# adelacvg/NS2VC

Measured on AMD Instinct MI355X. Metric: denoiser-steps/sec (10s@24kHz Vocos latent, bs32), higher is better.
Workload: dtype fp16; 1 GPU; 10 s utterance (T=938 Vocos frames), batch 32/GPU, prompt Lp=469, 20-step unipc order 2, hipGraph-captured loop, fp16 MFMA operands; timed job = set_condition + 20 steps; global_batch=32, frames=938, prompt_frames=469, solver=unipc, parallelism=dp1

## Files before the change

ns2vc_amd/csrc/attn.hip:

```cpp
#include "common.h"
#include "mma.h"
#include <cstdlib>

namespace ns2vc {

template <typename T> struct AMma;
template <> struct AMma<float> {
  static constexpr int SZ = 4;
  __device__ static __forceinline__ void mma(f32x16_t& acc, const u32x4_t& a, const u32x4_t& b) {
    acc = __builtin_amdgcn_mfma_f32_32x32x2f32(__uint_as_float(a.x), __uint_as_float(b.x), acc, 0, 0, 0);
    acc = __builtin_amdgcn_mfma_f32_32x32x2f32(__uint_as_float(a.y), __uint_as_float(b.y), acc, 0, 0, 0);
    acc = __builtin_amdgcn_mfma_f32_32x32x2f32(__uint_as_float(a.z), __uint_as_float(b.z), acc, 0, 0, 0);
    acc = __builtin_amdgcn_mfma_f32_32x32x2f32(__uint_as_float(a.w), __uint_as_float(b.w), acc, 0, 0, 0);
  }
  __device__ static __forceinline__ f32x16_t mma0(const u32x4_t& a, const u32x4_t& b) {
    f32x16_t acc = __builtin_amdgcn_mfma_f32_32x32x2f32(__uint_as_float(a.x), __uint_as_float(b.x), f32x16_t{0.f, 0.f, 0.f, 0.f, 0.f, 0.f, 0.f, 0.f, 0.f, 0.f, 0.f, 0.f, 0.f, 0.f, 0.f, 0.f}, 0, 0, 0);
    acc = __builtin_amdgcn_mfma_f32_32x32x2f32(__uint_as_float(a.y), __uint_as_float(b.y), acc, 0, 0, 0);
    acc = __builtin_amdgcn_mfma_f32_32x32x2f32(__uint_as_float(a.z), __uint_as_float(b.z), acc, 0, 0, 0);
    acc = __builtin_amdgcn_mfma_f32_32x32x2f32(__uint_as_float(a.w), __uint_as_float(b.w), acc, 0, 0, 0);
    return acc;
  }
  __device__ static __forceinline__ int vpos(int key) { return key; }
};
template <typename TM> struct AMma16 {
// ... 34 lines not shown
  return fmaxf(__uint_as_float(r[0]), __uint_as_float(r[1]));
}
__device__ __forceinline__ float half_sum(float v) {
  const auto r = __builtin_amdgcn_permlane32_swap(__float_as_uint(v), __float_as_uint(v), false, false);
  return __uint_as_float(r[0]) + __uint_as_float(r[1]);
}

template <typename TM> __device__ __forceinline__ float round_op(float x);
template <> __device__ __forceinline__ float round_op<float>(float x) { return x; }
template <> __device__ __forceinline__ float round_op<bf16_t>(float x) { return __uint_as_float(pack_bf16x2(0.f, x) & 0xffff0000u); }
template <> __device__ __forceinline__ float round_op<f16_t>(float x) { return f16_lo(pack_f16x2(x, 0.f)); }
template <typename TM> __device__ __forceinline__ u32x4_t aux_chunk(float e0, float e1);
template <> __device__ __forceinline__ u32x4_t aux_chunk<float>(float e0, float e1) { return u32x4_t{__float_as_uint(e0), __float_as_uint(e1), 0u, 0u}; }
template <> __device__ __forceinline__ u32x4_t aux_chunk<bf16_t>(float e0, float e1) { return u32x4_t{pack_bf16x2(e0, e1), 0u, 0u, 0u}; }
template <> __device__ __forceinline__ u32x4_t aux_chunk<f16_t>(float e0, float e1) { return u32x4_t{pack_f16x2(e0, e1), 0u, 0u, 0u}; }
template <typename TM> __device__ __forceinline__ TM op_from_float(float x);
template <> __device__ __forceinline__ float op_from_float<float>(float x) { return x; }
template <> __device__ __forceinline__ bf16_t op_from_float<bf16_t>(float x) { bf16_t r; r.v = (uint16_t)pack_bf16x2(x, 0.f); return r; }
template <> __device__ __forceinline__ f16_t op_from_float<f16_t>(float x) { f16_t r; r.v = (uint16_t)pack_f16x2(x, 0.f); return r; }

__device__ __forceinline__ uint32_t pack_fp8x4(float a, float b, float c, float d) {
  int v = __builtin_amdgcn_cvt_pk_fp8_f32(a, b, 0, false);
  v = __builtin_amdgcn_cvt_pk_fp8_f32(c, d, v, true);
  return (uint32_t)v;
}
typedef int i32x8_t __attribute__((ext_vector_type(8)));
#ifndef NS2VC_ATTN_OPT
#define NS2VC_ATTN_OPT 1
#endif
template <bool B> struct OptTag { static constexpr bool value = B; };
__device__ int g_attn_exact_only = 0;
__device__ __forceinline__ int vpos8(int key) { return ((key & 4) << 3) | ((key & 32) >> 1) | ((key & 24) >> 1) | (key & 3); }
template <typename TM, int HD, int KEYS, bool P8, bool MASKED = false>
__global__ __launch_bounds__(256) void attn_kernel(const AttnArgs a) {
  op_mode_init<TM>();
  static_assert(!P8 || (sizeof(TM) == 2 && KEYS == 64), "the fp8 PV path: 16-bit operand types, one 64-key tile per f8f6f4 MFMA");
  constexpr int NSUB = KEYS / 32;
  constexpr int SZ = AMma<TM>::SZ;
  constexpr int EPC = 16 / SZ;
  constexpr int NS = HD * SZ / 32;
  constexpr int KROWB = HD * SZ + 48;
  constexpr int VSZ = P8 ? 1 : SZ;
  constexpr int VROWB = KEYS * VSZ + 16;
  constexpr int HDX = (HD + 1 + 31) / 32 * 32;
  constexpr int DT = HDX / 32;
  constexpr int NSL = SZ;
  constexpr int KBYTES = KEYS * KROWB, VBYTES = HDX * VROWB;
  constexpr int STAGE = KBYTES + VBYTES;
  constexpr int PPR = HD * SZ / 16;
  constexpr int NPIECE = KEYS * PPR;
  constexpr int UPT = (NPIECE + 255) / 256;
  constexpr float THRESH = P8 ? 8.0f : 12.0f;
  extern __shared__ __attribute__((aligned(16))) char smem[];

  const int tid = threadIdx.x, lane = tid & 63, wave = tid >> 6;
  const int l31 = lane & 31, hi = lane >> 5;
  const int nqb = (a.Lq + 127) >> 7;
  int b, h, qb;
  {
    const int nwg = gridDim.x, bid = blockIdx.x;
    const int qn = nwg >> 3, rn = nwg & 7, xcd = bid & 7, idx = bid >> 3;
    const int swz = (xcd < rn ? xcd * (qn + 1) : rn * (qn + 1) + (xcd - rn) * qn) + idx;
    b = swz / (a.H * nqb);
    const int rem = swz - b * (a.H * nqb);
    h = rem / nqb;
    qb = rem - h * nqb;
  }
  const int q = qb * 128 + wave * 32 + l31;
  int Lqb = a.Lq, Lkb = a.Lk;
  if constexpr (MASKED) {
    if (a.q_lens) Lqb = min(max(a.q_lens[b], 0), a.Lq);
    if (a.k_lens) Lkb = min(max(a.k_lens[b], 1), a.Lk);
    if (qb * 128 >= Lqb) {
      if (q < a.Lq) {
        char* zp = reinterpret_cast<char*>(a.out) + ((size_t)(b * a.Lq + q) * a.ldo + h * HD) * SZ;
#pragma unroll
        for (int pc = hi; pc < PPR; pc += 2) *reinterpret_cast<u32x4_t*>(zp + pc * 16) = u32x4_t{0, 0, 0, 0};
      }
      return;
    }
  }
  const float LOG2E = 1.4426950408889634f;
  const float sc2 = a.scale * LOG2E;

  for (int i = tid * 16; i < 2 * STAGE; i += 256 * 16) *reinterpret_cast<u32x4_t*>(smem + i) = u32x4_t{0, 0, 0, 0};
  __syncthreads();
  for (int i = tid; i < 2 * KEYS; i += 256) {
    const int st = i / KEYS, key = i - st * KEYS;
    *reinterpret_cast<TM*>(smem + st * STAGE + key * KROWB + HD * SZ) = op_from_float<TM>(1.0f);
    if constexpr (P8) *reinterpret_cast<uint8_t*>(smem + st * STAGE + KBYTES + HD * VROWB + key) = (uint8_t)0x38;
    else *reinterpret_cast<TM*>(smem + st * STAGE + KBYTES + HD * VROWB + key * SZ) = op_from_float<TM>(1.0f);
  }

// ... 232 lines not shown
          const uint32_t b0 = Op16<TM>::pack(o[d][8 * gp + 4] * inv, o[d][8 * gp + 5] * inv), b1 = Op16<TM>::pack(o[d][8 * gp + 6] * inv, o[d][8 * gp + 7] * inv);
          const auto x0 = __builtin_amdgcn_permlane32_swap(a0, b0, false, false);
          const auto x1 = __builtin_amdgcn_permlane32_swap(a1, b1, false, false);
#if defined(NS2VC_ATTN_ABLATE_STORE)
          asm volatile("" :: "v"(x0[0]), "v"(x1[0]), "v"(x0[1]), "v"(x1[1]));
#else
          if (q < a.Lq) *reinterpret_cast<u32x4_t*>(op + d * 32 + 8 * (2 * gp + hi)) = padded ? u32x4_t{0, 0, 0, 0} : u32x4_t{x0[0], x1[0], x0[1], x1[1]};
#endif
        }
      }
  } else if (q < a.Lq) {
#pragma unroll
    for (int d = 0; d < DT; ++d)
#pragma unroll
      for (int gq = 0; gq < 4; ++gq) {
        const int d0 = d * 32 + 8 * gq + 4 * hi;
        if (d0 < HD) store_op4<TM>(op + d0, padded ? 0.f : o[d][4 * gq] * inv, padded ? 0.f : o[d][4 * gq + 1] * inv, padded ? 0.f : o[d][4 * gq + 2] * inv,
                                   padded ? 0.f : o[d][4 * gq + 3] * inv);
      }
  }
}

template <typename TM, int HD, int KEYS> static constexpr size_t attn_lds() {
  constexpr int SZ = AMma<TM>::SZ;
  constexpr int HDX = (HD + 1 + 31) / 32 * 32;
  return 2 * (size_t)(KEYS * (HD * SZ + 48) + HDX * (KEYS * SZ + 16));
}

template <typename TM, int HD> static constexpr bool attn_has128() { return sizeof(TM) == 2 && HD <= 32; }
static int g_force_keys = 0;
void set_forced_attn_keys(int keys) { g_force_keys = keys; }
void set_attn_optimistic(int on) { const int v = on ? 0 : 1; (void)hipMemcpyToSymbol(HIP_SYMBOL(g_attn_exact_only), &v, sizeof(v)); }

template <typename TM, int HD, int KEYS> static hipError_t launch_hdk(const AttnArgs& a, hipStream_t s) {
  dim3 grid(((a.Lq + 127) / 128) * a.H * a.B);
  const size_t lds = attn_lds<TM, HD, KEYS>();
  if (a.q_lens || a.k_lens) hipLaunchKernelGGL((attn_kernel<TM, HD, KEYS, false, true>), grid, dim3(256), lds, s, a);
  else hipLaunchKernelGGL((attn_kernel<TM, HD, KEYS, false>), grid, dim3(256), lds, s, a);
  return hipGetLastError();
}
template <typename TM, int HD> static hipError_t launch_hd(const AttnArgs& a, hipStream_t s) {
  if (a.pv_fp8 && (a.q_lens || a.k_lens)) return hipErrorInvalidValue;
  if constexpr (sizeof(TM) == 2) {
    if (a.pv_fp8) {
      dim3 grid(((a.Lq + 127) / 128) * a.H * a.B);
      const size_t lds = attn_lds<TM, HD, 64>();
      hipLaunchKernelGGL((attn_kernel<TM, HD, 64, true>), grid, dim3(256), lds, s, a);
      return hipGetLastError();
    }
  } else if (a.pv_fp8) return hipErrorInvalidValue;
  if constexpr (attn_has128<TM, HD>()) {
    if (g_force_keys == 128) return launch_hdk<TM, HD, 128>(a, s);
  }
  return launch_hdk<TM, HD, 64>(a, s);
}

template <typename TM> static hipError_t launch_tm(const AttnArgs& a, int hd, hipStream_t s) {
  switch (hd) {
    case 16: return launch_hd<TM, 16>(a, s);
    case 32: return launch_hd<TM, 32>(a, s);
    case 48: return launch_hd<TM, 48>(a, s);
    case 64: return launch_hd<TM, 64>(a, s);
    default: return hipErrorInvalidValue;
  }
}

template <typename TM, int HD> static hipError_t set_attr() {
  hipError_t e = hipFuncSetAttribute(reinterpret_cast<const void*>(attn_kernel<TM, HD, 64, false>), hipFuncAttributeMaxDynamicSharedMemorySize,
                                     (int)attn_lds<TM, HD, 64>());
  if (e == hipSuccess)
    e = hipFuncSetAttribute(reinterpret_cast<const void*>(attn_kernel<TM, HD, 64, false, true>), hipFuncAttributeMaxDynamicSharedMemorySize,
                            (int)attn_lds<TM, HD, 64>());
  if constexpr (attn_has128<TM, HD>()) {
    if (e == hipSuccess)
      e = hipFuncSetAttribute(reinterpret_cast<const void*>(attn_kernel<TM, HD, 128, false>), hipFuncAttributeMaxDynamicSharedMemorySize,
                              (int)attn_lds<TM, HD, 128>());
    if (e == hipSuccess)
      e = hipFuncSetAttribute(reinterpret_cast<const void*>(attn_kernel<TM, HD, 128, false, true>), hipFuncAttributeMaxDynamicSharedMemorySize,
                              (int)attn_lds<TM, HD, 128>());
  }
  if constexpr (sizeof(TM) == 2) {
    if (e == hipSuccess)
      e = hipFuncSetAttribute(reinterpret_cast<const void*>(attn_kernel<TM, HD, 64, true>), hipFuncAttributeMaxDynamicSharedMemorySize,
                              (int)attn_lds<TM, HD, 64>());
  }
  return e;
}
template <typename TM> static hipError_t set_attr_tm() {
  hipError_t e;
  if ((e = set_attr<TM, 16>()) != hipSuccess) return e;
  if ((e = set_attr<TM, 32>()) != hipSuccess) return e;
  if ((e = set_attr<TM, 48>()) != hipSuccess) return e;
  return set_attr<TM, 64>();
}
hipError_t init_attn_attributes() {
  hipError_t e = set_attr_tm<float>();
  if (e == hipSuccess) e = set_attr_tm<bf16_t>();
  if (e == hipSuccess) e = set_attr_tm<f16_t>();
  return e;
}

bool attention_masks_rows(const AttnArgs& a, int head_dim, int prec) {
  if (a.pv_fp8) return false;
  if (head_dim != 16 && head_dim != 32 && head_dim != 48 && head_dim != 64) return false;
  return prec == PREC_BF16 || prec == PREC_F16 || prec == PREC_F32;
}

hipError_t launch_attention(const AttnArgs& a, int head_dim, int prec, hipStream_t s) {
  const int al = prec == PREC_F32 ? 3 : 7;
  if (!a.q || !a.k || !a.v || !a.out) return hipErrorInvalidValue;
  if ((a.q_lens || a.k_lens) && !attention_masks_rows(a, head_dim, prec)) return hipErrorInvalidValue;
  if (a.Lq <= 0 || a.Lk <= 0 || (a.ldq & al) || (a.ldk & al) || (a.ldv & al) || (a.ldo & al)) return hipErrorInvalidValue;
  if (reinterpret_cast<uintptr_t>(a.out) & 15) return hipErrorInvalidValue;
  switch (prec) {
    case PREC_BF16: return launch_tm<bf16_t>(a, head_dim, s);
    case PREC_F16: return launch_tm<f16_t>(a, head_dim, s);
    case PREC_F32: return launch_tm<float>(a, head_dim, s);
    default: return hipErrorInvalidValue;
  }
}

}
```

ns2vc_amd/csrc/common.h:

```cpp
#pragma once
#include <hip/hip_runtime.h>
#include <stdint.h>
#include <stddef.h>
#include <vector>
#include "../../include/ns2vc_hip.h"

namespace ns2vc {

typedef __attribute__((ext_vector_type(8))) __bf16 bf16x8_t;
typedef __attribute__((ext_vector_type(16))) float f32x16_t;
typedef __attribute__((ext_vector_type(4))) float f32x4_t;
typedef __attribute__((ext_vector_type(4))) unsigned int u32x4_t;

struct bf16_t { uint16_t v; };
struct f16_t { uint16_t v; };

__host__ __device__ inline uint16_t f32_to_bf16_bits(float f) {
  union { float f; uint32_t u; } x;
  x.f = f;
  uint32_t u = x.u;
  if ((u & 0x7fffffffu) > 0x7f800000u) return (uint16_t)((u >> 16) | 0x40);
  u += 0x7fffu + ((u >> 16) & 1u);
  return (uint16_t)(u >> 16);
}
__host__ __device__ inline float bf16_bits_to_f32(uint16_t h) {
  union { float f; uint32_t u; } x;
  x.u = (uint32_t)h << 16;
  return x.f;
}

__host__ __device__ inline uint16_t f32_to_f16_bits(float f) {
  union { float f; uint32_t u; } x;
  x.f = f;
  const uint32_t sign = (x.u >> 16) & 0x8000u;
  uint32_t a = x.u & 0x7fffffffu;
  if (a > 0x7f800000u) return (uint16_t)(sign | 0x7e00u);
  if (a >= 0x477ff000u) return (uint16_t)(sign | 0x7c00u);
  if (a < 0x38800000u) {
// ... 172 lines not shown
  const float nd = k.d1c * (vmp - m) + d2c * dm2;
  oxb = nb; od1 = nd; oxe = nb - k.pc * nd - pe * dm2; om = m;
}

__device__ __forceinline__ uint4 philox4x32_10(uint4 c, uint32_t k0, uint32_t k1) {
#pragma unroll
  for (int r = 0; r < 10; ++r) {
    if (r) { k0 += 0x9E3779B9u; k1 += 0xBB67AE85u; }
    const uint32_t lo0 = 0xD2511F53u * c.x, hi0 = __umulhi(0xD2511F53u, c.x);
    const uint32_t lo1 = 0xCD9E8D57u * c.z, hi1 = __umulhi(0xCD9E8D57u, c.z);
    c = make_uint4(hi1 ^ c.y ^ k0, lo1, hi0 ^ c.w ^ k1, lo0);
  }
  return c;
}
__device__ __forceinline__ void box_muller(uint32_t a, uint32_t b, float& z0, float& z1) {
  const float u1 = ((float)a + 1.0f) * 0x1p-32f;
  const float u2 = (float)b * 0x1p-32f;
  const float r = sqrtf(-2.0f * logf(u1));
  float sn, cs;
  sincosf(u2 * 6.2831853071795864769f, &sn, &cs);
  z0 = r * cs; z1 = r * sn;
}
__device__ __forceinline__ float4 philox_gauss4(unsigned long long seed, uint32_t t, uint32_t q, uint32_t step) {
  const uint4 x = philox4x32_10(make_uint4(t, q, step, 0u), (uint32_t)seed, (uint32_t)(seed >> 32));
  float4 z;
  box_muller(x.x, x.y, z.x, z.y);
  box_muller(x.z, x.w, z.z, z.w);
  return z;
}

constexpr double GN_SUM_SCALE = 268435456.0;
constexpr double GN_SQ_SCALE = 65536.0;

hipError_t launch_gemm(const GemmArgs& g, int prec, hipStream_t s);
size_t xattn_pack_bytes(int B, int Lk, int hd);
hipError_t launch_xattn_pack(const void* k, int ldk, const void* v, int ldv, int B, int Lk, int hd, void* out, int prec, hipStream_t s);
bool gemm_masks_rows(const GemmArgs& g, int prec);
bool gemm_uses_convts(const GemmArgs& g, int prec);
int last_gemm_refusal_line();
hipError_t launch_attention(const AttnArgs& a, int head_dim, int prec, hipStream_t s);
bool attention_masks_rows(const AttnArgs& a, int head_dim, int prec);
hipError_t init_gemm_attributes();
bool convts_eligible(const GemmArgs& g, int prec);
int convts_default_bn(const GemmArgs& g);
int convts_bn_for(const GemmArgs& g, int bn128_min);
void set_convts_bn128_min(int wgs);
int convts_row_blocks(const GemmArgs& g);
hipError_t launch_convts(const GemmArgs& g, int prec, int bn, int nl, int ks, hipStream_t s);
hipError_t init_convts_attributes();
hipError_t pack_conv3_tiled(const float* rows, int N, int ctot, int c2, int prec, std::vector<unsigned char>& out);
void set_forced_gemm_tile(int bm, int bn, int stages);
void set_gemm_trace(unsigned long long* p);
hipError_t init_attn_attributes();
void set_forced_attn_keys(int keys);
hipError_t launch_ffn(const ::ns2vc_ffn_args& a, int prec, hipStream_t s);
bool ffn_eligible(int dim, int T, int prec);
bool ffn_masks_rows(const ::ns2vc_ffn_args& a, int prec);
hipError_t init_ffn_attributes();
hipError_t pack_ffn_stream(const float* w1p, const float* w2f, const float* w0, int dim, int prec, std::vector<unsigned short>& out);
void set_ffn_trace(unsigned long long* p);
bool geglu_eligible(int dim, int T, int prec);
hipError_t pack_geglu_stream(const float* w1p, const float* bias1p, int dim, int prec, std::vector<unsigned short>& stream, std::vector<float>& consts);
hipError_t launch_geglu(const ::ns2vc_geglu_args& a, int prec, hipStream_t s);
bool geglu_masks_rows(const ::ns2vc_geglu_args& a, int prec);
hipError_t init_geglu_attributes();
void set_gg_trace(unsigned long long* p);
void set_ts_trace(unsigned long long* p);
void set_attn_optimistic(int on);

hipError_t launch_gn_partial(const float* a0, int lda0, int c0, const float* a1, int lda1, int c1,
                             int B, int T, int G, double* partial, int nchunk, int rows_per_chunk, hipStream_t s);
hipError_t launch_gn_apply(const float* a0, int lda0, int c0, const float* a1, int lda1, int c1, int B, int T, int G, float eps,
                           const double* partial, int nchunk, const long long* st0, const long long* st1, const float* gamma,
                           const float* beta, const float* temb, int ldtemb, int temb_off, int silu, void* out_op, void* raw_op,
                           int prec, hipStream_t s, int pair = 0,
                           const int* lens = nullptr);
hipError_t launch_mask_rows(void* dst, size_t ldd_bytes, size_t row_bytes, int B, int T, const int* lens, hipStream_t s, const void* src = nullptr,
                            size_t lds_bytes = 0, int Tsrc = 0, int up = 0);
hipError_t launch_ln_apply_op(const float* x, int ldx, int M, int C, float eps, void* out_op, int prec, hipStream_t s);
hipError_t launch_cast_op(const float* x, size_t n, void* out_op, int prec, hipStream_t s, int split = 0);
hipError_t launch_time_embed(const float* t_ptr, int t_stride, const int* step_ptr, int coef_stride,
                             const float* w1t, const float* b1, const float* w2t, const float* b2,
                             const float* aug, float* emb, void* emb_act_op, int prec, int B, int tdim, int edim, hipStream_t s);
hipError_t launch_rowchain(const ::ns2vc_rowchain_args& a, int prec, hipStream_t s);
bool rowchain_eligible(int dim, int n2, int T, int prec);
bool rowchain_masks_rows(const ::ns2vc_rowchain_args& a, int prec);
hipError_t init_rowchain_attributes();
hipError_t pack_rowchain_stream(const float* w1, const float* w2, int dim, int n2, int prec, std::vector<unsigned short>& out, int slices = 1);
int rowchain_slice_blocks(int n2, int slices);
void set_rc_trace(unsigned long long* p);
void set_forced_rowchain_tokens(int nt);
hipError_t launch_emb_from_table(const float* table, const int* step_ptr, const float* aug, float* emb, void* emb_act_op, int prec, int B,
                                 int edim, hipStream_t s);
int probe_xcd_round_robin(unsigned* map8 = nullptr);
hipError_t launch_zero(void* p, size_t bytes, hipStream_t s, int* counter = nullptr);
hipError_t launch_copy16(const void* src, void* dst, size_t bytes, hipStream_t s);
hipError_t launch_poison(unsigned pattern, int lds_bytes, unsigned* sink, hipStream_t s);
hipError_t launch_nct_to_btc(const float* src, int C, int T, int B, float* dst_f32, void* dst_op, int prec, int ldd, int cpad, hipStream_t s,
                             int ldd_op = 0, int split = 0);
hipError_t launch_btc_to_nct(const float* src, int lds, int C, int T, int B, float* dst, hipStream_t s);
hipError_t launch_mask_bias(const uint8_t* mask, int n, float* bias, hipStream_t s);
hipError_t launch_ln_apply(const float* x, int M, int C, float eps, const float* gamma, const float* beta,
                           float* out, int L, int Lout_stride_rows, hipStream_t s);
hipError_t launch_pool_cls(float* seq, int B, int L, int C, const float* pos, hipStream_t s);
hipError_t launch_pool_attn(const float* qkv, int B, int L1, int C, int heads, float* pooled, hipStream_t s);
hipError_t launch_pool_proj(const float* pooled, int B, int C, const float* wt, const float* b, int E,
                            const float* gamma, const float* beta, float eps, float* out, hipStream_t s);
struct SolverNoise { const unsigned long long* seeds = nullptr; const int* lens = nullptr; int T = 0, ld = 0, nc = 0; };
hipError_t launch_solver_update(const float* coef, const int* step_ptr, int ncoef, const float* x0,
                                float* xe, void* xe_op, int prec, float* xbar, float* d1, float* mprev, size_t n, hipStream_t s,
                                int split = 0,
                                const SolverNoise& noise = SolverNoise(),
                                float* mprev2 = nullptr);
hipError_t launch_noise(const unsigned long long* seeds, int B, int nc, int T, int ld, int step, const int* lens, float* out, hipStream_t s);
hipError_t launch_fill_i32(int* p, int v, hipStream_t s);
hipError_t launch_placement(unsigned* dev_out, int n_blocks, int spin, hipStream_t s);
hipError_t launch_snapshot_u32(unsigned* src, unsigned* dst, hipStream_t s);
// ... 3 lines not shown
```

ns2vc_amd/csrc/convts.hip:

```cpp
#include "common.h"
#include "mma.h"
#include "gnpro.h"
#include "epilogue.h"
#include <type_traits>
#include <vector>
#include <cstring>

namespace ns2vc {

constexpr int TS_ROW = 128;
constexpr int TS_BM = 128;
constexpr int TS_BMO = 126;
constexpr int TS_ASLOT = TS_BM * TS_ROW;

__device__ unsigned long long* g_ts_trace = nullptr;
void set_ts_trace(unsigned long long* p) { (void)hipMemcpyToSymbol(HIP_SYMBOL(g_ts_trace), &p, sizeof(p)); }
#ifndef NS2VC_GEMM_TRACE
#define NS2VC_GEMM_TRACE 0
#endif
#if NS2VC_GEMM_TRACE
#define TS_NOW() __builtin_readcyclecounter()
#define TS_STAMP(i) do { if (tr && (tid == 0)) tr[i] = TS_NOW(); } while (0)
#define TS_CLK(t) do { t = TS_NOW(); } while (0)
#define TS_ACC(a, t) do { const unsigned long long n_ = TS_NOW(); a += n_ - t; t = n_; } while (0)
// ... 9 lines not shown
#endif
#ifndef NS2VC_TS_KS_DEFAULT
#define NS2VC_TS_KS_DEFAULT 0
#endif
#ifndef NS2VC_TS_NL_DEFAULT
#define NS2VC_TS_NL_DEFAULT 8
#endif
#ifndef NS2VC_TS_GNP_XB
#define NS2VC_TS_GNP_XB 4
#endif
#ifndef NS2VC_TS_NLD4
#define NS2VC_TS_NLD4 0
#endif
#ifndef NS2VC_CONS_PF
#define NS2VC_CONS_PF 1
#endif
#ifndef NS2VC_TS_CHUNK
#define NS2VC_TS_CHUNK 1
#endif
#if NS2VC_TS_CHUNK
template <int BN> struct TsRing { static constexpr int SW = BN == 64 ? 9 : 6; };
#else
template <int BN> struct TsRing { static constexpr int SW = 3; };
#endif
template <int LO, int HI> struct TsWait {
  static __device__ __forceinline__ void run(int n) {
    if constexpr (LO == HI) wait_vmcnt<LO>();
    else { constexpr int MID = (LO + HI + 1) / 2; if (n >= MID) TsWait<MID, HI>::run(n); else TsWait<LO, MID - 1>::run(n); }
  }
};

enum { TS_GN_NONE = 0, TS_GN_PRO = 1, TS_GN_INLOOP = 2, TS_GN_PAIR = 3, TS_MASKED = 4 };
template <typename TM, int BN, int NL, int GNPF, bool KS = false, bool SOL = false>
__global__ __launch_bounds__(64 * (NL + 4)) void conv3ts_kernel(const GemmArgs g) {
  constexpr int GNP = GNPF & 3;
  constexpr bool MASKED = (GNPF & TS_MASKED) != 0;
  op_mode_init<TM>();
  constexpr int EPC = MmaT<TM>::EPC;
  constexpr int BKE = 8 * EPC;
  constexpr int NW = NL + 4, EOFF = NW - 8;
  constexpr int NLD = (GNP == 2 || (NS2VC_TS_CHUNK && NS2VC_TS_NLD4 && NL == 8)) ? 4 : NL;
  constexpr int LTH = NLD * 64, RPP = LTH / 8, PASSB = RPP * TS_ROW;
  constexpr int LA = TS_BM / RPP, LB = BN / RPP;
  static_assert(!KS || BN == 64, "the K-split consumer layout is the 64-column tile's");
  constexpr int WGN = BN / 64, WGM = KS ? 2 : 4 / WGN, WM = TS_BM / WGM, MT = WM / 32, NT = 2;
  constexpr int NKK = KS ? 2 : 4;
  constexpr int WSLOT = BN * TS_ROW;
  constexpr int SW = TsRing<BN>::SW, D = SW - 1;
  constexpr unsigned SZB = sizeof(TM);
  static_assert(BN == 64 || BN == 128, "BN");
  static_assert(LA >= 1 && LB >= 1 && (NS2VC_TS_CHUNK ? SW : D) * LB + 3 * LA <= 60, "vmcnt range");
  extern __shared__ __attribute__((aligned(16))) char smem[];
  char* const aring = smem;
  char* const wring = smem + 3 * TS_ASLOT;
  char* const tabmem = smem + 3 * TS_ASLOT + SW * WSLOT;
  static_assert(GNP != 2 || NS2VC_TS_CHUNK, "the in-loop GroupNorm rides the chunk-granular loop");

  const int tid = threadIdx.x;
  const int lane = tid & 63;
  const int wave = __builtin_amdgcn_readfirstlane(tid >> 6);
  const bool loader = wave < NLD, consumer = wave >= NL;
  const bool producer = GNP == 2 && wave >= NLD && wave < NL;
  const int ewave = wave - EOFF;
  const int cw = consumer ? wave - NL : 0;
  const int wm = KS ? cw >> 1 : cw / WGN, wn = KS ? 0 : cw % WGN;
  const int kh = KS ? cw & 1 : 0;
  const unsigned lds0 = (unsigned)(size_t)smem;
// ... 440 lines not shown
        for (int p = 0; p < 8; ++p) {
          const int lc = p ^ ((r >> 1) & 7);
          for (int e = 0; e < epc; ++e) {
            const float v = rows[(size_t)n * K + koff + lc * epc + e];
            unsigned char* dst = blk + r * 128 + p * 16 + e * esz;
            if (prec == PREC_F32) memcpy(dst, &v, 4);
            else { const uint16_t q = f32_to_op16_bits(v, prec); memcpy(dst, &q, 2); }
          }
        }
      }
    }
  return hipSuccess;
}

static constexpr size_t ts_lds_bytes(int bn) { return (size_t)3 * TS_ASLOT + (size_t)(bn == 64 ? TsRing<64>::SW : TsRing<128>::SW) * bn * TS_ROW + 4096; }

bool convts_eligible(const GemmArgs& g, int prec) {
  const int bke = prec == PREC_F32 ? 32 : 64;
  if (g.taps != 3 || g.tmode != TMODE_SAME || g.Tin != g.Tout || g.Tin < 66 || g.geglu || g.rowstats || g.ln_stats) return false;
  if ((g.N % 64) || (g.c0 % bke) || (g.c1 % bke) || (g.c2 % bke) || g.c0 + g.c1 < bke) return false;
  if ((unsigned long long)g.B * (g.Tin + 1) > 0x7fff0000ull) return false;
  if (g.sol_coef && (g.N != 128 || !g.sol_step || !g.sol_xe || !g.sol_xe_op || !g.sol_xbar || !g.sol_d1 || !g.sol_mprev || (g.sol_ld & 3))) return false;
  return true;
}
static int g_bn128_min = 160;
void set_convts_bn128_min(int wgs) { g_bn128_min = wgs > 0 ? wgs : 160; }
int convts_bn_for(const GemmArgs& g, int bn128_min) {
  const long long nbm = ((long long)g.B * (g.Tin + 1) + TS_BMO - 1) / TS_BMO;
  return ((g.N % 128) == 0 && nbm * (g.N / 128) >= bn128_min) ? 128 : 64;
}
int convts_default_bn(const GemmArgs& g) { return (g.conv_bn == 64 || (g.conv_bn == 128 && g.N % 128 == 0)) ? g.conv_bn : convts_bn_for(g, g_bn128_min); }
int convts_row_blocks(const GemmArgs& g) { return (int)(((long long)g.B * (g.Tin + 1) + TS_BMO - 1) / TS_BMO); }

template <typename TM, int BN, int NL, bool KS> static hipError_t launch_ts_cfg(const GemmArgs& g, hipStream_t s) {
  const int nbm = convts_row_blocks(g), nbn = g.N / BN;
  int nb = nbm * nbn;
  if (g.gnp_x && g.gnp_sync && nbn > 1) nb = 8 * ((nbm + 7) / 8) * nbn;
  constexpr bool HAS_INLOOP = NS2VC_TS_CHUNK && NL == 8 && !KS;
  if (g.lens) {
    constexpr bool HAS_MASKED = NL == 8 && !KS;
    if constexpr (HAS_MASKED) {
      if (g.sol_coef) return hipErrorInvalidValue;
      if (g.gnp_x && g.gnp_pair) {
        if constexpr (!std::is_same<TM, float>::value) hipLaunchKernelGGL((conv3ts_kernel<TM, BN, NL, TS_GN_PAIR | TS_MASKED, KS>), dim3(nb), dim3(64 * (NL + 4)), ts_lds_bytes(BN), s, g);
        else return hipErrorInvalidValue;
      }
      else if (g.gnp_x) hipLaunchKernelGGL((conv3ts_kernel<TM, BN, NL, TS_GN_PRO | TS_MASKED, KS>), dim3(nb), dim3(64 * (NL + 4)), ts_lds_bytes(BN), s, g);
      else hipLaunchKernelGGL((conv3ts_kernel<TM, BN, NL, TS_GN_NONE | TS_MASKED, KS>), dim3(nb), dim3(64 * (NL + 4)), ts_lds_bytes(BN), s, g);
    } else return hipErrorInvalidValue;
  }
  else if (g.sol_coef) {
    constexpr bool HAS_SOL = BN == 128 && NL == 8 && !KS;
    if constexpr (HAS_SOL) {
      if (g.gnp_x && g.gnp_pair) {
        if constexpr (!std::is_same<TM, float>::value) hipLaunchKernelGGL((conv3ts_kernel<TM, BN, NL, 3, KS, true>), dim3(nb), dim3(64 * (NL + 4)), ts_lds_bytes(BN), s, g);
        else return hipErrorInvalidValue;
      }
      else if (g.gnp_x) hipLaunchKernelGGL((conv3ts_kernel<TM, BN, NL, 1, KS, true>), dim3(nb), dim3(64 * (NL + 4)), ts_lds_bytes(BN), s, g);
      else hipLaunchKernelGGL((conv3ts_kernel<TM, BN, NL, 0, KS, true>), dim3(nb), dim3(64 * (NL + 4)), ts_lds_bytes(BN), s, g);
    } else return hipErrorInvalidValue;
  }
  else if (g.gnp_x && g.gnp_pair) {
    if constexpr (!std::is_same<TM, float>::value && NL == 8 && !KS) hipLaunchKernelGGL((conv3ts_kernel<TM, BN, NL, 3, KS>), dim3(nb), dim3(64 * (NL + 4)), ts_lds_bytes(BN), s, g);
    else return hipErrorInvalidValue;
  }
  else if (g.gnp_x && HAS_INLOOP && g.algo != 2) {
    if constexpr (HAS_INLOOP) hipLaunchKernelGGL((conv3ts_kernel<TM, BN, NL, 2, KS>), dim3(nb), dim3(64 * (NL + 4)), ts_lds_bytes(BN), s, g);
  }
  else if (g.gnp_x) hipLaunchKernelGGL((conv3ts_kernel<TM, BN, NL, 1, KS>), dim3(nb), dim3(64 * (NL + 4)), ts_lds_bytes(BN), s, g);
  else hipLaunchKernelGGL((conv3ts_kernel<TM, BN, NL, 0, KS>), dim3(nb), dim3(64 * (NL + 4)), ts_lds_bytes(BN), s, g);
  return hipGetLastError();
}
template <typename TM> static hipError_t launch_ts_typed(const GemmArgs& g, int bn, int nl, int ks, hipStream_t s) {
  if (bn == 64 && nl == 4) return ks ? launch_ts_cfg<TM, 64, 4, true>(g, s) : launch_ts_cfg<TM, 64, 4, false>(g, s);
  if (bn == 64 && nl == 8) return ks ? launch_ts_cfg<TM, 64, 8, true>(g, s) : launch_ts_cfg<TM, 64, 8, false>(g, s);
  if (bn == 128 && nl == 4) return launch_ts_cfg<TM, 128, 4, false>(g, s);
  if (bn == 128 && nl == 8) return launch_ts_cfg<TM, 128, 8, false>(g, s);
  return hipErrorInvalidValue;
}
hipError_t launch_convts(const GemmArgs& g, int prec, int bn, int nl, int ks, hipStream_t s) {
  if (!convts_eligible(g, prec)) return hipErrorInvalidValue;
  if (!bn) bn = convts_default_bn(g);
  if (!nl) nl = NS2VC_TS_NL_DEFAULT;
  if (ks < 0) ks = NS2VC_TS_KS_DEFAULT;
  if (g.sol_coef) { bn = 128; nl = 8; ks = 0; }
  if (g.lens) { nl = 8; ks = 0; }
  if (g.N % bn) return hipErrorInvalidValue;
  switch (prec) {
    case PREC_BF16: return launch_ts_typed<bf16_t>(g, bn, nl, ks, s);
    case PREC_F16: return launch_ts_typed<f16_t>(g, bn, nl, ks, s);
    case PREC_F32: return launch_ts_typed<float>(g, bn, nl, ks, s);
    default: return hipErrorInvalidValue;
  }
}

template <typename K> static hipError_t ts_set_lds(K kern, size_t bytes) {
  return hipFuncSetAttribute(reinterpret_cast<const void*>(kern), hipFuncAttributeMaxDynamicSharedMemorySize, (int)bytes);
}
template <typename TM> static hipError_t ts_init_typed() {
  hipError_t e = hipSuccess;
#define NS2VC_TS_SET(BN_, NL_)                                                                      \
  if (e == hipSuccess) e = ts_set_lds(conv3ts_kernel<TM, BN_, NL_, 0>, ts_lds_bytes(BN_));     \
  if (e == hipSuccess) e = ts_set_lds(conv3ts_kernel<TM, BN_, NL_, 1>, ts_lds_bytes(BN_))
  NS2VC_TS_SET(64, 4); NS2VC_TS_SET(128, 4); NS2VC_TS_SET(64, 8); NS2VC_TS_SET(128, 8);
#if NS2VC_TS_CHUNK
  if (e == hipSuccess) e = ts_set_lds(conv3ts_kernel<TM, 64, 8, 2>, ts_lds_bytes(64));
  if (e == hipSuccess) e = ts_set_lds(conv3ts_kernel<TM, 128, 8, 2>, ts_lds_bytes(128));
#endif
  if (e == hipSuccess) e = ts_set_lds(conv3ts_kernel<TM, 128, 8, 0, false, true>, ts_lds_bytes(128));
  if (e == hipSuccess) e = ts_set_lds(conv3ts_kernel<TM, 128, 8, 1, false, true>, ts_lds_bytes(128));
  if constexpr (!std::is_same<TM, float>::value) {
    if (e == hipSuccess) e = ts_set_lds(conv3ts_kernel<TM, 128, 8, 3, false, true>, ts_lds_bytes(128));
    if (e == hipSuccess) e = ts_set_lds(conv3ts_kernel<TM, 64, 8, 3>, ts_lds_bytes(64));
    if (e == hipSuccess) e = ts_set_lds(conv3ts_kernel<TM, 128, 8, 3>, ts_lds_bytes(128));
  }
  if (e == hipSuccess) e = ts_set_lds(conv3ts_kernel<TM, 64, 8, TS_GN_NONE | TS_MASKED>, ts_lds_bytes(64));
  if (e == hipSuccess) e = ts_set_lds(conv3ts_kernel<TM, 64, 8, TS_GN_PRO | TS_MASKED>, ts_lds_bytes(64));
  if (e == hipSuccess) e = ts_set_lds(conv3ts_kernel<TM, 128, 8, TS_GN_NONE | TS_MASKED>, ts_lds_bytes(128));
  if (e == hipSuccess) e = ts_set_lds(conv3ts_kernel<TM, 128, 8, TS_GN_PRO | TS_MASKED>, ts_lds_bytes(128));
  if constexpr (!std::is_same<TM, float>::value) {
    if (e == hipSuccess) e = ts_set_lds(conv3ts_kernel<TM, 64, 8, TS_GN_PAIR | TS_MASKED>, ts_lds_bytes(64));
    if (e == hipSuccess) e = ts_set_lds(conv3ts_kernel<TM, 128, 8, TS_GN_PAIR | TS_MASKED>, ts_lds_bytes(128));
  }
  if (e == hipSuccess) e = ts_set_lds(conv3ts_kernel<TM, 64, 4, 0, true>, ts_lds_bytes(64));
// ... 15 lines not shown
```

ns2vc_amd/csrc/engine.cpp:

```cpp
#include "engine_internal.h"

#include <algorithm>
#include <cstdlib>
#include <cstring>

using namespace ns2vc;

static int bind_device(ns2vc_unet* h) {
  int cur = -1;
  HIPCHK(hipGetDevice(&cur));
  if (cur != h->device) HIPCHK(hipSetDevice(h->device));
  return 0;
}
int ns2vc::check_ready(ns2vc_unet* h, bool need_plan) {
  if (!h) return fail("null engine handle");
  if (bind_device(h)) return 1;
  if (!h->finalized) return fail("weights not finalized (call ns2vc_unet_finalize_weights)");
  if (need_plan && !h->arena) return fail("engine not prepared (call ns2vc_unet_prepare)");
  return 0;
}

int ns2vc::load_state(ns2vc_unet* h, const float* x_bct, hipStream_t s) {
  HIPCHK(launch_nct_to_btc(x_bct, h->cfg.latent_channels, h->T, h->B, h->xe, h->xe_op, h->prec, h->CP, h->CP, s, h->pair_width(), h->pair_off()));
  if (!h->lens.masked) return 0;
  const size_t ob = (size_t)h->pair_width() * operand_bytes(h->prec);
  HIPCHK(launch_mask_rows(h->xe, (size_t)h->CP * 4, (size_t)h->CP * 4, h->B, h->T, h->lens.dev, s));
  HIPCHK(launch_mask_rows(h->xe_op, ob, ob, h->B, h->T, h->lens.dev, s));
  return 0;
}

static const struct { const char* name; const char* env; bool ns2vc_unet::* member; } kOptions[] = {
  {"ln_linear", "NS2VC_LN_LINEAR", &ns2vc_unet::ln_linear}, {"fold_ff", "NS2VC_FOLD_FF", &ns2vc_unet::fold_ff},
  {"fuse_ffn", "NS2VC_FUSE_FFN", &ns2vc_unet::fuse_ffn}, {"fuse_ffn_pre", "NS2VC_FUSE_FFN_PRE", &ns2vc_unet::fuse_ffn_pre},
  {"fuse_geglu", "NS2VC_FUSE_GEGLU", &ns2vc_unet::fuse_geglu}, {"fuse_rows", "NS2VC_FUSE_ROWS", &ns2vc_unet::fuse_rows},
  {"fuse_rows_gn", "NS2VC_FUSE_ROWS_GN", &ns2vc_unet::fuse_rows_gn}, {"fuse_gn_gemm", "NS2VC_FUSE_GN_GEMM", &ns2vc_unet::fuse_gn_gemm},
  {"fuse_gn_cat", "NS2VC_FUSE_GN_CAT", &ns2vc_unet::fuse_gn_cat}, {"gn_coop", "NS2VC_GN_COOP", &ns2vc_unet::gn_coop},
  {"slice_rows", "NS2VC_SLICE_ROWS", &ns2vc_unet::slice_rows}, {"attn_fp8", "NS2VC_ATTN_FP8", &ns2vc_unet::attn_fp8},
  {"attn_optimistic", "NS2VC_ATTN_OPTIMISTIC", &ns2vc_unet::attn_optimistic}, {"conv_ts", "NS2VC_CONV_TS", &ns2vc_unet::conv_ts},
  {"conv_wtiled", "NS2VC_CONV_WTILED", &ns2vc_unet::conv_wtiled}, {"gn_inloop", "NS2VC_GN_INLOOP", &ns2vc_unet::gn_inloop},
  {"fuse_solver", "NS2VC_FUSE_SOLVER", &ns2vc_unet::fuse_solver}, {"fuse_xattn", "NS2VC_FUSE_XATTN", &ns2vc_unet::fuse_xattn},
  {"fork_temb", "NS2VC_FORK_TEMB", &ns2vc_unet::fork_temb}, {"exact_io", "NS2VC_EXACT_IO", &ns2vc_unet::exact_io},
  {"split_io", "NS2VC_SPLIT_IO", &ns2vc_unet::split_io}, {"masked_fuse", "NS2VC_MASKED_FUSE", &ns2vc_unet::masked_fuse},
  {"masked_attn", "NS2VC_MASKED_ATTN", &ns2vc_unet::masked_attn}, {"masked_rows", "NS2VC_MASKED_ROWS", &ns2vc_unet::masked_rows},
  {"masked_ffn", "NS2VC_MASKED_FFN", &ns2vc_unet::masked_ffn}, {"masked_geglu", "NS2VC_MASKED_GEGLU", &ns2vc_unet::masked_geglu}};
static bool* option_ptr(ns2vc_unet* h, const char* name) {
  for (const auto& o : kOptions)
    if (!strcmp(name, o.name)) return &(h->*o.member);
  return nullptr;
}

extern "C" {

int ns2vc_unet_create(const ns2vc_unet_cfg* cfg, ns2vc_unet** out) {
  if (!cfg || !out) return fail("null argument");
  if (cfg->n_levels < 2 || cfg->n_levels > NS2VC_MAX_LEVELS) return fail("n_levels=%d out of range (2..%d)", cfg->n_levels, NS2VC_MAX_LEVELS);
  if (cfg->latent_channels <= 0 || cfg->latent_channels > 128) return fail("latent_channels=%d must be in 1..128", cfg->latent_channels);
  if (cfg->content_channels <= 0 || cfg->content_channels % 64)
    return fail("content_channels=%d must be a positive multiple of 64", cfg->content_channels);
  if (cfg->cross_attention_dim <= 0 || cfg->cross_attention_dim % 128)
    return fail("cross_attention_dim=%d must be a positive multiple of 128", cfg->cross_attention_dim);
  if (cfg->heads < 1) return fail("heads=%d must be >= 1", cfg->heads);
  if (cfg->norm_num_groups < 1 || cfg->norm_num_groups > 8) return fail("norm_num_groups=%d unsupported (1..8)", cfg->norm_num_groups);
  if (cfg->layers_per_block < 1) return fail("layers_per_block=%d must be >= 1", cfg->layers_per_block);
  if (cfg->pool_heads < 1 || cfg->cross_attention_dim % cfg->pool_heads || cfg->cross_attention_dim / cfg->pool_heads > 8)
    return fail("cross_attention_dim=%d over pool_heads=%d: the pool head width must be a whole number <= 8", cfg->cross_attention_dim, cfg->pool_heads);
  if (cfg->block_out_channels[0] != 128) return fail("block_out_channels[0]=%d must be 128 (padded latent width)", cfg->block_out_channels[0]);
  for (int l = 0; l < cfg->n_levels; ++l) {
    const int c = cfg->block_out_channels[l];
    if (c <= 0 || c % 128 || c > 512) return fail("block_out_channels[%d]=%d must be a multiple of 128 in 128..512", l, c);
    if (c % cfg->heads) return fail("block_out_channels[%d]=%d not divisible by heads=%d", l, c, cfg->heads);
    const int hd = c / cfg->heads;
    if (hd != 16 && hd != 32 && hd != 48 && hd != 64)
      return fail("heads=%d gives head width %d at block_out_channels[%d]=%d (16/32/48/64 supported)", cfg->heads, hd, l, c);
    if (c % cfg->norm_num_groups || (c / cfg->norm_num_groups) % 4)
      return fail("block_out_channels[%d]=%d incompatible with norm_num_groups=%d (group width must be a multiple of 4)", l, c, cfg->norm_num_groups);
  }
  for (const BlockW& b : make_topology(*cfg))
// ... 304 lines not shown
int ns2vc_unet_tap_info(ns2vc_unet* h, int idx, char* name, int buflen, int* rows, int* cols) {
  if (!h || idx < 0 || idx >= (int)h->taps.size()) return fail("tap index out of range");
  snprintf(name, buflen, "%s", h->taps[idx].name.c_str());
  *rows = h->taps[idx].rows; *cols = h->taps[idx].cols;
  return 0;
}
int ns2vc_unet_tap_read(ns2vc_unet* h, int idx, float* host_dst) {
  if (!h || idx < 0 || idx >= (int)h->taps.size()) return fail("tap index out of range");
  HIPCHK(hipDeviceSynchronize());
  const Tap& t = h->taps[idx];
  HIPCHK(hipMemcpy(host_dst, t.copy, (size_t)t.rows * t.cols * sizeof(float), hipMemcpyDeviceToHost));
  return 0;
}
int ns2vc_unet_num_launches(ns2vc_unet* h, int* per_forward, int* per_condition) {
  if (!h) return fail("null engine handle");
  if (per_forward) *per_forward = (int)h->fwd_ops.size();
  if (per_condition) *per_condition = (int)h->cond_ops.size();
  return 0;
}

int ns2vc_unet_op_info(ns2vc_unet* h, int which, int idx, char* name, int buflen, int* kind, double* flops, double* bytes) {
  if (!h) return fail("null engine handle");
  if (which == 2) {
    static const char* const field[6] = {"begin", "end", "join", "first_reader", "readers", "forks"};
    if (!h->arena) return fail("engine not prepared (call ns2vc_unet_prepare)");
    if (idx < 0 || idx >= 6) return fail("op index out of range");
    GemmArgs g;
    const int v[6] = {h->tfork.begin, h->tfork.end, h->tfork.join, h->tfork.first, h->tfork.readers,
                      temb_forks(h, solver_in_conv_out(h, g) ? (size_t)h->conv_out_idx : h->fwd_ops.size()) ? 1 : 0};
    snprintf(name, buflen, "%s", field[idx]);
    *kind = v[idx]; *flops = 0.0; *bytes = 0.0;
    return 0;
  }
  const std::vector<Op>& ops = which ? h->cond_ops : h->fwd_ops;
  if (idx < 0 || idx >= (int)ops.size()) return fail("op index out of range");
  snprintf(name, buflen, "%s", ops[idx].name.c_str());
  *kind = ops[idx].kind; *flops = ops[idx].flops; *bytes = ops[idx].bytes;
  return 0;
}

int ns2vc_unet_profile_forward(ns2vc_unet* h, float* ms, int n_ms, int reps, void* stream) {
  if (check_ready(h, true)) return 1;
  const size_t n = h->fwd_ops.size();
  if ((size_t)n_ms < n) return fail("ms buffer too small: need %zu", n);
  if (reps < 1) reps = 1;
  hipStream_t s = (hipStream_t)stream;
  h->use_step_table = false;
  std::vector<hipEvent_t> ev(2 * n);
  for (auto& e : ev) HIPCHK(hipEventCreate(&e));
  int rc = 0;
  hipEvent_t rz0 = nullptr, rz1 = nullptr;
  const Op* rz_op = nullptr;
  for (size_t i = 0; i < n && !rc; ++i) {
    const Op& op = h->fwd_ops[i];
    if (op.rearm && !rz_op) rz_op = &op;
    if (hipEventRecord(ev[2 * i], s) != hipSuccess) rc = fail("hipEventRecord failed");
    for (int r = 0; r < reps && !rc; ++r) {
      hipError_t e = op.rearm ? op.rearm(s) : hipSuccess;
      if (e == hipSuccess) e = op.fn(s);
      if (e != hipSuccess) rc = fail("launch of '%s' failed: %s", op.name.c_str(), hipGetErrorString(e));
    }
    if (!rc && hipEventRecord(ev[2 * i + 1], s) != hipSuccess) rc = fail("hipEventRecord failed");
  }
  if (!rc && rz_op) {
    if (hipEventCreate(&rz0) != hipSuccess || hipEventCreate(&rz1) != hipSuccess) rc = fail("hipEventCreate failed");
    if (!rc) (void)hipEventRecord(rz0, s);
// ... 20 lines not shown
```

ns2vc_amd/csrc/engine_internal.h:

```cpp
#pragma once
#include "common.h"

#include <cstdarg>
#include <cstdio>
#include <functional>
#include <map>
#include <string>
#include <vector>

namespace ns2vc {

inline thread_local std::string g_err;

inline int fail(const char* fmt, ...) {
  char buf[1024];
  va_list ap;
  va_start(ap, fmt);
  vsnprintf(buf, sizeof(buf), fmt, ap);
  va_end(ap);
  g_err = buf;
  return 1;
}
#define HIPCHK(expr)                                                                                       \
  do {                                                                                                     \
    hipError_t _e = (expr);                                                                                \
    if (_e != hipSuccess) return ns2vc::fail("%s failed: %s (%s:%d)", #expr, hipGetErrorString(_e), __FILE__, __LINE__); \
  } while (0)

inline int round_up(int v, int m) { return (v + m - 1) / m * m; }

struct HostTensor {
  std::vector<float> data;
  std::vector<int64_t> shape;
  size_t numel() const { size_t n = 1; for (auto s : shape) n *= (size_t)s; return n; }
};

struct PackedW {
  void* w = nullptr;
  void* wt = nullptr;
// ... 10 lines not shown
  PackedW conv1, conv2, sc;
};
struct AttnW {
  std::string prefix;
  int dim = 0, kv_off = 0;
  float *ng = nullptr, *nb = nullptr;
  PackedW proj_in, qkv, o1, q2, o2, ff1, ff2, proj_out;
  PackedW ffpo;
  void* ffn_pre_stream = nullptr;
  void* ffn_stream = nullptr;
  float* ffn_consts = nullptr;
  void* geglu_stream = nullptr;
  float* geglu_consts = nullptr;
  void *chain_in = nullptr, *chain_mid = nullptr;
  void* chain_in_s2 = nullptr;
  float *chain_in_consts = nullptr, *chain_mid_consts = nullptr;
};
struct BlockW {
  std::string kind;
  int index = 0, level = 0, channels = 0;
  std::vector<ResnetW> res;
  std::vector<AttnW> attn;
  int sampler = 0;
  PackedW samp;
};

struct Op {
  std::string name;
  std::function<hipError_t(hipStream_t)> fn;
  int kind = 0;
  double flops = 0.0;
  double bytes = 0.0;
  std::function<hipError_t(hipStream_t)> rearm;
};
struct Tap {
  std::string name;
  float* copy = nullptr;
  int rows = 0, cols = 0;
};

struct Staged {
  void* buf = nullptr;
  size_t cap = 0;
  hipEvent_t event = nullptr;
  bool pending = false;
  int reserve(size_t bytes) {
    if (!event) HIPCHK(hipEventCreateWithFlags(&event, hipEventDisableTiming));
    if (pending) { HIPCHK(hipEventSynchronize(event)); pending = false; }
    if (cap < bytes) {
      if (buf) HIPCHK(hipHostFree(buf));
      buf = nullptr; cap = 0;
      HIPCHK(hipHostMalloc(&buf, bytes, hipHostMallocDefault));
      cap = bytes;
    }
    return 0;
  }
  int record(hipStream_t s) {
    HIPCHK(hipEventRecord(event, s));
    pending = true;
    return 0;
  }
  ~Staged() {
    if (pending) (void)hipEventSynchronize(event);
    if (event) (void)hipEventDestroy(event);
    if (buf) (void)hipHostFree(buf);
  }
};

}

struct ns2vc_unet {
  ns2vc_unet_cfg cfg{};
  std::map<std::string, ns2vc::HostTensor> raw;
  std::vector<std::pair<std::string, std::vector<int64_t>>> expected;
  int prec = -1;
  bool finalized = false;
  std::vector<void*> weight_allocs;

  std::vector<ns2vc::BlockW> blocks;
  ns2vc::PackedW conv_in_x, conv_in_c, conv_out, temb_all, kv_all, pool_qkv;
  ns2vc::PackedW conv_in_xp, conv_in_cp, conv_outp;
  ns2vc::PackedW conv_in_x32, conv_in_c32, conv_out32, temb_all32;
  float *t_w1t = nullptr, *t_b1 = nullptr, *t_w2t = nullptr, *t_b2 = nullptr;
  float *p_n1g = nullptr, *p_n1b = nullptr, *p_pos = nullptr, *p_projT = nullptr, *p_projb = nullptr, *p_n2g = nullptr, *p_n2b = nullptr;
  float *out_ng = nullptr, *out_nb = nullptr;
  int n_temb = 0, n_kv = 0;
  int CP = 128;

  int B = 0, T = 0, Lp = 0;
  void* arena = nullptr;
  size_t arena_bytes = 0, arena_used = 0;
  std::vector<ns2vc::Op> cond_ops, fwd_ops;
  size_t cond_split = 0;
  bool debug = false;
  int device = 0;
  bool ln_linear = true;
  bool fold_ff = true;
  bool fuse_ffn = true;
  bool fuse_rows = true;
  bool attn_fp8 = false;
  bool fuse_ffn_pre = true;
  bool fuse_geglu = true;
  bool fuse_rows_gn = true;
  bool fuse_gn_gemm = true;
  bool fuse_gn_cat = true;
  bool gn_coop = true;
  bool conv_ts = true;
  bool conv_wtiled = true;
  bool split_io = true;
  bool exact_io = false;
// ... 1 lines not shown
  float* emb_act_f32 = nullptr;
  int conv_out_prec = -1;
  bool fork_temb = false;
  struct TembFork {
    int begin = -1, end = -1, join = -1;
    int first = -1, readers = 0;
    bool ok = false;
    int join_skip = 0;
    hipStream_t side_stream = nullptr;
    hipEvent_t ev_fork = nullptr, ev_join = nullptr;
  } tfork;
  bool fuse_xattn = false;
  bool fuse_solver = false;
  ns2vc::GemmArgs conv_out_g;
  int conv_out_idx = -1;
  bool warned_wtiled = false;
  int bn128_min = 160;
  bool gn_inloop = false;
  int gn_coop_min = 2;
  int cus = 256;
  int xcd_probe = -1;
  bool slice_rows = true;
  unsigned* ln_health = nullptr;
  bool attn_optimistic = true;
  unsigned* attn_fallbacks = nullptr;
  unsigned long long coef_hash = 0;
  std::vector<ns2vc::Tap> taps;
  bool has_mask = false;
  bool masked_fuse = false;
  bool masked_attn = false;
  bool masked_rows = false;
  bool masked_ffn = false;
  bool masked_geglu = false;
  struct Lengths {
    bool masked = false;
    int* dev = nullptr;
    size_t off = 0;
    float* selfbias = nullptr;
    std::vector<int32_t> applied;
    ns2vc::Staged stage;
  } lens;
  struct Seeds {
    unsigned long long* dev = nullptr;
    int cap = 0;
    bool set = false;
    ns2vc::Staged stage;
  } seeds;
  bool stochastic = false;
  struct History2 {
    bool on = false;
    float* mprev2 = nullptr;
    size_t n = 0;
  } hist2;

  float *xe = nullptr, *xbar = nullptr, *d1 = nullptr, *mprev = nullptr, *x0 = nullptr;
  float *content_conv = nullptr, *prompt = nullptr, *maskbias = nullptr;
  float *aug = nullptr, *emb = nullptr, *temb = nullptr;
  float *seq = nullptr, *pool_qkv_buf = nullptr, *pooled = nullptr;
  void *xe_op = nullptr, *content_op = nullptr, *prompt_op = nullptr, *emb_act_op = nullptr, *kv = nullptr, *seq_op = nullptr;
  float *t_dev = nullptr;
  uint8_t* mask_dev = nullptr;
  int* step_dev = nullptr;
  size_t stats_bytes = 8;
  float* coef_dev = nullptr;
  float* temb_table = nullptr;
  bool temb_table_valid = false;
// ... 8 lines not shown

  hipStream_t cap_stream = nullptr;
  hipGraphExec_t step_graph = nullptr;

  int pair_width() const { return prec != ns2vc::PREC_F32 ? 2 * CP : CP; }
  int pair_off() const { return prec != ns2vc::PREC_F32 ? CP : 0; }

  ~ns2vc_unet() {
    if (seeds.dev) (void)hipFree(seeds.dev);
    if (hist2.mprev2) (void)hipFree(hist2.mprev2);
    if (step_graph) (void)hipGraphExecDestroy(step_graph);
    if (cap_stream) (void)hipStreamDestroy(cap_stream);
    if (tfork.side_stream) (void)hipStreamDestroy(tfork.side_stream);
    if (tfork.ev_fork) (void)hipEventDestroy(tfork.ev_fork);
    if (tfork.ev_join) (void)hipEventDestroy(tfork.ev_join);
    if (ln_out.event) (void)hipEventDestroy(ln_out.event);
    if (ln_out.mail) (void)hipHostFree(ln_out.mail);
    if (arena) (void)hipFree(arena);
    if (coef_dev) (void)hipFree(coef_dev);
    if (temb_table) (void)hipFree(temb_table);
    for (void* p : weight_allocs) (void)hipFree(p);
  }
};

namespace ns2vc {

std::vector<BlockW> make_topology(const ns2vc_unet_cfg& c);
void build_expected(ns2vc_unet* h);
std::vector<float> rounded_rowsum(const float* rows, int N, int K, int Np, int prec);
int pack_all(ns2vc_unet* h);
extern int g_geglu_min_rows;
std::vector<int> level_lengths(int T, int n_levels);
int build_plan(ns2vc_unet* h, bool sizing);
int run_ops(const std::vector<Op>& ops, hipStream_t s, size_t first = 0, size_t last = (size_t)-1);
bool temb_forks(const ns2vc_unet* h, size_t last);
void drop_step_graph(ns2vc_unet* h);
void drop_plan(ns2vc_unet* h);
int check_ready(ns2vc_unet* h, bool need_plan);
int load_state(ns2vc_unet* h, const float* x_bct, hipStream_t s);
bool solver_in_conv_out(ns2vc_unet* h, GemmArgs& g);
hipError_t init_all_attributes();
int xcd_round_robin_of_current_device();

}
```

ns2vc_amd/csrc/ffn.hip:

```cpp
#include "common.h"
#include <type_traits>
#include "mma.h"
#include <vector>

namespace ns2vc {

typedef ::ns2vc_ffn_args FfnArgs;

__device__ unsigned long long* g_ffn_trace = nullptr;
#ifndef NS2VC_GEMM_TRACE
#define NS2VC_GEMM_TRACE 0
#endif
#ifndef NS2VC_FFN_FENCE
#define NS2VC_FFN_FENCE 1
#endif
#ifndef NS2VC_FFN_WARM
#define NS2VC_FFN_WARM 1
#endif
#if NS2VC_FFN_FENCE == 1
#define FFN_FRAG_FENCE() do { asm volatile("s_waitcnt lgkmcnt(0)" ::: "memory"); __builtin_amdgcn_sched_barrier(0); } while (0)
#elif NS2VC_FFN_FENCE == 2
#define FFN_FRAG_FENCE() __builtin_amdgcn_sched_barrier(0)
#else
#define FFN_FRAG_FENCE() do {} while (0)
#endif
#if NS2VC_GEMM_TRACE
#define FFN_NOW() __builtin_readcyclecounter()
#define FFN_TR(i, v) do { if (tr && tid == 0) tr[i] = (v); } while (0)
#else
#define FFN_NOW() 0ull
#define FFN_TR(i, v) do { (void)tr; } while (0)
#endif
void set_ffn_trace(unsigned long long* p) { (void)hipMemcpyToSymbol(HIP_SYMBOL(g_ffn_trace), &p, sizeof(p)); }

#ifndef NS2VC_XATT_ABLATE
#define NS2VC_XATT_ABLATE 0
#endif
__device__ __forceinline__ float half_max_f(float v) {
  const auto r = __builtin_amdgcn_permlane32_swap(__float_as_uint(v), __float_as_uint(v), false, false);
  return fmaxf(__uint_as_float(r[0]), __uint_as_float(r[1]));
}
__device__ __forceinline__ float exp2f_fast(float x) { return __builtin_amdgcn_exp2f(x); }

constexpr int FFN_TILE = 128 * 128;
constexpr int FFN_PAIR = 2 * FFN_TILE;

template <int D, bool PRE = false> struct FfnGeom {
  static constexpr int RING = D <= 128 ? 4 : 3;
  static constexpr int KT = D / 64;
  static constexpr int NB = D / 32;
  static constexpr int NSS = D / 32;
  static constexpr int NB128 = D / 128;
  static constexpr int PO_STEPS = NB128 * KT / 2;
  static constexpr int PRE_PAIRS = PRE ? NB128 * KT / 2 : 0;
  static constexpr int PAIRS = PRE_PAIRS + NSS * (KT + NB128) + PO_STEPS;
  static constexpr int PANEL = KT * 64 * 128;
  static constexpr int CONSTS = 8 * D * 8;
  static constexpr int XCH = PRE ? 64 * 4 * 8 : 0;
  static constexpr int LDS = RING * FFN_PAIR + PANEL + CONSTS + XCH;
  static_assert(LDS <= 160 * 1024, "LDS budget");
  static constexpr int EP = 36;
  static_assert(2 * 2 * 4 * 32 * EP * 4 <= RING * FFN_PAIR, "epilogue staging (two 32-channel blocks) fits in the ring");
  static_assert(NB * 512 * 8 <= PANEL, "per-lane statistics partials fit in the panel");
};

template <typename TM, int D, bool PRE, bool ATT = false, bool MASKED = false>
__global__ __launch_bounds__(512) void ffn_kernel(const FfnArgs a) {
  op_mode_init<TM>();
  static_assert(!ATT || PRE, "the in-kernel cross-attention feeds the pre-stage");
  static_assert(!(ATT && MASKED), "the in-kernel cross-attention has no masked form");
  using G = FfnGeom<D, PRE>;
  constexpr int KT = G::KT, NB = G::NB, NSS = G::NSS, NB128 = G::NB128, NP = G::PAIRS, EP = G::EP, RING = G::RING;
  extern __shared__ __attribute__((aligned(16))) char smem[];
  char* const ring = smem;
  char* const panel = smem + RING * FFN_PAIR;
  const float* const consts = reinterpret_cast<const float*>(panel + G::PANEL);

  const int tid = threadIdx.x, lane = tid & 63;
  const int wave = __builtin_amdgcn_readfirstlane(tid >> 6);
  const int tw = wave & 1, hw = wave >> 1;
  const int l31 = lane & 31, hi = lane >> 5;
  const int sw = (l31 >> 1) & 7;
  const unsigned lds0 = (unsigned)(size_t)smem;
  const int nbi = ATT ? (a.T + 63) >> 6 : 1;
  const int ab = ATT ? (int)blockIdx.x / nbi : 0;
  const int m0 = ATT ? ab * a.T + ((int)blockIdx.x - ab * nbi) * 64 : (int)blockIdx.x * 64;
  const int mlim = ATT ? (ab + 1) * a.T : a.M;
  const int mtok = m0 + 32 * tw + l31;
  bool live_p = false, live_t = false, live_e = false;
  if constexpr (MASKED) {
    const int nitem = a.M / a.T, ib = min(m0 / a.T, nitem - 1);
    const int l0 = a.lens[ib], l1 = a.lens[min(ib + 1, nitem - 1)];
    const int end0 = ib * a.T + min(max(l0, 0), a.T), start1 = (ib + 1) * a.T;
    const int end1 = ib + 1 < nitem ? start1 + min(max(l1, 0), a.T) : start1;
    auto live = [&](int m) __attribute__((always_inline)) { return m < end0 || (m >= start1 && m < end1); };
    const int em = m0 + (tid >> 3);
    live_p = live(m0 + 8 * wave + (lane >> 3));
    live_t = live(mtok);
    live_e = live(em);
    if (!(m0 < end0 || (start1 < m0 + 64 && start1 < end1))) {
// ... 106 lines not shown
              for (int r = 0; r < 16; ++r) pr[r] = (NS2VC_XATT_ABLATE & 2) ? sa[r] : exp2f_fast(fmaf(sa[r], sc2, -m2[qs]));
              const u32x4_t p0 = u32x4_t{Op16<TM>::pack(pr[0], pr[1]), Op16<TM>::pack(pr[2], pr[3]), Op16<TM>::pack(pr[4], pr[5]), Op16<TM>::pack(pr[6], pr[7])};
              const u32x4_t p1 = u32x4_t{Op16<TM>::pack(pr[8], pr[9]), Op16<TM>::pack(pr[10], pr[11]), Op16<TM>::pack(pr[12], pr[13]), Op16<TM>::pack(pr[14], pr[15])};
              if (NS2VC_XATT_ABLATE & 4) { oacc[qs][0][0] += __uint_as_float(p0.x ^ p1.y ^ vf[j][0].x ^ vf[j][1].w); }
              else {
              MmaT<TM>::mma(oacc[qs][0], vf[j][0], p0);
              MmaT<TM>::mma(oacc[qs][0], vf[j][1], p1);
              if constexpr (HD == 32) { MmaT<TM>::mma(oacc[qs][1], ones, p0); MmaT<TM>::mma(oacc[qs][1], ones, p1); }
              }
            }
            if (!(NS2VC_XATT_ABLATE & 8)) { load_k(t0 + j + PD, kf[j], kb[j]); load_v(t0 + j + PD, vf[j]); }
          }
        }
      }
    }
#pragma unroll
    for (int qs = 0; qs < 2; ++qs) {
      const int tokq = 32 * qs + l31;
      float den = HD == 16 ? oacc[qs][0][8] : oacc[qs][NO - 1][0];
      den = __shfl(den, l31);
      const float inv = m0 + tokq < mlim ? 1.0f / den : 0.f;
      const int swt = (tokq >> 1) & 7;
#pragma unroll
      for (int g = 0; g < HD / 8; ++g) {
        const int n = hd0 + 8 * g + 4 * hi;
        char* dst = panel + (n >> 6) * 8192 + tokq * 128 + ((((n & 63) >> 3) ^ swt) * 16) + 8 * hi;
        *reinterpret_cast<uint2*>(dst) = make_uint2(Op16<TM>::pack(oacc[qs][0][4 * g] * inv, oacc[qs][0][4 * g + 1] * inv),
                                                    Op16<TM>::pack(oacc[qs][0][4 * g + 2] * inv, oacc[qs][0][4 * g + 3] * inv));
      }
    }
  }
#if NS2VC_FFN_WARM
  {
    const unsigned nx = (gridDim.x + 7) >> 3, jx = blockIdx.x >> 3;
    const unsigned total = (unsigned)NP * FFN_PAIR;
    const unsigned per = (((total + nx - 1) / nx) + 8191u) & ~8191u;
    for (unsigned off = jx * per + wave * 1024; off < min(total, (jx + 1) * per); off += 8192)
      blds16(rW, lane16, off, lds0 + (RING - 1) * FFN_PAIR + wave * 1024);
  }
#endif
  {
    const int prow = 8 * wave + (lane >> 3), pchunk = lane & 7;
    const int m = m0 + prow;
    const int ldp = PRE ? a.pre_lda : a.ldy;
    const unsigned voff = (MASKED ? live_p : m < mlim) ? (unsigned)m * (unsigned)ldp * 2u + (unsigned)((pchunk ^ ((prow >> 1) & 7)) * 16) : DMA_OOB;
    const i32x4_t rY = make_rsrc(PRE ? a.pre_a : a.yn, (unsigned long long)a.M * ldp * 2ull);
    if constexpr (!ATT) {
#pragma unroll
      for (int kt = 0; kt < KT; ++kt) blds16(rY, voff, (unsigned)(kt * 128), lds0 + RING * FFN_PAIR + kt * 8192 + wave * 1024);
    }
    const i32x4_t rC = make_rsrc(a.consts, (unsigned long long)G::CONSTS);
#pragma unroll
    for (int j = 0; j < G::CONSTS / 8192; ++j)
      blds16(rC, (unsigned)(lane * 16), (unsigned)((j * 8 + wave) * 1024), lds0 + RING * FFN_PAIR + G::PANEL + (j * 8 + wave) * 1024);
  }
  float4 b0[NB128][4], rr0[NB128][4];
  if constexpr (PRE && MASKED) {
#pragma unroll
    for (int rb = 0; rb < NB128; ++rb)
#pragma unroll
      for (int g = 0; g < 4; ++g) {
        b0[rb][g] = *reinterpret_cast<const float4*>(a.pre_bias + 128 * rb + 32 * hw + 8 * g + 4 * hi);
        rr0[rb][g] = make_float4(0.f, 0.f, 0.f, 0.f);
      }
    if (live_t) {
#pragma unroll
      for (int rb = 0; rb < NB128; ++rb)
// ... 331 lines not shown
    for (int pos = 0; pos < 8; ++pos) {
      const int lc = pos ^ ((r >> 1) & 7);
      for (int e = 0; e < 8; ++e) {
        const int k = lc * 8 + e;
        const int col = col0 + (perm ? perm[k] : k);
        out.push_back(f32_to_op16_bits(mat[(size_t)(row0 + r) * ld + col], prec));
      }
    }
}

hipError_t pack_ffn_stream(const float* w1p, const float* w2f, const float* w0, int dim, int prec, std::vector<unsigned short>& out) {
  if ((dim != 128 && dim != 256) || (prec != PREC_BF16 && prec != PREC_F16)) return hipErrorInvalidValue;
  const int KT = dim / 64, NSS = dim / 32, NB128 = dim / 128;
  int perm[64];
  for (int k = 0; k < 64; ++k) perm[k] = (k & ~12) | ((k & 4) << 1) | ((k & 8) >> 1);
  out.clear();
  out.reserve((size_t)(NSS * (KT + NB128) + NB128 * KT) * FFN_PAIR / 2);
  if (w0)
    for (int kt = 0; kt < KT; ++kt)
      for (int rb = 0; rb < NB128; ++rb) append_tile(out, w0, dim, 128 * rb, 64 * kt, prec, nullptr);
  for (int ss = 0; ss < NSS; ++ss) {
    for (int kt = 0; kt < KT; ++kt)
      for (int half = 0; half < 2; ++half) append_tile(out, w1p, dim, 256 * ss + 128 * half, 64 * kt, prec, nullptr);
    for (int nb = 0; nb < NB128; ++nb)
      for (int kt2 = 0; kt2 < 2; ++kt2) append_tile(out, w2f, 5 * (size_t)dim, 128 * nb, 128 * ss + 64 * kt2, prec, perm);
  }
  for (int nb = 0; nb < NB128; ++nb)
    for (int kt = 0; kt < KT; ++kt) append_tile(out, w2f, 5 * (size_t)dim, 128 * nb, 4 * dim + 64 * kt, prec, nullptr);
  return hipSuccess;
}

bool ffn_eligible(int dim, int T, int prec) { return (dim == 128 || dim == 256) && T >= 64 && (prec == PREC_BF16 || prec == PREC_F16); }

template <typename TM, int D> static hipError_t launch_ffn_t(const FfnArgs& a, hipStream_t s) {
  if (a.lens) {
    const size_t lds = a.pre_a ? FfnGeom<D, true>::LDS : FfnGeom<D, false>::LDS;
    if (a.pre_a) hipLaunchKernelGGL((ffn_kernel<TM, D, true, false, true>), dim3((a.M + 63) / 64), dim3(512), lds, s, a);
    else hipLaunchKernelGGL((ffn_kernel<TM, D, false, false, true>), dim3((a.M + 63) / 64), dim3(512), lds, s, a);
  } else if (a.att_q) {
    const size_t lds = FfnGeom<D, true>::LDS;
    hipLaunchKernelGGL((ffn_kernel<TM, D, true, true>), dim3(a.B * ((a.T + 63) / 64)), dim3(512), lds, s, a);
  } else if (a.pre_a) {
    const size_t lds = FfnGeom<D, true>::LDS;
    hipLaunchKernelGGL((ffn_kernel<TM, D, true>), dim3((a.M + 63) / 64), dim3(512), lds, s, a);
  } else {
    const size_t lds = FfnGeom<D, false>::LDS;
    hipLaunchKernelGGL((ffn_kernel<TM, D, false>), dim3((a.M + 63) / 64), dim3(512), lds, s, a);
  }
  return hipGetLastError();
}

bool ffn_masks_rows(const FfnArgs& a, int prec) {
  return ffn_eligible(a.dim, a.T, prec) && a.B >= 1 && a.M == a.B * a.T && !a.att_q;
}

hipError_t launch_ffn(const FfnArgs& a, int prec, hipStream_t s) {
  if (!ffn_eligible(a.dim, a.T, prec) || a.M <= 0 || a.M != a.B * a.T) return hipErrorInvalidValue;
  if (a.lens) {
    if (!ffn_masks_rows(a, prec)) return hipErrorInvalidValue;
  }
  if (!a.wstream || !a.consts || !a.bias2 || !a.res || (!a.out_f32 && !a.out_op)) return hipErrorInvalidValue;
  if (a.att_q) {
    if (!a.pre_bias || !a.pre_res || (a.pre_ldres & 3) || !a.att_kv || a.att_Lk < 1 || (a.att_ldq & 7) ||
        ((reinterpret_cast<uintptr_t>(a.att_q) | reinterpret_cast<uintptr_t>(a.att_kv)) & 15) || !(a.att_scale > 0.f))
      return hipErrorInvalidValue;
  } else if (a.pre_a ? (!a.pre_bias || !a.pre_res || (a.pre_lda & 7) || (a.pre_ldres & 3) || (unsigned long long)a.M * a.pre_lda * 2ull > 0xFFF00000ull)
              : (!a.yn || !a.ln_stats))
    return hipErrorInvalidValue;
  if ((!a.pre_a && !a.att_q && (a.ldy & 7)) || (a.ldres & 3) || (a.out_f32 && (a.ldo_f32 & 3)) || (a.out_op && (a.ldo_op & 3))) return hipErrorInvalidValue;
  if (!a.pre_a && !a.att_q && (unsigned long long)a.M * a.ldy * 2ull > 0xFFF00000ull) return hipErrorInvalidValue;
  if (prec == PREC_BF16) return a.dim == 128 ? launch_ffn_t<bf16_t, 128>(a, s) : launch_ffn_t<bf16_t, 256>(a, s);
  return a.dim == 128 ? launch_ffn_t<f16_t, 128>(a, s) : launch_ffn_t<f16_t, 256>(a, s);
}

template <typename TM>
__global__ __launch_bounds__(256) void xattn_pack_kernel(const TM* __restrict__ k, int ldk, const TM* __restrict__ v, int ldv, int Lk, int ntile, int hd, uint4* __restrict__ out) {
  const int nsl = hd >> 4, nfr = nsl + 2;
  const size_t piece = (size_t)blockIdx.x * 256 + threadIdx.x;
  const size_t total = (size_t)gridDim.y * ntile * nfr * 64;
  (void)total;
  const int bh = blockIdx.y;
  if (piece >= (size_t)ntile * nfr * 64) return;
  const int lane = (int)(piece & 63), frag = (int)((piece >> 6) % nfr), t = (int)((piece >> 6) / nfr);
  const int b = bh >> 3, hh = bh & 7, l31 = lane & 31, hi = lane >> 5;
  union { uint4 u; uint16_t e[8]; } r;
  r.u = make_uint4(0u, 0u, 0u, 0u);
  const uint16_t one = std::is_same<TM, f16_t>::value ? (uint16_t)0x3C00 : (uint16_t)0x3F80;
  if (frag < nsl) {
    const int key = 32 * t + l31;
    if (key < Lk) r.u = *reinterpret_cast<const uint4*>(k + (size_t)(b * Lk + key) * ldk + hh * hd + 16 * frag + 8 * hi);
  } else {
    const int j = frag - nsl, d = l31;
#pragma unroll
    for (int e = 0; e < 8; ++e) {
      const int slot = 16 * j + 8 * hi + e;
      const int key = 32 * t + ((slot & ~12) | ((slot & 4) << 1) | ((slot & 8) >> 1));
      if (d < hd) { if (key < Lk) r.e[e] = v[(size_t)(b * Lk + key) * ldv + hh * hd + d].v; }
      else if (d == hd && hd == 16) r.e[e] = one;
    }
  }
  out[((size_t)bh * ntile * nfr) * 64 + piece] = r.u;
}
size_t xattn_pack_bytes(int B, int Lk, int hd) { return (size_t)B * 8 * (size_t)((Lk + 31) >> 5) * (size_t)((hd >> 4) + 2) * 1024; }
hipError_t launch_xattn_pack(const void* k, int ldk, const void* v, int ldv, int B, int Lk, int hd, void* out, int prec, hipStream_t s) {
  if (!k || !v || !out || B < 1 || Lk < 1 || (hd != 16 && hd != 32) || (prec != PREC_BF16 && prec != PREC_F16) || (ldk & 7) ||
// ... 33 lines not shown
```

ns2vc_amd/csrc/geglu.hip:

```cpp
#include "common.h"
#include "mma.h"
#include <type_traits>
#include <vector>

#ifndef NS2VC_GG_ABLATE
#define NS2VC_GG_ABLATE 0
#endif

#ifndef NS2VC_GEMM_TRACE
#define NS2VC_GEMM_TRACE 0
#endif
#ifndef NS2VC_GG_PRIO
#define NS2VC_GG_PRIO 0
#endif
#ifndef NS2VC_GG_ROTATE
#define NS2VC_GG_ROTATE 0
#endif
#ifndef NS2VC_GG_PINGPONG
#define NS2VC_GG_PINGPONG 1
#endif

namespace ns2vc {

typedef ::ns2vc_geglu_args GegluArgs;
// ... 4 lines not shown
#define GG_NOW() __builtin_readcyclecounter()
#define GG_ACC(i) do { const unsigned long long t_ = GG_NOW(); tacc[i] += t_ - tmark; tmark = t_; } while (0)
#else
#define GG_NOW() 0ull
#define GG_ACC(i) do {} while (0)
#endif

constexpr int GG_TILE = 128 * 128;
constexpr int GG_TOK = 128;
constexpr int GG_SPLIT = 4;
constexpr int GG_RING = 8;

template <int D> struct GegluGeom {
  static constexpr int KT = D / 64;
  static constexpr int UB = 4 * D / 64 / GG_SPLIT;
  static constexpr int NP = UB * KT;
  static constexpr int CONSTS = UB * 128 * 8;
  static constexpr int STAGE = 4 * 32 * 128;
  static constexpr int LDS = GG_RING * GG_TILE + CONSTS + STAGE;
  static_assert(LDS <= 160 * 1024, "LDS budget");
  static_assert((4 * D / 64) % GG_SPLIT == 0, "whole unit blocks per quarter");
  static_assert(KT % 2 == 0, "fragment double buffer: the parity of a step is the parity of its K tile");
  static_assert(NP >= GG_RING, "prologue issues a full ring");
};

static inline int gg_unit_of_row(int m) { return 16 * ((m >> 2) & 1) + 4 * (m >> 3) + (m & 3); }

template <int N> __device__ __forceinline__ void gg_wait_tiles(int t) {
  if constexpr (N == 0) wait_vmcnt<0>();
  else { if (t >= N) wait_vmcnt<2 * N>(); else gg_wait_tiles<N - 1>(t); }
}

template <typename TM, int D, bool MASKED = false>
__global__ __launch_bounds__(512) void geglu_kernel(const GegluArgs a) {
  op_mode_init<TM>();
  using G = GegluGeom<D>;
  constexpr int KT = G::KT, UB = G::UB, NP = G::NP, RING = GG_RING;
  extern __shared__ __attribute__((aligned(16))) char smem[];
  char* const ring = smem;
  const float* const consts = reinterpret_cast<const float*>(smem + RING * GG_TILE);

  const int tid = threadIdx.x, lane = tid & 63;
  const int wave = __builtin_amdgcn_readfirstlane(tid >> 6);
  const int hg = wave & 1, tq = wave >> 1;
  unsigned long long tacc[8] = {0, 0, 0, 0, 0, 0, 0, 0}, tmark = 0;
  (void)tacc; (void)tmark;
  const unsigned long long t_entry = GG_NOW();
  (void)t_entry;
  const int l31 = lane & 31, hi = lane >> 5;
  const int sw = (l31 >> 1) & 7;
  const unsigned lds0 = (unsigned)(size_t)smem;

  const int ntb = (a.M + GG_TOK - 1) / GG_TOK;
  int tb, q;
  {
    const int nwg = ntb * GG_SPLIT, bid = blockIdx.x;
    const int qn = nwg >> 3, rn = nwg & 7, xcd = bid & 7, idx = bid >> 3;
    const int swz = (xcd < rn ? xcd * (qn + 1) : rn * (qn + 1) + (xcd - rn) * qn) + idx;
    tb = swz / GG_SPLIT;
    q = swz - tb * GG_SPLIT;
  }
  const int m0 = tb * GG_TOK;
  const int mtok = m0 + 32 * tq + l31;

  unsigned long long live_lo = 0ull, live_hi = 0ull;
  bool live_t = true;
  if constexpr (MASKED) {
// ... 326 lines not shown
}

bool geglu_eligible(int dim, int T, int prec) { return dim == 384 && T >= 1 && (prec == PREC_BF16 || prec == PREC_F16); }

hipError_t pack_geglu_stream(const float* w1p, const float* bias1p, int dim, int prec, std::vector<unsigned short>& stream, std::vector<float>& consts) {
  if (dim != 384 || (prec != PREC_BF16 && prec != PREC_F16)) return hipErrorInvalidValue;
  const int KT = dim / 64, NUB = 4 * dim / 64;
  stream.clear();
  stream.reserve((size_t)8 * dim * dim);
  consts.assign((size_t)8 * dim * 2, 0.f);
  auto src_row = [&](int sr) {
    const int grp = sr >> 6, half = (sr >> 5) & 1, m = sr & 31;
    return grp * 64 + half * 32 + gg_unit_of_row(m);
  };
  for (int ubg = 0; ubg < NUB; ++ubg)
    for (int kt = 0; kt < KT; ++kt)
      for (int r = 0; r < 128; ++r) {
        const int pr = src_row(ubg * 128 + r);
        for (int pos = 0; pos < 8; ++pos) {
          const int lc = pos ^ ((r >> 1) & 7);
          for (int e = 0; e < 8; ++e) stream.push_back(f32_to_op16_bits(w1p[(size_t)pr * dim + 64 * kt + lc * 8 + e], prec));
        }
      }
  for (int sr = 0; sr < 8 * dim; ++sr) {
    const int pr = src_row(sr);
    double s = 0.0;
    for (int k = 0; k < dim; ++k) s += (double)op16_bits_to_f32(f32_to_op16_bits(w1p[(size_t)pr * dim + k], prec), prec);
    consts[2 * sr] = (float)s;
    consts[2 * sr + 1] = bias1p ? bias1p[pr] : 0.f;
  }
  return hipSuccess;
}

template <typename TM, bool MASKED> static hipError_t launch_geglu_t(const GegluArgs& a, hipStream_t s) {
  const int ntb = (a.M + GG_TOK - 1) / GG_TOK;
  hipLaunchKernelGGL((geglu_kernel<TM, 384, MASKED>), dim3(ntb * GG_SPLIT), dim3(512), GegluGeom<384>::LDS, s, a);
  return hipGetLastError();
}

bool geglu_masks_rows(const GegluArgs& a, int prec) {
  return geglu_eligible(a.dim, 1, prec) && a.M > 0 && a.T >= 1 && (a.M % a.T) == 0;
}

hipError_t launch_geglu(const GegluArgs& a, int prec, hipStream_t s) {
  if (!geglu_eligible(a.dim, 1, prec) || a.M <= 0) return hipErrorInvalidValue;
  if (!a.yn || !a.wstream || !a.consts || !a.out_op) return hipErrorInvalidValue;
  if (!a.lens && !a.ln_stats) return hipErrorInvalidValue;
  if (a.lens && !geglu_masks_rows(a, prec)) return hipErrorInvalidValue;
  if (a.ldy < a.dim || a.ldo < 4 * a.dim || (a.ldy & 7) || (a.ldo & 7) || (unsigned long long)a.M * a.ldy * 2ull > 0xFFF00000ull || (unsigned long long)a.M * a.ldo * 2ull > 0x7FF00000ull) return hipErrorInvalidValue;
  if ((reinterpret_cast<uintptr_t>(a.out_op) & 15) != 0) return hipErrorInvalidValue;
  if (a.lens) return prec == PREC_BF16 ? launch_geglu_t<bf16_t, true>(a, s) : launch_geglu_t<f16_t, true>(a, s);
  return prec == PREC_BF16 ? launch_geglu_t<bf16_t, false>(a, s) : launch_geglu_t<f16_t, false>(a, s);
}

hipError_t init_geglu_attributes() {
  hipError_t e = hipFuncSetAttribute(reinterpret_cast<const void*>(geglu_kernel<bf16_t, 384, false>), hipFuncAttributeMaxDynamicSharedMemorySize, (int)GegluGeom<384>::LDS);
  if (e == hipSuccess) e = hipFuncSetAttribute(reinterpret_cast<const void*>(geglu_kernel<f16_t, 384, false>), hipFuncAttributeMaxDynamicSharedMemorySize, (int)GegluGeom<384>::LDS);
  if (e == hipSuccess) e = hipFuncSetAttribute(reinterpret_cast<const void*>(geglu_kernel<bf16_t, 384, true>), hipFuncAttributeMaxDynamicSharedMemorySize, (int)GegluGeom<384>::LDS);
  if (e == hipSuccess) e = hipFuncSetAttribute(reinterpret_cast<const void*>(geglu_kernel<f16_t, 384, true>), hipFuncAttributeMaxDynamicSharedMemorySize, (int)GegluGeom<384>::LDS);
  return e;
}

}
```

ns2vc_amd/csrc/gemm.hip:

```cpp
#include "common.h"
#include "mma.h"
#include "epilogue.h"

namespace ns2vc {

__device__ unsigned long long* g_gemm_trace = nullptr;
#ifndef NS2VC_GEMM_TRACE
#define NS2VC_GEMM_TRACE 0
#endif
#if NS2VC_GEMM_TRACE
#define NS2VC_STAMP(i) do { if (tr && tid == 0) tr[i] = __builtin_readcyclecounter(); } while (0)
#define NS2VC_TRACE_PTR() (g_gemm_trace ? g_gemm_trace + (size_t)blockIdx.x * 8 : nullptr)
#else
#define NS2VC_STAMP(i) do { (void)tr; } while (0)
#define NS2VC_TRACE_PTR() nullptr
#endif

constexpr int TROW = 128;

__device__ __forceinline__ void gemm_item_split(const GemmArgs& g, int mw0, int& b0, int& mB) {
  b0 = g.stats ? min(mw0, g.M - 1) / g.Tout : 0;
  mB = g.stats ? (b0 + 1) * g.Tout : 0x7fffffff;
}

// ... 273 lines not shown
      epi_linear_store<TM, LPR, NIT, true>(g, lane, lc.ncol, e, rowof);
    }
  }
  gn.template commit<LPR>(g, lane, b0, lc.ncol, mw0 < g.M, mB < g.M && mB < mw0 + WM);
#if NS2VC_GEMM_TRACE
  asm volatile("s_waitcnt vmcnt(0)" ::: "memory");
#endif
  NS2VC_STAMP(6);
}

#ifndef NS2VC_GEMM_ABLATE
#define NS2VC_GEMM_ABLATE 0
#endif
#ifndef NS2VC_G4_CONS_PF
#define NS2VC_G4_CONS_PF 0
#endif
#if NS2VC_GEMM_ABLATE
#define NS2VC_G4_FLAGS_PARAM , const int flags
#define NS2VC_G4_FLAG(b) ((flags & (b)) != 0)
#else
#define NS2VC_G4_FLAGS_PARAM
#define NS2VC_G4_FLAG(b) false
#endif
}
#include "gnpro.h"
namespace ns2vc {

template <int SPEC> struct G4Waves {
  static constexpr int NL = SPEC == 0 ? 8 : SPEC == 1 ? 4 : 8;
  static constexpr int NC = SPEC == 0 ? 8 : SPEC == 2 ? 8 : 4;
  static constexpr int NW = SPEC == 0 ? 8 : NL + NC;
};
template <typename TM, int BM, int BN, int STAGES, bool LNC, int SPEC = 0, bool GNP = false, bool MASKED = false>
__global__ __launch_bounds__(64 * G4Waves<SPEC>::NW) void gemm4_kernel(const GemmArgs g NS2VC_G4_FLAGS_PARAM) {
  op_mode_init<TM>();
  constexpr int EPC = MmaT<TM>::EPC;
  constexpr int BKE = 8 * EPC;
  constexpr int WM = BM / 2, WN = BN / 2, MT = WM / 32, NT = WN / 32;
  constexpr int NL = G4Waves<SPEC>::NL, NC = G4Waves<SPEC>::NC, NW = G4Waves<SPEC>::NW;
  constexpr int EOFF = NW - 8;
  constexpr int LTH = NL * 64;
  constexpr int RPP = LTH / 8;
  constexpr int PASSB = RPP * TROW;
  constexpr int LA = BM / RPP, LB = BN / RPP, LPT = LA + LB;
  constexpr int STAGE = (BM + BN) * TROW;
  static_assert(BN == 128 && NT == 2, "wave tile is (BM/2) x 64");
  static_assert(LPT * (STAGES - 1) < 60, "vmcnt range");
  extern __shared__ __attribute__((aligned(16))) char smem[];

  const int tid = threadIdx.x;
  const int lane = tid & 63;
  const int wave = __builtin_amdgcn_readfirstlane(tid >> 6);
  const int ewave = wave - EOFF;
  const int kg = (ewave >> 2) & 1, wq = ewave & 3;
  const int wm = wq >> 1, wn = wq & 1;
  const bool loader = SPEC == 0 || wave < NL;
  const bool consumer = SPEC == 0 || wave >= NW - NC;
  const unsigned lds0 = (unsigned)(size_t)smem;
  unsigned long long* tr = NS2VC_TRACE_PTR();
  NS2VC_STAMP(0);

  const int nb_n = g.N / BN;
  const int nb_m = (g.M + BM - 1) / BM;
  const int nwg = nb_n * nb_m;
  int tm, tn;
  const bool coop = GNP && g.gnp_x != nullptr && g.gnp_sync != nullptr && nb_n > 1;
  if (coop) {
// ... 244 lines not shown
    refill();
    multiply();
    if (++stage == STAGES) stage = 0;
  }

  if (SPEC != 0 && ewave < 0) return;
  gemm4_epilogue<TM, BM, LNC, MASKED>(g, acc, smem, m0, n0, tid - EOFF * 64, tr, lnraw);
}

static constexpr size_t gemm_lds_bytes(int bm, int bn, int stages) {
  const size_t ring = (size_t)stages * (bm + bn) * TROW;
  const size_t epi = (size_t)4 * (bm / 2) * (bn / 2 + 4) * 4;
  return ring > epi ? ring : epi;
}

static int g_gemm_flags = 0;
template <typename TM, int BM, int BN, int STAGES>
static hipError_t launch_cfg(const GemmArgs& g, hipStream_t s) {
  const int nb = (g.N / BN) * ((g.M + BM - 1) / BM);
  const size_t lds = gemm_lds_bytes(BM, BN, STAGES);
  if (g.ln_stats) hipLaunchKernelGGL((gemm2_kernel<TM, BM, BN, STAGES, true>), dim3(nb), dim3(256), lds, s, g, g_gemm_flags);
  else hipLaunchKernelGGL((gemm2_kernel<TM, BM, BN, STAGES, false>), dim3(nb), dim3(256), lds, s, g, g_gemm_flags);
  return hipGetLastError();
}

void set_gemm_trace(unsigned long long* p) { (void)hipMemcpyToSymbol(HIP_SYMBOL(g_gemm_trace), &p, sizeof(p)); }

static constexpr size_t gemm4_lds_bytes(int bm, int bn, int stages) {
  const size_t ring = (size_t)stages * (bm + bn) * TROW;
  const size_t epi = (size_t)8 * 32 * (bn / 2 + 4) * 4;
  return ring > epi ? ring : epi;
}
template <typename TM, int BM, int BN, int STAGES, int SPEC = 0>
static hipError_t launch_cfg4(const GemmArgs& g, hipStream_t s) {
  int nb = (g.N / BN) * ((g.M + BM - 1) / BM);
  if (g.gnp_x && g.gnp_sync && g.N / BN > 1) nb = 8 * (((g.M + BM - 1) / BM + 7) / 8) * (g.N / BN);
#if NS2VC_GEMM_ABLATE
  if (g.lens) return hipErrorInvalidValue;
  if (g.gnp_x) hipLaunchKernelGGL((gemm4_kernel<TM, BM, BN, STAGES, false, SPEC, true>), dim3(nb), dim3(64 * G4Waves<SPEC>::NW), gemm4_lds_bytes(BM, BN, STAGES), s, g, g_gemm_flags);
  else if (g.ln_stats) hipLaunchKernelGGL((gemm4_kernel<TM, BM, BN, STAGES, true, SPEC>), dim3(nb), dim3(64 * G4Waves<SPEC>::NW), gemm4_lds_bytes(BM, BN, STAGES), s, g, g_gemm_flags);
  else hipLaunchKernelGGL((gemm4_kernel<TM, BM, BN, STAGES, false, SPEC>), dim3(nb), dim3(64 * G4Waves<SPEC>::NW), gemm4_lds_bytes(BM, BN, STAGES), s, g, g_gemm_flags);
#else
  if (g.lens) hipLaunchKernelGGL((gemm4_kernel<TM, BM, BN, STAGES, false, SPEC, false, true>), dim3(nb), dim3(64 * G4Waves<SPEC>::NW), gemm4_lds_bytes(BM, BN, STAGES), s, g);
  else if (g.gnp_x) hipLaunchKernelGGL((gemm4_kernel<TM, BM, BN, STAGES, false, SPEC, true>), dim3(nb), dim3(64 * G4Waves<SPEC>::NW), gemm4_lds_bytes(BM, BN, STAGES), s, g);
  else if (g.ln_stats) hipLaunchKernelGGL((gemm4_kernel<TM, BM, BN, STAGES, true, SPEC>), dim3(nb), dim3(64 * G4Waves<SPEC>::NW), gemm4_lds_bytes(BM, BN, STAGES), s, g);
  else hipLaunchKernelGGL((gemm4_kernel<TM, BM, BN, STAGES, false, SPEC>), dim3(nb), dim3(64 * G4Waves<SPEC>::NW), gemm4_lds_bytes(BM, BN, STAGES), s, g);
#endif
  return hipGetLastError();
}

static thread_local int g_gemm_fail_line = 0;
static hipError_t gemm_invalid(int line) { g_gemm_fail_line = line; return hipErrorInvalidValue; }
int last_gemm_refusal_line() { const int l = g_gemm_fail_line; g_gemm_fail_line = 0; return l; }

static int g_force_bm = 0, g_force_bn = 0, g_force_st = 0;
static int g_ts = 1, g_ts_nl = 0, g_ts_ks = -1;
static int g_spec = 1;
void set_forced_gemm_tile(int bm, int bn, int stages) {
  if (bm == -1 || bm == -2) { g_spec = bm == -2 ? 1 : 0; return; }
  if (bm == -3 || bm == -4) { g_ts = bm == -4 ? 1 : 0; g_ts_nl = (bm == -4 && (stages == 4 || stages == 8)) ? stages : 0; g_ts_ks = bm == -4 ? (bn == 1 ? 1 : bn == 2 ? 0 : -1) : -1; return; } g_force_bm = bm; g_force_bn = bn; g_force_st = stages & 255; g_gemm_flags = stages >> 8; }

template <typename TM>
static hipError_t launch_typed(const GemmArgs& g, hipStream_t s, bool dry = false) {
  const int bke = 128 / (int)sizeof(TM);
  const int nk = g.K / bke;
  int bm, bn, st;
  const bool n128 = (g.N % 128) == 0;
  if (g_force_bm) {
    bm = g_force_bm; bn = g_force_bn; st = g_force_st ? g_force_st : 3;
    if (g.N % bn || ((g.geglu || g.rowstats) && bn != 128)) return gemm_invalid(__LINE__);
  } else {
    const bool big_m = g.M >= 7000;
    if (g.geglu) {
      if (!n128) return gemm_invalid(__LINE__);
      if (g.N >= 2048) { bm = 128; bn = 128; st = 12; }
      else { bm = 64; bn = 128; st = 2; }
    } else if (n128 && g.N <= 512) {
      bn = 128; st = 13;
      bm = (big_m && nk >= 12) ? 128 : 64;
      if (g_spec && nk >= 4 && (bm == 64 || g.M < 12000)) { bm = 64; st = 23; }
      else if (g_spec && bm == 128) st = 23;
      if (g.M >= 12000 && g.N > 128 && nk <= 2) { bm = 128; st = 12; }
    } else if (n128) {
      bn = 128;
      if (g.M >= 12000) { bm = 128; st = 12; } else { bm = 64; st = (g_spec && nk >= 4) ? 23 : 13; }
    } else {
      bm = 64; bn = 64; st = nk >= 32 ? 4 : (nk >= 20 ? 3 : 2);
    }
  }
  if (g.gnp_x && !((st >= 12 && st <= 13) || (st >= 22 && st <= 44))) return gemm_invalid(__LINE__);
  if (g.lens && !((st >= 12 && st <= 13) || (st >= 22 && st <= 44))) return gemm_invalid(__LINE__);
  if (dry) return hipSuccess;
  if (st >= 22 && st <= 44) {
    if (bn != 128) return gemm_invalid(__LINE__);
#define NS2VC_CASE4S(BM_, ST_, SP_) if (bm == BM_ && st == 10 * (1 + SP_) + ST_) return launch_cfg4<TM, BM_, 128, ST_, SP_>(g, s)
    NS2VC_CASE4S(128, 3, 1); NS2VC_CASE4S(64, 3, 1);
#undef NS2VC_CASE4S
    return gemm_invalid(__LINE__);
  }
  if (st == 12 || st == 13) {
    if (bn != 128) return gemm_invalid(__LINE__);
#define NS2VC_CASE4(BM_, ST_) if (bm == BM_ && st == 10 + ST_) return launch_cfg4<TM, BM_, 128, ST_>(g, s)
    NS2VC_CASE4(128, 2); NS2VC_CASE4(128, 3); NS2VC_CASE4(64, 2); NS2VC_CASE4(64, 3);
#undef NS2VC_CASE4
    return gemm_invalid(__LINE__);
  }
#define NS2VC_CASE(BM_, BN_, ST_) if (bm == BM_ && bn == BN_ && st == ST_) return launch_cfg<TM, BM_, BN_, ST_>(g, s)
  NS2VC_CASE(64, 128, 2);
  NS2VC_CASE(64, 64, 2); NS2VC_CASE(64, 64, 3); NS2VC_CASE(64, 64, 4);
#undef NS2VC_CASE
  return gemm_invalid(__LINE__);
}

hipError_t launch_gemm(const GemmArgs& g_, int prec, hipStream_t s) {
  GemmArgs g = g_;
  if (g.N % 64 != 0 || g.M <= 0) return gemm_invalid(__LINE__);
  if (g.N / 64 > 15) g.gnp_sync = nullptr;
  const int bke = prec == PREC_F32 ? 32 : 64;
  if (g.K % bke != 0 || g.c0 % bke != 0 || g.c1 % bke != 0 || g.c2 % bke != 0 || g.K != g.taps * (g.c0 + g.c1) + g.c2) return gemm_invalid(__LINE__);
  if (g.c2 && (!g.a2 || g.tmode != TMODE_SAME || (g.lda2 % (bke / 8)))) return gemm_invalid(__LINE__);
  if ((g.lda0 % (bke / 8)) || (g.c1 && (g.lda1 % (bke / 8)))) return gemm_invalid(__LINE__);
  if (!g.out_f32 && !g.out_op && !g.sol_coef) return gemm_invalid(__LINE__);
  if (g.stats && (g.geglu || g.Tout < 64 || (g.N & 15))) return gemm_invalid(__LINE__);
  if (g.rowstats && g.geglu) return gemm_invalid(__LINE__);
  if (g.ln_stats && (!g.ln_wsum || g.ln_dim <= 0 || (g.ln_dim & 127) || g.ln_dim > 512)) return gemm_invalid(__LINE__);
  if (g.rowstats && (g.N & 127)) return gemm_invalid(__LINE__);
  if ((g.out_f32 && (g.ldo_f32 & 3)) || (g.out_op && (g.ldo_op & 3)) || (g.res && (g.ldres & 3))) return gemm_invalid(__LINE__);
  if (g.lens && (g.rowstats || g.ln_stats || g.sol_coef || g.Tout < 1 || g.M != g.B * g.Tout)) return gemm_invalid(__LINE__);
  if (g.gnp_x) {
    const int cn = g.gnp_pair ? g.c0 >> 1 : g.c0;
    if (g.gnp_pair ? (prec == PREC_F32 || (g.c0 & 7) || (g.c1 && (g.a1 != g.a0 || g.c1 != cn || g.lda1 != g.lda0))) : g.c1 != 0) return gemm_invalid(__LINE__);
    if (g.ln_stats || g.tmode != TMODE_SAME || g.Tin != g.Tout || g.geglu || (g.N & 127) || g.c0 > 1024 || (cn & 3) || !g.gnp_stats || !g.gnp_gamma ||
        !g.gnp_beta || g.gnp_G < 1 || g.gnp_G > 8 || (cn % g.gnp_G) || ((cn / g.gnp_G) & 15) || g.Tin < 66 || (g.gnp_ldx & 3) || (g.lda0 & 3))
      return gemm_invalid(__LINE__);
    if (g.gnp_sync && ((reinterpret_cast<uintptr_t>(g.a0) & 127) || (((size_t)g.lda0 * operand_bytes(prec)) & 127) || (reinterpret_cast<uintptr_t>(g.gnp_sync) & 7)))
      return gemm_invalid(__LINE__);
    if (g.gnp_c1 && (g.gnp_c1 < 0 || g.gnp_c1 >= cn || (g.gnp_c1 & 15) || ((cn - g.gnp_c1) & 15) || !g.gnp_x1 || !g.gnp_stats1 || (g.gnp_ldx1 & 3)))
      return gemm_invalid(__LINE__);
  }
  {
    const unsigned long long sz = operand_bytes(prec), lim = 0xFFF00000ull;
    const unsigned long long rows = (unsigned long long)g.B * g.Tin;
    if (rows * g.lda0 * sz > lim || (g.c1 && rows * g.lda1 * sz > lim) || (g.c2 && rows * g.lda2 * sz > lim) ||
        (unsigned long long)g.N * g.K * sz > lim)
      return gemm_invalid(__LINE__);
  }
  {
    const bool forced_ks = g_force_bm == 128 && g_force_bn == 64 && (g_force_st == 64 || g_force_st == 68);
    const bool forced_ts = (g_force_bm == 128 && (g_force_st == 54 || g_force_st == 58)) || forced_ks;
    if (g.algo != 1 && (forced_ts || (g_ts && !g_force_bm)) && convts_eligible(g, prec))
      return launch_convts(g, prec, forced_ts ? g_force_bn : 0, forced_ts ? g_force_st % 10 : g_ts_nl, forced_ts ? (forced_ks ? 1 : 0) : g_ts_ks, s);
    if (forced_ts) return gemm_invalid(__LINE__);
  }
  if (g.sol_coef) return gemm_invalid(__LINE__);
  if (g.gnp_pair) return gemm_invalid(__LINE__);
  if (g.lens && g.gnp_x) return gemm_invalid(__LINE__);
  switch (prec) {
    case PREC_BF16: return launch_typed<bf16_t>(g, s);
    case PREC_F16: return launch_typed<f16_t>(g, s);
    case PREC_F32: return launch_typed<float>(g, s);
    default: return gemm_invalid(__LINE__);
  }
}

bool gemm_masks_rows(const GemmArgs& g_, int prec) {
  GemmArgs g = g_;
  if (g.rowstats || g.ln_stats || g.sol_coef || g.N % 64 != 0 || g.M <= 0 || g.Tout < 1 || g.M != g.B * g.Tout) return false;
  if (gemm_uses_convts(g, prec)) return true;
  if (g.gnp_x || g.gnp_pair) return false;
  static const int dummy = 0;
  g.lens = &dummy;
  hipError_t e;
  switch (prec) {
    case PREC_BF16: e = launch_typed<bf16_t>(g, nullptr, true); break;
    case PREC_F16: e = launch_typed<f16_t>(g, nullptr, true); break;
    case PREC_F32: e = launch_typed<float>(g, nullptr, true); break;
    default: return false;
  }
  g_gemm_fail_line = 0;
  return e == hipSuccess;
}

bool gemm_uses_convts(const GemmArgs& g, int prec) {
  const bool forced_ks = g_force_bm == 128 && g_force_bn == 64 && (g_force_st == 64 || g_force_st == 68);
  const bool forced_ts = (g_force_bm == 128 && (g_force_st == 54 || g_force_st == 58)) || forced_ks;
  return g.algo != 1 && (forced_ts || (g_ts && !g_force_bm)) && convts_eligible(g, prec);
}

template <typename K> static hipError_t set_lds(K kern, size_t bytes) {
  return hipFuncSetAttribute(reinterpret_cast<const void*>(kern), hipFuncAttributeMaxDynamicSharedMemorySize, (int)bytes);
}

#define NS2VC_SET(TM, BM, BN, ST)                                                                              \
// ... 37 lines not shown
```

ns2vc_amd/csrc/mma.h:

```cpp
#pragma once
#include "common.h"

namespace ns2vc {



template <typename T> struct MmaT;
template <> struct MmaT<float> {
  static constexpr int EPC = 4;
  __device__ static __forceinline__ void mma(f32x16_t& acc, const u32x4_t& a, const u32x4_t& b) {
    acc = __builtin_amdgcn_mfma_f32_32x32x2f32(__uint_as_float(a.x), __uint_as_float(b.x), acc, 0, 0, 0);
    acc = __builtin_amdgcn_mfma_f32_32x32x2f32(__uint_as_float(a.y), __uint_as_float(b.y), acc, 0, 0, 0);
    acc = __builtin_amdgcn_mfma_f32_32x32x2f32(__uint_as_float(a.z), __uint_as_float(b.z), acc, 0, 0, 0);
    acc = __builtin_amdgcn_mfma_f32_32x32x2f32(__uint_as_float(a.w), __uint_as_float(b.w), acc, 0, 0, 0);
  }
};
template <> struct MmaT<bf16_t> {
  static constexpr int EPC = 8;
  __device__ static __forceinline__ void mma(f32x16_t& acc, const u32x4_t& a, const u32x4_t& b) {
    union U { u32x4_t u; bf16x8_t v; };
    U ua, ub;
    ua.u = a; ub.u = b;
    acc = __builtin_amdgcn_mfma_f32_32x32x16_bf16(ua.v, ub.v, acc, 0, 0, 0);
  }
// ... 11 lines not shown

__device__ __forceinline__ void glds16(const void* gsrc, unsigned lds_dst) {
  unsigned keep;
  asm volatile("s_mov_b32 %0, m0\n\ts_mov_b32 m0, %2\n\ts_nop 0\n\tglobal_load_lds_dwordx4 %1, off\n\ts_mov_b32 m0, %0"
               : "=&s"(keep) : "v"(gsrc), "s"(lds_dst) : "memory");
}
typedef int i32x4_t __attribute__((ext_vector_type(4)));
constexpr unsigned DMA_OOB = 0xFFFFFFF0u;
__device__ __forceinline__ i32x4_t make_rsrc(const void* base, unsigned long long bytes) {
  const unsigned long long p = reinterpret_cast<unsigned long long>(base);
  i32x4_t r;
  r.x = __builtin_amdgcn_readfirstlane((int)(unsigned)p);
  r.y = __builtin_amdgcn_readfirstlane((int)(unsigned)(p >> 32));
  r.z = __builtin_amdgcn_readfirstlane((int)(unsigned)(bytes > 0xFFFFFFE0ull ? 0xFFFFFFE0ull : bytes));
  r.w = 0x00020000;
  return r;
}
__device__ __forceinline__ i32x4_t uniform_rsrc(const i32x4_t r) {
  i32x4_t u;
  u.x = __builtin_amdgcn_readfirstlane(r.x); u.y = __builtin_amdgcn_readfirstlane(r.y);
  u.z = __builtin_amdgcn_readfirstlane(r.z); u.w = __builtin_amdgcn_readfirstlane(r.w);
  return u;
}
__device__ __forceinline__ void blds16(const i32x4_t rsrc_, unsigned voff, unsigned soff_, unsigned lds_dst_) {
  const i32x4_t rsrc = uniform_rsrc(rsrc_);
  const unsigned soff = (unsigned)__builtin_amdgcn_readfirstlane((int)soff_);
  const unsigned lds_dst = (unsigned)__builtin_amdgcn_readfirstlane((int)lds_dst_);
  unsigned keep;
  asm volatile("s_mov_b32 %0, m0\n\ts_mov_b32 m0, %3\n\ts_nop 0\n\tbuffer_load_dwordx4 %1, %2, %4 offen lds\n\ts_mov_b32 m0, %0"
               : "=&s"(keep) : "v"(voff), "s"(rsrc), "s"(lds_dst), "s"(soff) : "memory");
}
template <int N> __device__ __forceinline__ void wait_vmcnt() { asm volatile("s_waitcnt vmcnt(%0)" ::"i"(N) : "memory"); }


}
```

ns2vc_amd/csrc/pack.cpp:

```cpp
#include "engine_internal.h"

#include <algorithm>
#include <cstring>

namespace ns2vc {

std::vector<BlockW> make_topology(const ns2vc_unet_cfg& c) {
  std::vector<BlockW> out;
  const int n = c.n_levels;
  int out_c = c.block_out_channels[0];
  for (int i = 0; i < n; ++i) {
    const int in_c = out_c;
    out_c = c.block_out_channels[i];
    BlockW b;
    b.kind = "down"; b.index = i; b.level = i; b.channels = out_c;
    const bool cross = (i != n - 1);
    for (int j = 0; j < c.layers_per_block; ++j) {
      ResnetW r;
      r.prefix = "down_blocks." + std::to_string(i) + ".resnets." + std::to_string(j);
      r.cin = j == 0 ? in_c : out_c; r.cout = out_c; r.shortcut = r.cin != r.cout;
      b.res.push_back(r);
      if (cross) {
        AttnW a;
        a.prefix = "down_blocks." + std::to_string(i) + ".attentions." + std::to_string(j);
// ... 95 lines not shown
  }
  expect(h, "conv_norm_out.weight", {c0}); expect(h, "conv_norm_out.bias", {c0});
  expect(h, "conv_out.weight", {c.latent_channels, c0, 3}); expect(h, "conv_out.bias", {c.latent_channels});
}

std::vector<float> rounded_rowsum(const float* rows, int N, int K, int Np, int prec) {
  std::vector<float> ws(Np, 0.f);
  for (int n = 0; n < N; ++n) {
    double acc = 0.0;
    for (int k = 0; k < K; ++k) {
      float v = rows[(size_t)n * K + k];
      if (prec != PREC_F32) v = op16_bits_to_f32(f32_to_op16_bits(v, prec), prec);
      acc += (double)v;
    }
    ws[n] = (float)acc;
  }
  return ws;
}

namespace {
struct Packer {
  ns2vc_unet* h;
  int err = 0;

  const HostTensor& T(const std::string& k) {
    auto it = h->raw.find(k);
    if (it == h->raw.end()) { err = fail("weight %s missing", k.c_str()); static HostTensor empty; return empty; }
    return it->second;
  }
  void* upload(const void* src, size_t bytes, const char* what = "weights") {
    void* d = nullptr;
    if (hipMalloc(&d, std::max<size_t>(bytes, 1)) != hipSuccess) { err = fail("hipMalloc failed (%s)", what); return nullptr; }
    h->weight_allocs.push_back(d);
    if (hipMemcpy(d, src, bytes, hipMemcpyHostToDevice) != hipSuccess) err = fail("hipMemcpy failed (weights)");
    return d;
  }
  float* upload_f32(const std::vector<float>& v) { return (float*)upload(v.data(), v.size() * sizeof(float)); }
  void* upload_u16(const std::vector<unsigned short>& v) { return upload(v.data(), v.size() * 2); }
  float* vec(const std::string& k) { return upload_f32(T(k).data); }
  int prec_override = -1;
  PackedW pack(const std::vector<float>& rows, int N, int K, const std::vector<float>& bias, bool want_wsum = false, int tile3_ctot = 0, int tile3_c2 = 0) {
    const int wprec = prec_override >= 0 ? prec_override : h->prec;
    PackedW p;
    const int Np = round_up(N, 128);
    p.N = Np; p.K = K;
    if (tile3_ctot > 0 && K == 3 * tile3_ctot + tile3_c2 && h->conv_ts && h->conv_wtiled) {
      std::vector<unsigned char> img;
      if (pack_conv3_tiled(rows.data(), N, tile3_ctot, tile3_c2, wprec, img) != hipSuccess) {
        if (!h->warned_wtiled) { fprintf(stderr, "ns2vc: tile-major conv weights unavailable for a %d x %d weight (channels not a multiple of the chunk): row-major fallback\n", N, K); h->warned_wtiled = true; }
      } else {
        p.wt = upload(img.data(), img.size(), "tile-major weights");
        if (!p.wt) return p;
      }
    }
    if (want_wsum) p.wsum = upload_f32(rounded_rowsum(rows.data(), N, K, Np, wprec));
    if (wprec != PREC_F32) {
      std::vector<uint16_t> q((size_t)Np * K, 0);
      for (size_t i = 0; i < (size_t)N * K; ++i) q[i] = f32_to_op16_bits(rows[i], wprec);
      p.w = upload(q.data(), q.size() * 2);
    } else {
      std::vector<float> q((size_t)Np * K, 0.f);
      memcpy(q.data(), rows.data(), (size_t)N * K * sizeof(float));
      p.w = upload(q.data(), q.size() * 4);
    }
    if (!p.w) return p;
    if (!bias.empty()) {
// ... 280 lines not shown
```

ns2vc_amd/csrc/plan.cpp:

```cpp
#include "engine_internal.h"

#include <algorithm>
#include <cmath>
#include <cstring>

namespace ns2vc {

int g_geglu_min_rows = 4608;

std::vector<int> level_lengths(int T, int n_levels) {
  std::vector<int> Ts(n_levels);
  Ts[0] = T;
  for (int l = 1; l < n_levels; ++l) Ts[l] = (Ts[l - 1] + 1) / 2;
  return Ts;
}

namespace {

struct Planner {
  ns2vc_unet* h;
  std::vector<Op>* ops;
  bool sizing = false;
  size_t off = 0;
  int B, T, Lp, G, prec;
// ... 37 lines not shown
    long long* p = stats_pool ? stats_pool + stats_used : reinterpret_cast<long long*>(sizeof(long long) * (stats_used + 1));
    stats_used += n;
    stats_of[tensor] = p;
    return p;
  }
  unsigned* new_sync(size_t nblocks) {
    nblocks = (nblocks + 1) & ~(size_t)1;
    stats_used = (stats_used + 1) & ~(size_t)1;
    if (stats_used + nblocks > stats_cap) return nullptr;
    long long* p = stats_pool ? stats_pool + stats_used : reinterpret_cast<long long*>(sizeof(long long) * (stats_used + 1));
    stats_used += nblocks;
    return reinterpret_cast<unsigned*>(p);
  }
  long long* find_stats(const float* tensor) const {
    auto it = stats_of.find(tensor);
    return it == stats_of.end() ? nullptr : it->second;
  }

  char* alloc_bytes(size_t bytes) {
    bytes = (bytes + 255) & ~(size_t)255;
    char* p = sizing ? nullptr : reinterpret_cast<char*>(h->arena) + off;
    off += bytes;
    return p;
  }
  template <typename Tp> Tp* alloc(size_t count) { return reinterpret_cast<Tp*>(alloc_bytes(count * sizeof(Tp))); }
  void* alloc_op(size_t count) { return alloc_bytes(count * opsz); }
  void* op_off(void* p, size_t elems) const { return p ? static_cast<void*>(static_cast<char*>(p) + elems * opsz) : nullptr; }

  void add(const std::string& name, std::function<hipError_t(hipStream_t)> fn, int kind = 0, double flops = 0.0, double bytes = 0.0) {
    if (sizing) return;
    Op op;
    op.name = name; op.fn = std::move(fn); op.kind = kind; op.flops = flops; op.bytes = bytes;
    ops->push_back(std::move(op));
  }
  void temb_reader() {
    if (sizing || ops != &h->fwd_ops) return;
    const int idx = (int)ops->size();
    if (h->tfork.first < 0) h->tfork.first = idx;
    if (h->tfork.join < 0 && h->tfork.readers >= h->tfork.join_skip) h->tfork.join = idx;
    ++h->tfork.readers;
  }
  void tap(const std::string& name, const float* src, int rows, int cols) {
    if (!h->debug) return;
    float* cp = alloc<float>((size_t)rows * cols);
    if (sizing) return;
    h->taps.push_back({name, cp, rows, cols});
    const size_t bytes = (size_t)rows * cols * sizeof(float);
    add("tap:" + name, [=](hipStream_t s) { return hipMemcpyAsync(cp, src, bytes, hipMemcpyDeviceToDevice, s); }, 4, 0.0, 2.0 * bytes);
  }

  void gemm(const std::string& name, GemmArgs g, int pr_override = -1) {
    const int pr = pr_override >= 0 ? pr_override : prec;
    const double osz = (double)opsz;
    const double nout = g.geglu ? g.N / 2 : g.N;
    const bool pair = g.c1 && g.a1 == g.a0 && g.c0 == 2 * g.c1 && g.c2 == 0;
    const double Kalg = pair ? g.K / 3.0 : (double)g.K, cin = pair ? g.c1 : g.c0 + g.c1 + g.c2, cgn = pair ? g.c1 : g.c0;
    const double flops = 2.0 * g.M * (double)g.N * Kalg;
    const double in_rows = (double)g.B * g.Tin;
    const double bytes = in_rows * cin * osz + (double)g.N * Kalg * osz + (g.out_f32 ? g.M * nout * 4.0 : 0.0) +
                         (g.out_op ? g.M * nout * osz : 0.0) + (g.res ? g.M * nout * 4.0 : 0.0);
    const double pro = g.gnp_x ? in_rows * cgn * (4.0 + osz * (g.gnp_raw ? 2.0 : 1.0)) : 0.0;
    if (g.taps == 3 && g.tmode == TMODE_SAME && !g.conv_bn) g.conv_bn = convts_bn_for(g, h->bn128_min);
    const bool self_mask = fused && ops == &h->fwd_ops && g.Tout > 1 && level_of(g.Tout) >= 0 && gemm_masks_rows(g, pr);
    if (self_mask) {
      g.lens = lens_of(g.Tout);
      if (g.gnp_x && g.algo == 0) g.algo = 2;
    } else if (masked && g.stats) { stats_of.erase(g.out_f32); g.stats = nullptr; }
    if (g.gnp_temb) temb_reader();
    add(g.gnp_x ? name + "[+norm]" : name, [=](hipStream_t s) { return launch_gemm(g, pr, s); }, 1, flops, bytes + pro);
    if (!sizing && g.gnp_x && g.gnp_sync) {
      unsigned* words = g.gnp_sync;
      const size_t nbytes = (((size_t)g.B * g.Tin + 63) / 64) * 8;
      ops->back().rearm = [=](hipStream_t s) { return launch_zero(words, (nbytes + 15) & ~(size_t)15, s); };
    }
    if (g.Tout > 1 && !self_mask) {
      const int nc = g.geglu ? g.N / 2 : g.N;
      mask(name, g.out_f32, g.ldo_f32, nc, 4, g.Tout);
      mask(name, g.out_op, g.ldo_op, nc, operand_bytes(pr), g.Tout);
    }
  }
  GemmArgs base(const void* a0, int lda0, int c0, int Tin, int Tout, const PackedW& w, float* out_f32, void* out_op, int ldo) {
    GemmArgs g;
    memset(&g, 0, sizeof(g));
    g.a0 = a0; g.lda0 = lda0; g.c0 = c0;
    g.B = B; g.Tin = Tin; g.Tout = Tout; g.M = B * Tout;
    g.taps = 1; g.tmode = TMODE_SAME;
    g.w = w.w; g.K = w.K; g.N = w.N; g.bias = w.bias;
    g.w_tiled = h->conv_wtiled ? w.wt : nullptr;
    g.out_f32 = out_f32; g.ldo_f32 = ldo;
    g.out_op = out_op; g.ldo_op = ldo;
    g.algo = h->conv_ts ? (h->gn_inloop ? 0 : 2) : 1;
    return g;
  }
  struct GnPro { const float* x = nullptr; int ldx = 0; const long long* st = nullptr; const float* gamma = nullptr; const float* beta = nullptr;
                 const float* temb = nullptr; int ldtemb = 0; float eps = 0.f; int G = 0, silu = 0; unsigned* sync = nullptr; unsigned* alone = nullptr;
                 const float* x1 = nullptr; int ldx1 = 0, c1 = 0; const long long* st1 = nullptr; void* raw = nullptr; };
  static void gn_fuse(GemmArgs& g, const GnPro& p) {
    if (!p.x) return;
    g.gnp_x = p.x; g.gnp_ldx = p.ldx; g.gnp_stats = p.st; g.gnp_gamma = p.gamma; g.gnp_beta = p.beta;
    g.gnp_temb = p.temb; g.gnp_ldtemb = p.ldtemb; g.gnp_eps = p.eps; g.gnp_G = p.G; g.gnp_silu = p.silu;
    g.gnp_sync = p.sync; g.gnp_alone = p.alone;
    g.gnp_x1 = p.x1; g.gnp_ldx1 = p.ldx1; g.gnp_c1 = p.c1; g.gnp_stats1 = p.st1; g.gnp_raw = p.raw;
// ... 61 lines not shown
    g.stats = new_stats(h1, Tl, r.cout);
    gemm(r.prefix + ".conv1", g);
    const GnPro p2 = groupnorm(r.prefix + ".norm2", h1, r.cout, r.cout, nullptr, 0, 0, Tl, 1e-5f, r.n2g, r.n2b, h->temb, r.temb_off, r.cout, 1, hn,
                               nullptr, r.conv2.N, 3);
    GemmArgs g2 = base(hn, r.cout, r.cout, Tl, Tl, r.conv2, out, out_op, r.cout);
    g2.taps = 3;
    gn_fuse(g2, p2);
    if (r.shortcut) {
      g2.a2 = xr; g2.lda2 = cin; g2.c2 = cin;
    } else {
      g2.res = a0; g2.ldres = lda0;
    }
    g2.stats = new_stats(out, Tl, r.cout);
    gemm(r.prefix + ".conv2", g2);
  }

  void attention(const std::string& name, const void* q, int ldq, const void* k, int ldk, const void* v, int ldv, int Lq, int Lk,
                 const float* bias, int hd, void* out, int ldo, bool self = false) {
    AttnArgs a;
    memset(&a, 0, sizeof(a));
    a.q = q; a.k = k; a.v = v; a.ldq = ldq; a.ldk = ldk; a.ldv = ldv;
    a.B = B; a.H = h->cfg.heads; a.Lq = Lq; a.Lk = Lk; a.bias = bias;
    a.scale = 1.0f / std::sqrt((float)hd);
    a.out = out; a.ldo = ldo;
    a.pv_fp8 = (h->attn_fp8 && prec != PREC_F32) ? 1 : 0;
    a.exact_only = h->attn_optimistic ? 0 : 1;
    a.fallbacks = h->attn_fallbacks;
    const int pr = prec;
    const bool self_mask = masked && h->masked_attn && ops == &h->fwd_ops && level_of(Lq) >= 0 && attention_masks_rows(a, hd, pr);
    if (self_mask) {
      a.q_lens = lens_of(Lq);
      if (self) a.k_lens = lens_of(Lk);
    } else if (self) a.bias = selfbias_of(Lk);
    add(name, [=](hipStream_t s) { return launch_attention(a, hd, pr, s); }, 2, 4.0 * B * a.H * (double)Lq * Lk * hd,
        (double)opsz * B * a.H * hd * (2.0 * Lq + 2.0 * Lk));
    if (!self_mask) mask(name, out, ldo, a.H * hd, opsz, Lq);
  }

  std::map<std::string, void*> xattn_vt;
  bool xattn_fused(const AttnW& a, int Tl) const {
    const int d = a.dim;
    const bool lin = h->ln_linear && (d % 128 == 0) && d <= 512 && !masked;
    return h->fuse_xattn && lin && h->fold_ff && h->fuse_ffn && a.ffn_stream && ffn_eligible(d, Tl, prec) && h->fuse_ffn_pre && a.ffn_pre_stream &&
           h->cfg.heads == 8 && (d == 128 || d == 256);
  }
  void transformer(const AttnW& a, const float* x, int Tl, float* y, void* yn, void* qkv, void* ao, void* qb, void* ffh, float* out,
                   void* out_op) {
    const int d = a.dim, M = B * Tl, hd = d / h->cfg.heads, pr = prec;
    const std::string t = a.prefix + ".transformer_blocks.0";
    GemmArgs g;
    auto layernorm = [&](const std::string& nm) {
      add(nm, [=](hipStream_t s) { return launch_ln_apply_op(y, d, M, d, 1e-5f, yn, pr, s); }, 3, 8.0 * M * d, (4.0 + opsz) * M * d);
    };
    const bool lin_dense = h->ln_linear && (d % 128 == 0) && d <= 512;
    const bool lin = lin_dense && !masked;
    const bool lens_rows = masked && h->masked_rows && ops == &h->fwd_ops && level_of(Tl) >= 0;
    auto consume = [&](GemmArgs& gg, float* rs, const PackedW& w) {
      if (rs) { gg.ln_stats = rs; gg.ln_wsum = w.wsum; gg.ln_eps = 1e-5f; gg.ln_dim = d; gg.ln_health = h->ln_health; }
    };
    float* r1 = lin ? rs1 : nullptr;
    auto rowchain = [&](const std::string& nm, const void* a_op, const long long* gn_st, void* stream, const float* bias1, const float* consts2,
                        const float* res, void* z_op, int n2) {
      ns2vc_rowchain_args c;
      memset(&c, 0, sizeof(c));
      c.a_op = a_op; c.lda = d; c.wstream = stream; c.bias1 = bias1; c.consts2 = consts2;
      c.res = res; c.ldres = d; c.out1_f32 = y; c.ldo1 = d; c.out2_op = z_op; c.ldo2 = n2;
      c.ln_eps = 1e-5f; c.M = M; c.dim = d; c.n2 = n2; c.ln_health = h->ln_health;
      if (gn_st) {
        c.a_op = nullptr; c.gn_x = x; c.ldx = d; c.gn_stats = gn_st; c.gn_gamma = a.ng; c.gn_beta = a.nb; c.gn_eps = 1e-6f; c.T = Tl; c.G = G;
      }
      if (!res && stream == a.chain_in && a.chain_in_s2 && h->slice_rows && 2 * ((M + 63) / 64) <= h->cus + 8) { c.wstream = a.chain_in_s2; c.slices = 2; }
      if (lens_rows) { c.lens = lens_of(Tl); c.T = Tl; }
      add(c.slices == 2 ? nm + "[2 slices]" : nm, [=](hipStream_t s) { return launch_rowchain(c, pr, s); }, 1, 2.0 * M * (double)d * (d + n2),
          (double)M * (d * ((gn_st ? 4.0 : opsz) + 4.0 + (res ? 4.0 : 0.0)) + n2 * opsz) + (double)(d + n2) * d * opsz);
    };
    auto chains_mask_rows = [&]() {
      ns2vc_rowchain_args c;
      memset(&c, 0, sizeof(c));
      c.M = M; c.dim = d; c.T = Tl;
      c.n2 = 3 * d;
      const bool in_ok = rowchain_masks_rows(c, pr);
      c.n2 = d;
      return in_ok && rowchain_masks_rows(c, pr);
    };
    const bool rows_ok = (masked ? lin_dense && lens_rows && chains_mask_rows() : lin) && h->fuse_rows && a.chain_in && a.chain_mid &&
                         rowchain_eligible(d, d, Tl, pr);
    const long long* xst = (rows_ok && h->fuse_rows_gn && Tl >= 64 && (d % G) == 0 && ((d / G) % 16) == 0) ? find_stats(x) : nullptr;
    GnPro pn;
    if (!xst) pn = groupnorm(a.prefix + ".norm", x, d, d, nullptr, 0, 0, Tl, 1e-6f, a.ng, a.nb, nullptr, 0, 0, 0, xn, nullptr, rows_ok ? 0 : a.proj_in.N);
    if (rows_ok) {
      rowchain(a.prefix + (xst ? ".rows[norm+proj_in+qkv]" : ".rows[proj_in+qkv]"), xn, xst, a.chain_in, a.proj_in.bias, a.chain_in_consts, nullptr, qkv,
               3 * d);
    } else {
      g = base(xn, d, d, Tl, Tl, a.proj_in, y, r1 ? yn : nullptr, d);
      gn_fuse(g, pn);
      g.rowstats = r1;
      gemm(a.prefix + ".proj_in", g);
      if (!r1) layernorm(t + ".norm1");
      g = base(yn, d, d, Tl, Tl, a.qkv, nullptr, qkv, 3 * d);
      consume(g, r1, a.qkv);
      gemm(t + ".attn1.qkv", g);
    }
    attention(t + ".attn1.sdpa", qkv, 3 * d, op_off(qkv, d), 3 * d, op_off(qkv, 2 * d), 3 * d, Tl, Tl, nullptr, hd, ao, d, true);
    float* r2 = lin ? rs2 : nullptr;
    if (rows_ok) {
      rowchain(t + ".rows[attn1.to_out+attn2.to_q]", ao, nullptr, a.chain_mid, a.o1.bias, a.chain_mid_consts, y, qb, d);
    } else {
// ... 20 lines not shown
      f.B = B; f.T = Tl; f.M = M; f.dim = d;
      return ffn_masks_rows(f, pr);
    };
    const bool lens_ffn = masked && h->masked_ffn && ops == &h->fwd_ops && level_of(Tl) >= 0 && lin_dense && fold && h->fuse_ffn && a.ffn_stream &&
                          h->fuse_ffn_pre && a.ffn_pre_stream && ffn_eligible(d, Tl, pr) && ffn_masks();
    const bool ffn_ok = lens_ffn || (fold && r3 && h->fuse_ffn && a.ffn_stream && ffn_eligible(d, Tl, pr));
    const bool ffn_pre = ffn_ok && h->fuse_ffn_pre && a.ffn_pre_stream;
    if (!ffn_pre) {
      g = base(ao, d, d, Tl, Tl, a.o2, y, yraw, d);
      g.res = y; g.ldres = d;
      g.rowstats = r3;
      gemm(t + ".attn2.to_out", g);
    }
    if (ffn_ok) {
      ns2vc_ffn_args f;
      memset(&f, 0, sizeof(f));
      f.yn = yn; f.ldy = d; f.ln_stats = r3; f.ln_eps = 1e-5f;
      f.wstream = a.ffn_stream; f.consts = a.ffn_consts; f.bias2 = a.ffpo.bias;
      if (ffn_pre) {
        f.yn = nullptr; f.ln_stats = nullptr; f.wstream = a.ffn_pre_stream;
        f.pre_a = ao; f.pre_lda = d; f.pre_bias = a.o2.bias; f.pre_res = y; f.pre_ldres = d;
      }
      if (xatt) {
        f.pre_a = nullptr;
        f.att_q = qb; f.att_ldq = d; f.att_kv = xattn_vt[a.prefix];
        f.att_bias = h->has_mask ? h->maskbias : nullptr; f.att_scale = 1.0f / std::sqrt((float)hd); f.att_Lk = Lp;
      }
      f.res = x; f.ldres = d;
      f.out_f32 = out; f.ldo_f32 = d; f.out_op = out_op; f.ldo_op = d;
      f.stats = new_stats(out, Tl, d);
      f.B = B; f.T = Tl; f.M = M; f.dim = d; f.ln_health = h->ln_health;
      if (lens_ffn) f.lens = lens_of(Tl);
      const double fl = 2.0 * M * (double)d * ((ffn_pre ? 14.0 : 13.0) * d) + (xatt ? 4.0 * B * h->cfg.heads * (double)Tl * Lp * hd : 0.0);
      add(a.prefix + (xatt ? ".ffn[attn2.sdpa+to_out+geglu+ff.out+proj_out]" : ffn_pre ? ".ffn[attn2.to_out+geglu+ff.out+proj_out]" : ".ffn[geglu+ff.out+proj_out]"),
          [=](hipStream_t s) { return launch_ffn(f, pr, s); }, 1, fl,
          (double)M * d * (opsz + 8.0 + (ffn_pre ? 4.0 : 0.0) + (out_op ? opsz : 0.0)) + (ffn_pre ? 14.0 : 13.0) * d * d * opsz +
              (xatt ? (double)opsz * B * d * 2.0 * Lp : 0.0));
      return;
    }
    auto geglu_masks = [&]() {
      ns2vc_geglu_args f;
      memset(&f, 0, sizeof(f));
      f.M = M; f.dim = d; f.T = Tl;
      return geglu_masks_rows(f, pr);
    };
    const bool lens_geglu = masked && h->masked_geglu && ops == &h->fwd_ops && level_of(Tl) >= 0 && lin_dense && fold && h->fuse_geglu &&
                            a.geglu_stream && geglu_eligible(d, Tl, pr) && M >= g_geglu_min_rows && geglu_masks();
    if (!r3 && !lens_geglu) layernorm(t + ".norm3");
    if (lens_geglu || (r3 && h->fuse_geglu && a.geglu_stream && geglu_eligible(d, Tl, pr) && M >= g_geglu_min_rows)) {
      ns2vc_geglu_args f;
      memset(&f, 0, sizeof(f));
      f.yn = yn; f.ldy = d; f.ln_stats = r3; f.ln_eps = 1e-5f;
      if (lens_geglu) { f.yn = qb; f.ln_stats = nullptr; f.T = Tl; f.lens = lens_of(Tl); }
      f.wstream = a.geglu_stream; f.consts = a.geglu_consts;
      f.out_op = ffh; f.ldo = 4 * d; f.M = M; f.dim = d; f.ln_health = h->ln_health;
      add(t + ".ff.geglu[token-stationary]", [=](hipStream_t s) { return launch_geglu(f, pr, s); }, 1, 2.0 * M * (double)d * 8.0 * d,
          (double)M * d * opsz * 5.0 + (double)M * (d / 64) * 8.0 + 8.0 * d * d * opsz);
    } else {
      g = base(yn, d, d, Tl, Tl, a.ff1, nullptr, ffh, 4 * d);
      g.geglu = 1;
      consume(g, r3, a.ff1);
      gemm(t + ".ff.geglu", g);
    }
    if (fold) {
      g = base(ffh, 4 * d, 4 * d, Tl, Tl, a.ffpo, out, out_op, d);
      g.a2 = yraw; g.lda2 = d; g.c2 = d;
      g.res = x; g.ldres = d;
      g.stats = new_stats(out, Tl, d);
      gemm(a.prefix + ".ff.out+proj_out", g);
    } else {
      g = base(ffh, 4 * d, 4 * d, Tl, Tl, a.ff2, nullptr, yn, d);
      g.res = y; g.ldres = d;
      gemm(t + ".ff.out", g);
      g = base(yn, d, d, Tl, Tl, a.proj_out, out, out_op, d);
      g.res = x; g.ldres = d;
      g.stats = new_stats(out, Tl, d);
      gemm(a.prefix + ".proj_out", g);
    }
  }
};
}

int build_plan(ns2vc_unet* h, bool sizing) {
  const auto& c = h->cfg;
  const int B = h->B, T = h->T, Lp = h->Lp, nl = c.n_levels;
  const int c0 = c.block_out_channels[0], E = 4 * c0, cross = c.cross_attention_dim, CP = h->CP;
  const std::vector<int> Ts = level_lengths(T, nl);

  Planner P;
  P.h = h; P.sizing = sizing; P.B = B; P.T = T; P.Lp = Lp; P.G = c.norm_num_groups; P.prec = h->prec;
// ... 226 lines not shown
        P.tap(tag + ".us", us, B * Ts[l - 1], b.channels);
        cur = us;
      }
    }
  }
  if (!skips.empty()) return fail("internal: %zu skips left over", skips.size());
  {
    const bool po = pio && 2 * curC <= 3 * c0 && h->conv_outp.w;
    const auto pno = P.groupnorm("conv_norm_out", cur, curC, curC, nullptr, 0, 0, T, 1e-5f, h->out_ng, h->out_nb, nullptr, 0, 0, 1, P.xn, nullptr, h->conv_out.N, 3, po ? 1 : 0);
    const bool xo = xio && pno.x != nullptr && (size_t)curC * 4 <= (size_t)3 * c0 * P.opsz;
    GemmArgs g = po ? P.base(P.xn, 2 * curC, 2 * curC, T, T, h->conv_outp, h->x0, nullptr, CP)
                    : P.base(P.xn, curC, curC, T, T, xo ? h->conv_out32 : h->conv_out, h->x0, nullptr, CP);
    if (po) { g.a1 = P.xn; g.lda1 = 2 * curC; g.c1 = curC; g.gnp_pair = pno.x ? 1 : 0; }
    g.taps = 3;
    P.gn_fuse(g, pno);
    if (h->conv_out.N != CP) return fail("internal: conv_out padded width %d != %d", h->conv_out.N, CP);
    const int conv_out_at = (int)h->fwd_ops.size();
    P.gemm("conv_out", g, xo ? PREC_F32 : -1);
    if (!sizing) { h->conv_out_g = g; h->conv_out_idx = conv_out_at; h->conv_out_prec = xo ? PREC_F32 : prec; }
    P.tap("out", h->x0, B * T, CP);
  }
  if (sizing) { h->lens.off = P.off; P.off += lens_bytes; }
  else if (P.off > h->lens.off) {
    h->cond_ops.clear(); h->fwd_ops.clear(); h->taps.clear();
    return fail("internal: plan needs %zu bytes in front of the length tables at %zu (re-run ns2vc_unet_prepare)", P.off, h->lens.off);
  } else P.off = h->lens.off + lens_bytes;
  if (sizing) h->arena_bytes = P.off;
  else if (P.off > h->arena_bytes) {
    h->cond_ops.clear(); h->fwd_ops.clear(); h->taps.clear();
    return fail("internal: plan needs %zu bytes but the arena holds %zu (re-run ns2vc_unet_prepare)", P.off, h->arena_bytes);
  }
  h->arena_used = P.off;
  h->stats_bytes = std::max<size_t>(P.stats_used, 1) * sizeof(long long);
  h->tfork.ok = !sizing && h->tfork.begin > 0 && h->tfork.end > h->tfork.begin && h->tfork.join >= h->tfork.end && h->tfork.first >= h->tfork.join;
  if (!sizing && h->fork_temb && !h->tfork.ok)
    fprintf(stderr, "ns2vc: fork_temb refused for this plan (join at launch %d, first reader of the time scale / shift rows at %d): the step graph stays linear\n",
            h->tfork.join, h->tfork.first);
  return 0;
}

bool temb_forks(const ns2vc_unet* h, size_t last) {
  return h->fork_temb && !h->debug && h->tfork.ok && (size_t)h->tfork.join <= last;
}

int run_ops(const std::vector<Op>& ops, hipStream_t s, size_t first, size_t last) {
  for (size_t i = first; i < std::min(last, ops.size()); ++i) {
    hipError_t e = ops[i].fn(s);
    if (e != hipSuccess) {
      const int line = last_gemm_refusal_line();
      if (line) return fail("launch of '%s' failed: %s (refused by the argument check at gemm.hip:%d)", ops[i].name.c_str(), hipGetErrorString(e), line);
      return fail("launch of '%s' failed: %s", ops[i].name.c_str(), hipGetErrorString(e));
    }
  }
  return 0;
}

void drop_step_graph(ns2vc_unet* h) {
  if (h->step_graph) { (void)hipGraphExecDestroy(h->step_graph); h->step_graph = nullptr; }
}
void drop_plan(ns2vc_unet* h) {
  drop_step_graph(h);
  if (h->arena) { (void)hipDeviceSynchronize(); (void)hipFree(h->arena); h->arena = nullptr; }
  h->cond_ops.clear(); h->fwd_ops.clear(); h->taps.clear();
  h->arena_bytes = h->arena_used = 0;
  h->next_step = -1;
  h->ln_out.posted = false;
  h->attn_fallbacks = nullptr;
  h->tfork.ok = false;
  h->ln_health = nullptr;
}

// ... 2 lines not shown
```

ns2vc_amd/csrc/rowchain.hip:

```cpp
#include "common.h"
#include "mma.h"
#include <cstdlib>
#include <vector>

namespace ns2vc {

typedef ::ns2vc_rowchain_args RowchainArgs;

__device__ unsigned long long* g_rc_trace = nullptr;
#ifndef NS2VC_GEMM_TRACE
#define NS2VC_GEMM_TRACE 0
#endif
#ifndef NS2VC_RC_ABLATE
#define NS2VC_RC_ABLATE 0
#endif
#ifndef NS2VC_RC_WT
#define NS2VC_RC_WT 1
#endif
#if NS2VC_GEMM_TRACE
#define RC_TR(i) do { if (tr && tid == 0) tr[i] = __builtin_readcyclecounter(); } while (0)
#else
#define RC_TR(i) do { (void)tr; } while (0)
#endif
void set_rc_trace(unsigned long long* p) { (void)hipMemcpyToSymbol(HIP_SYMBOL(g_rc_trace), &p, sizeof(p)); }

constexpr int RC_TILE = 128 * 128;
constexpr int RC_PAIR = 2 * RC_TILE;

template <int D, int R2, int NT> struct RowchainGeom {
  static constexpr int TOK = 64 * NT;
  static constexpr int KT = D / 64;
  static constexpr int NB1 = D / 128;
  static constexpr int S1 = KT * NB1, S2 = KT * R2;
  static_assert(S1 % 2 == 0 && S2 % 2 == 0, "stages start on pair boundaries");
  static constexpr int NP = (S1 + S2) / 2;
  static constexpr int RING = 3;
  static constexpr int PTILE = TOK * 128;
  static constexpr int PANEL = KT * PTILE;
  static constexpr int CONSTS = R2 * 128 * 8;
  static constexpr int STATS = TOK * 4 * 8;
  static constexpr int LDS = RING * RC_PAIR + PANEL + CONSTS + STATS;
  static_assert(LDS <= 160 * 1024, "LDS budget");
};

template <typename TM, int D, int R2, int NT, bool MASKED = false>
__global__ __launch_bounds__(512) void rowchain_kernel(const RowchainArgs a) {
  op_mode_init<TM>();
  using G = RowchainGeom<D, R2, NT>;
  constexpr int KT = G::KT, NB1 = G::NB1, S1 = G::S1, S2 = G::S2, NP = G::NP, RING = G::RING, TOK = G::TOK, PTILE = G::PTILE;
  extern __shared__ __attribute__((aligned(16))) char smem[];
  char* const ring = smem;
  char* const panel = smem + RING * RC_PAIR;
  const float* const consts = reinterpret_cast<const float*>(panel + G::PANEL);
  float2* const stats = reinterpret_cast<float2*>(panel + G::PANEL + G::CONSTS);
  int* const liveflag = reinterpret_cast<int*>(smem + G::LDS);

  const int tid = threadIdx.x, lane = tid & 63;
  const int wave = __builtin_amdgcn_readfirstlane(tid >> 6);
  unsigned long long* const tr = (NS2VC_GEMM_TRACE && g_rc_trace) ? g_rc_trace + (size_t)blockIdx.x * 8 : nullptr;
  RC_TR(0);
  const int tw = wave & 1, cg = wave >> 1;
  const int l31 = lane & 31, hi = lane >> 5;
  const int sw = (l31 >> 1) & 7;
  const unsigned lds0 = (unsigned)(size_t)smem;
  const int S = a.slices > 1 ? a.slices : 1;
  const int sl = S > 1 ? (int)(blockIdx.x % (8 * S)) / 8 : 0;
  const int blk = S > 1 ? (int)(blockIdx.x / (8 * S)) * 8 + (int)(blockIdx.x & 7) : (int)blockIdx.x;
  const int m0 = blk * TOK;
  if (m0 >= a.M) return;
  const int tok0 = 32 * NT * tw + l31;
  int tlen[NT], tfr[NT];
  if constexpr (MASKED) {
    const int nitem = a.M / a.T;
#pragma unroll
    for (int u = 0; u < NT; ++u) {
      const int m = min(m0 + tok0 + 32 * u, a.M - 1), b = min(m / a.T, nitem - 1);
      tfr[u] = m - b * a.T;
      tlen[u] = a.lens[b];
    }
// ... 350 lines not shown
static void rc_append_tile(std::vector<unsigned short>& out, const float* mat, size_t ld, int row0, int col0, int prec) {
  for (int r = 0; r < 128; ++r)
    for (int pos = 0; pos < 8; ++pos) {
      const int lc = pos ^ ((r >> 1) & 7);
      for (int e = 0; e < 8; ++e) out.push_back(f32_to_op16_bits(mat[(size_t)(row0 + r) * ld + col0 + lc * 8 + e], prec));
    }
}

int rowchain_slice_blocks(int n2, int slices) { return (n2 / 128 + slices - 1) / slices; }

hipError_t pack_rowchain_stream(const float* w1, const float* w2, int dim, int n2, int prec, std::vector<unsigned short>& out, int slices) {
  if (!rowchain_eligible(dim, n2, 64, prec) || slices < 1 || (slices > 1 && dim != 384)) return hipErrorInvalidValue;
  const int KT = dim / 64, nb2 = n2 / 128, r2s = rowchain_slice_blocks(n2, slices);
  out.clear();
  out.reserve((size_t)slices * (dim + r2s * 128) * dim);
  std::vector<float> zero((size_t)128 * dim, 0.f);
  for (int sl = 0; sl < slices; ++sl) {
    for (int kt = 0; kt < KT; ++kt)
      for (int rb = 0; rb < dim / 128; ++rb) rc_append_tile(out, w1, dim, 128 * rb, 64 * kt, prec);
    for (int kt = 0; kt < KT; ++kt)
      for (int j = 0; j < r2s; ++j) {
        const int rb = sl * r2s + j;
        if (rb < nb2) rc_append_tile(out, w2, dim, 128 * rb, 64 * kt, prec);
        else rc_append_tile(out, zero.data(), dim, 0, 64 * kt, prec);
      }
  }
  return hipSuccess;
}

bool rowchain_eligible(int dim, int n2, int T, int prec) {
  return (dim == 128 || dim == 256 || dim == 384) && (n2 == dim || n2 == 3 * dim) && T >= 1 && (prec == PREC_BF16 || prec == PREC_F16);
}

template <typename TM, int D, int R2, int NT, bool MASKED> static hipError_t launch_rc(const RowchainArgs& a, hipStream_t s) {
  constexpr int TOK = RowchainGeom<D, R2, NT>::TOK;
  const size_t lds = RowchainGeom<D, R2, NT>::LDS + (MASKED ? TOK * 4 : 0);
  static_assert(RowchainGeom<D, R2, NT>::LDS + TOK * 4 <= 160 * 1024, "LDS budget of the masked form");
  const int nblk = (a.M + TOK - 1) / TOK, S = a.slices > 1 ? a.slices : 1;
  hipLaunchKernelGGL((rowchain_kernel<TM, D, R2, NT, MASKED>), dim3(S > 1 ? ((nblk + 7) / 8) * 8 * S : nblk), dim3(512), lds, s, a);
  return hipGetLastError();
}
static int g_force_nt = 0;
void set_forced_rowchain_tokens(int nt) { g_force_nt = nt; }
template <typename TM, bool MK> static hipError_t launch_rc_tm(const RowchainArgs& a, hipStream_t s) {
  if (a.dim == 128) {
    const bool big = g_force_nt ? g_force_nt == 2 : (a.M + 63) / 64 > 256;
    if (big) return a.n2 == 128 ? launch_rc<TM, 128, 1, 2, MK>(a, s) : launch_rc<TM, 128, 3, 2, MK>(a, s);
    return a.n2 == 128 ? launch_rc<TM, 128, 1, 1, MK>(a, s) : launch_rc<TM, 128, 3, 1, MK>(a, s);
  }
  if (a.dim == 384 && a.slices == 2) return a.n2 == 384 ? launch_rc<TM, 384, 2, 1, MK>(a, s) : launch_rc<TM, 384, 5, 1, MK>(a, s);
  if (a.dim == 384) return a.n2 == 384 ? launch_rc<TM, 384, 3, 1, MK>(a, s) : launch_rc<TM, 384, 9, 1, MK>(a, s);
  return a.n2 == 256 ? launch_rc<TM, 256, 2, 1, MK>(a, s) : launch_rc<TM, 256, 6, 1, MK>(a, s);
}

bool rowchain_masks_rows(const RowchainArgs& a, int prec) {
  if (!rowchain_eligible(a.dim, a.n2, 64, prec) || a.M <= 0 || a.T < 1 || (a.M % a.T)) return false;
  return !a.gn_x || a.T >= 64;
}

hipError_t launch_rowchain(const RowchainArgs& a, int prec, hipStream_t s) {
  if (!rowchain_eligible(a.dim, a.n2, 64, prec) || a.M <= 0) return hipErrorInvalidValue;
  if (a.slices > 1 && (a.slices != 2 || a.dim != 384 || (a.res && (const void*)a.res == (const void*)a.out1_f32))) return hipErrorInvalidValue;
  if ((!a.a_op && !a.gn_x) || !a.wstream || !a.bias1 || !a.consts2 || !a.out2_op) return hipErrorInvalidValue;
  if (a.gn_x) {
    if (!a.gn_stats || !a.gn_gamma || !a.gn_beta || a.G < 1 || a.G > 8 || a.T < 64 || (a.dim % a.G) || ((a.dim / a.G) & 15) || (a.ldx & 3))
      return hipErrorInvalidValue;
  } else if (a.lda & 7) return hipErrorInvalidValue;
  if ( (a.res && (a.ldres & 3)) || (a.out1_f32 && (a.ldo1 & 3)) || (a.ldo2 & 7)) return hipErrorInvalidValue;
  if ((unsigned long long)a.M * a.lda * 2ull > 0xFFF00000ull) return hipErrorInvalidValue;
  if (a.lens) {
    if (!rowchain_masks_rows(a, prec)) return hipErrorInvalidValue;
    return prec == PREC_BF16 ? launch_rc_tm<bf16_t, true>(a, s) : launch_rc_tm<f16_t, true>(a, s);
  }
  return prec == PREC_BF16 ? launch_rc_tm<bf16_t, false>(a, s) : launch_rc_tm<f16_t, false>(a, s);
}

hipError_t init_rowchain_attributes() {
  hipError_t e;
#define NS2VC_RC_ATTR1(TM, DD_, RR_, NT_, MK_)                                                                                      \
  if ((e = hipFuncSetAttribute(reinterpret_cast<const void*>(rowchain_kernel<TM, DD_, RR_, NT_, MK_>), hipFuncAttributeMaxDynamicSharedMemorySize, \
                               (int)RowchainGeom<DD_, RR_, NT_>::LDS + ((MK_) ? RowchainGeom<DD_, RR_, NT_>::TOK * 4 : 0))) != hipSuccess) return e
#define NS2VC_RC_ATTR(TM, DD_, RR_, NT_) NS2VC_RC_ATTR1(TM, DD_, RR_, NT_, false); NS2VC_RC_ATTR1(TM, DD_, RR_, NT_, true)
  NS2VC_RC_ATTR(bf16_t, 128, 1, 1); NS2VC_RC_ATTR(bf16_t, 128, 3, 1); NS2VC_RC_ATTR(bf16_t, 256, 2, 1); NS2VC_RC_ATTR(bf16_t, 256, 6, 1);
  NS2VC_RC_ATTR(f16_t, 128, 1, 1); NS2VC_RC_ATTR(f16_t, 128, 3, 1); NS2VC_RC_ATTR(f16_t, 256, 2, 1); NS2VC_RC_ATTR(f16_t, 256, 6, 1);
  NS2VC_RC_ATTR(bf16_t, 128, 1, 2); NS2VC_RC_ATTR(bf16_t, 128, 3, 2); NS2VC_RC_ATTR(f16_t, 128, 1, 2); NS2VC_RC_ATTR(f16_t, 128, 3, 2);
  NS2VC_RC_ATTR(bf16_t, 384, 3, 1); NS2VC_RC_ATTR(bf16_t, 384, 9, 1); NS2VC_RC_ATTR(f16_t, 384, 3, 1); NS2VC_RC_ATTR(f16_t, 384, 9, 1);
  NS2VC_RC_ATTR(bf16_t, 384, 2, 1); NS2VC_RC_ATTR(bf16_t, 384, 5, 1); NS2VC_RC_ATTR(f16_t, 384, 2, 1); NS2VC_RC_ATTR(f16_t, 384, 5, 1);
#undef NS2VC_RC_ATTR
#undef NS2VC_RC_ATTR1
  return hipSuccess;
}

}
```

ns2vc_amd/engine.py:

```python
from __future__ import annotations

import ctypes as C
from typing import Dict, Iterable, List, Optional, Tuple

import numpy as np

from . import _lib
from ._lib import Ns2vcError, PREC_BF16, PREC_F16, PREC_F32, check
from .schedule import NCOEF, SolverTable, build_table
from .spec import UNetConfig, engine_block_types, engine_supports, param_spec

PRECISIONS = {"fp32": PREC_F32, "f32": PREC_F32, "bf16": PREC_BF16, "fp16": PREC_F16, "f16": PREC_F16}
DEFAULT_PRECISION = "fp16"


class DevBuf:

    def __init__(self, nbytes: int):
        self.lib = _lib.load()
        p = C.c_void_p()
        check(self.lib.ns2vc_dev_malloc(C.byref(p), nbytes), "ns2vc_dev_malloc")
        self.ptr = p.value
        self.nbytes = nbytes

# ... 304 lines not shown

    def sample_end(self, x_out, stream=None) -> None:
        check(self.lib.ns2vc_sampler_end(self.h, _ptr(x_out), _stream_ptr(stream)), "sampler_end")

    def attn_fallbacks(self, reset: bool = True, stream=None) -> int:
        n = C.c_ulonglong()
        check(self.lib.ns2vc_unet_attn_fallbacks(self.h, C.byref(n), int(reset), _stream_ptr(stream)), "attn_fallbacks")
        return int(n.value)

    def gn_coop_alone(self, reset: bool = True, stream=None) -> int:
        n = C.c_ulonglong()
        check(self.lib.ns2vc_unet_gn_coop_alone(self.h, C.byref(n), int(reset), _stream_ptr(stream)), "gn_coop_alone")
        return int(n.value)

    def op_info(self, which: int = 0) -> List[Tuple[str, int, float, float]]:
        nf, nc = self.launches()
        out = []
        name = C.create_string_buffer(256)
        kind, fl, by = C.c_int(), C.c_double(), C.c_double()
        for i in range(nc if which else nf):
            check(self.lib.ns2vc_unet_op_info(self.h, which, i, name, 256, C.byref(kind), C.byref(fl), C.byref(by)), "op_info")
            out.append((name.value.decode(), int(kind.value), float(fl.value), float(by.value)))
        return out

    def temb_fork(self) -> Dict[str, int]:
        out = {}
        name = C.create_string_buffer(32)
        v, fl, by = C.c_int(), C.c_double(), C.c_double()
        for i in range(6):
            check(self.lib.ns2vc_unet_op_info(self.h, 2, i, name, 32, C.byref(v), C.byref(fl), C.byref(by)), "op_info(2)")
            out[name.value.decode()] = int(v.value)
        return out

    def profile_forward(self, reps: int = 5, stream=None) -> np.ndarray:
        nf, _ = self.launches()
        ms = (C.c_float * nf)()
        check(self.lib.ns2vc_unet_profile_forward(self.h, ms, nf, int(reps), _stream_ptr(stream)), "profile_forward")
        return np.array(list(ms), dtype=np.float64)

    def taps(self) -> Dict[str, np.ndarray]:
        out: Dict[str, np.ndarray] = {}
        n = self.lib.ns2vc_unet_num_taps(self.h)
        name = C.create_string_buffer(256)
        rows, cols = C.c_int(), C.c_int()
        for i in range(n):
            check(self.lib.ns2vc_unet_tap_info(self.h, i, name, 256, C.byref(rows), C.byref(cols)), "tap_info")
            a = np.empty((rows.value, cols.value), dtype=np.float32)
            check(self.lib.ns2vc_unet_tap_read(self.h, i, a.ctypes.data), "tap_read")
            out[name.value.decode()] = a
        return out

    def close(self) -> None:
        if getattr(self, "h", None):
            self.lib.ns2vc_unet_destroy(self.h)
            self.h = None

    def __del__(self):
        try:
            self.close()
        except Exception:
            pass


def sync() -> None:
    check(_lib.load().ns2vc_dev_sync(), "dev_sync")
```

Measured before the change: 284.0 denoiser-steps/s (batch 32 per GPU, whole job).

## Append idle-CU prefetch blocks to kernels to warm next op's weights in L2

Adds extra workgroups to attention, conv, rowchain and other kernels. They fill CUs left idle in the last wave and prefetch the next op's weight bytes into cache through pf_block. The host computes each op's main grid, picks a block count from the leftover CUs, and points each op's prefetch at the following op's weights. This aims to hide the cold weight-fetch latency at kernel starts in the graph-captured loop, at the cost of extra blocks and possible cache pollution or contention.

```diff
diff --git a/ns2vc_amd/csrc/attn.hip b/ns2vc_amd/csrc/attn.hip
--- a/ns2vc_amd/csrc/attn.hip
+++ b/ns2vc_amd/csrc/attn.hip
@@ -90,7 +90,8 @@
 __device__ int g_attn_exact_only = 0;
 __device__ __forceinline__ int vpos8(int key) { return ((key & 4) << 3) | ((key & 32) >> 1) | ((key & 24) >> 1) | (key & 3); }
 template <typename TM, int HD, int KEYS, bool P8, bool MASKED = false>
-__global__ __launch_bounds__(256) void attn_kernel(const AttnArgs a) {
+__global__ __launch_bounds__(256) void attn_kernel(const AttnArgs a, const PfArgs pf) {
+  pf_block(pf);
   op_mode_init<TM>();
   static_assert(!P8 || (sizeof(TM) == 2 && KEYS == 64), "the fp8 PV path: 16-bit operand types, one 64-key tile per f8f6f4 MFMA");
   constexpr int NSUB = KEYS / 32;
@@ -116,7 +117,7 @@
   const int nqb = (a.Lq + 127) >> 7;
   int b, h, qb;
   {
-    const int nwg = gridDim.x, bid = blockIdx.x;
+    const int nwg = (int)gridDim.x - pf.count, bid = blockIdx.x;
     const int qn = nwg >> 3, rn = nwg & 7, xcd = bid & 7, idx = bid >> 3;
     const int swz = (xcd < rn ? xcd * (qn + 1) : rn * (qn + 1) + (xcd - rn) * qn) + idx;
     b = swz / (a.H * nqb);
@@ -415,35 +416,39 @@
 void set_forced_attn_keys(int keys) { g_force_keys = keys; }
 void set_attn_optimistic(int on) { const int v = on ? 0 : 1; (void)hipMemcpyToSymbol(HIP_SYMBOL(g_attn_exact_only), &v, sizeof(v)); }
 
-template <typename TM, int HD, int KEYS> static hipError_t launch_hdk(const AttnArgs& a, hipStream_t s) {
-  dim3 grid(((a.Lq + 127) / 128) * a.H * a.B);
+template <typename TM, int HD, int KEYS> static hipError_t launch_hdk(const AttnArgs& a, hipStream_t s, const PfArgs& pf_, int* main_grid) {
+  const int nb = ((a.Lq + 127) / 128) * a.H * a.B;
+  if (main_grid) { *main_grid = nb; return hipSuccess; }
+  const PfArgs pf = pf_.first == nb ? pf_ : PfArgs();
+  dim3 grid(nb + pf.count);
   const size_t lds = attn_lds<TM, HD, KEYS>();
-  if (a.q_lens || a.k_lens) hipLaunchKernelGGL((attn_kernel<TM, HD, KEYS, false, true>), grid, dim3(256), lds, s, a);
-  else hipLaunchKernelGGL((attn_kernel<TM, HD, KEYS, false>), grid, dim3(256), lds, s, a);
+  if (a.q_lens || a.k_lens) hipLaunchKernelGGL((attn_kernel<TM, HD, KEYS, false, true>), grid, dim3(256), lds, s, a, pf);
+  else hipLaunchKernelGGL((attn_kernel<TM, HD, KEYS, false>), grid, dim3(256), lds, s, a, pf);
   return hipGetLastError();
 }
-template <typename TM, int HD> static hipError_t launch_hd(const AttnArgs& a, hipStream_t s) {
+template <typename TM, int HD> static hipError_t launch_hd(const AttnArgs& a, hipStream_t s, const PfArgs& pf, int* main_grid) {
   if (a.pv_fp8 && (a.q_lens || a.k_lens)) return hipErrorInvalidValue;
   if constexpr (sizeof(TM) == 2) {
     if (a.pv_fp8) {
+      if (main_grid) { *main_grid = 0; return hipSuccess; }
       dim3 grid(((a.Lq + 127) / 128) * a.H * a.B);
       const size_t lds = attn_lds<TM, HD, 64>();
-      hipLaunchKernelGGL((attn_kernel<TM, HD, 64, true>), grid, dim3(256), lds, s, a);
+      hipLaunchKernelGGL((attn_kernel<TM, HD, 64, true>), grid, dim3(256), lds, s, a, PfArgs());
       return hipGetLastError();
     }
   } else if (a.pv_fp8) return hipErrorInvalidValue;
   if constexpr (attn_has128<TM, HD>()) {
-    if (g_force_keys == 128) return launch_hdk<TM, HD, 128>(a, s);
-  }
-  return launch_hdk<TM, HD, 64>(a, s);
-}
-
-template <typename TM> static hipError_t launch_tm(const AttnArgs& a, int hd, hipStream_t s) {
+    if (g_force_keys == 128) return launch_hdk<TM, HD, 128>(a, s, pf, main_grid);
+  }
+  return launch_hdk<TM, HD, 64>(a, s, pf, main_grid);
+}
+
+template <typename TM> static hipError_t launch_tm(const AttnArgs& a, int hd, hipStream_t s, const PfArgs& pf, int* main_grid) {
   switch (hd) {
-    case 16: return launch_hd<TM, 16>(a, s);
-    case 32: return launch_hd<TM, 32>(a, s);
-    case 48: return launch_hd<TM, 48>(a, s);
-    case 64: return launch_hd<TM, 64>(a, s);
+    case 16: return launch_hd<TM, 16>(a, s, pf, main_grid);
+    case 32: return launch_hd<TM, 32>(a, s, pf, main_grid);
+    case 48: return launch_hd<TM, 48>(a, s, pf, main_grid);
+    case 64: return launch_hd<TM, 64>(a, s, pf, main_grid);
     default: return hipErrorInvalidValue;
   }
 }
@@ -489,16 +494,16 @@
   return prec == PREC_BF16 || prec == PREC_F16 || prec == PREC_F32;
 }
 
-hipError_t launch_attention(const AttnArgs& a, int head_dim, int prec, hipStream_t s) {
+hipError_t launch_attention(const AttnArgs& a, int head_dim, int prec, hipStream_t s, const PfArgs& pf, int* main_grid) {
   const int al = prec == PREC_F32 ? 3 : 7;
   if (!a.q || !a.k || !a.v || !a.out) return hipErrorInvalidValue;
   if ((a.q_lens || a.k_lens) && !attention_masks_rows(a, head_dim, prec)) return hipErrorInvalidValue;
   if (a.Lq <= 0 || a.Lk <= 0 || (a.ldq & al) || (a.ldk & al) || (a.ldv & al) || (a.ldo & al)) return hipErrorInvalidValue;
   if (reinterpret_cast<uintptr_t>(a.out) & 15) return hipErrorInvalidValue;
   switch (prec) {
-    case PREC_BF16: return launch_tm<bf16_t>(a, head_dim, s);
-    case PREC_F16: return launch_tm<f16_t>(a, head_dim, s);
-    case PREC_F32: return launch_tm<float>(a, head_dim, s);
+    case PREC_BF16: return launch_tm<bf16_t>(a, head_dim, s, pf, main_grid);
+    case PREC_F16: return launch_tm<f16_t>(a, head_dim, s, pf, main_grid);
+    case PREC_F32: return launch_tm<float>(a, head_dim, s, pf, main_grid);
     default: return hipErrorInvalidValue;
   }
 }
diff --git a/ns2vc_amd/csrc/common.h b/ns2vc_amd/csrc/common.h
--- a/ns2vc_amd/csrc/common.h
+++ b/ns2vc_amd/csrc/common.h
@@ -4,6 +4,7 @@
 #include <stddef.h>
 #include <vector>
 #include "../../include/ns2vc_hip.h"
+#include "prefetch.h"
 
 namespace ns2vc {
 
@@ -242,13 +243,13 @@
 constexpr double GN_SUM_SCALE = 268435456.0;
 constexpr double GN_SQ_SCALE = 65536.0;
 
-hipError_t launch_gemm(const GemmArgs& g, int prec, hipStream_t s);
+hipError_t launch_gemm(const GemmArgs& g, int prec, hipStream_t s, const PfArgs& pf = PfArgs(), int* main_grid = nullptr);
 size_t xattn_pack_bytes(int B, int Lk, int hd);
 hipError_t launch_xattn_pack(const void* k, int ldk, const void* v, int ldv, int B, int Lk, int hd, void* out, int prec, hipStream_t s);
 bool gemm_masks_rows(const GemmArgs& g, int prec);
 bool gemm_uses_convts(const GemmArgs& g, int prec);
 int last_gemm_refusal_line();
-hipError_t launch_attention(const AttnArgs& a, int head_dim, int prec, hipStream_t s);
+hipError_t launch_attention(const AttnArgs& a, int head_dim, int prec, hipStream_t s, const PfArgs& pf = PfArgs(), int* main_grid = nullptr);
 bool attention_masks_rows(const AttnArgs& a, int head_dim, int prec);
 hipError_t init_gemm_attributes();
 bool convts_eligible(const GemmArgs& g, int prec);
@@ -256,14 +257,14 @@
 int convts_bn_for(const GemmArgs& g, int bn128_min);
 void set_convts_bn128_min(int wgs);
 int convts_row_blocks(const GemmArgs& g);
-hipError_t launch_convts(const GemmArgs& g, int prec, int bn, int nl, int ks, hipStream_t s);
+hipError_t launch_convts(const GemmArgs& g, int prec, int bn, int nl, int ks, hipStream_t s, const PfArgs& pf = PfArgs(), int* main_grid = nullptr);
 hipError_t init_convts_attributes();
 hipError_t pack_conv3_tiled(const float* rows, int N, int ctot, int c2, int prec, std::vector<unsigned char>& out);
 void set_forced_gemm_tile(int bm, int bn, int stages);
 void set_gemm_trace(unsigned long long* p);
 hipError_t init_attn_attributes();
 void set_forced_attn_keys(int keys);
-hipError_t launch_ffn(const ::ns2vc_ffn_args& a, int prec, hipStream_t s);
+hipError_t launch_ffn(const ::ns2vc_ffn_args& a, int prec, hipStream_t s, const PfArgs& pf = PfArgs(), int* main_grid = nullptr);
 bool ffn_eligible(int dim, int T, int prec);
 bool ffn_masks_rows(const ::ns2vc_ffn_args& a, int prec);
 hipError_t init_ffn_attributes();
@@ -271,7 +272,7 @@
 void set_ffn_trace(unsigned long long* p);
 bool geglu_eligible(int dim, int T, int prec);
 hipError_t pack_geglu_stream(const float* w1p, const float* bias1p, int dim, int prec, std::vector<unsigned short>& stream, std::vector<float>& consts);
-hipError_t launch_geglu(const ::ns2vc_geglu_args& a, int prec, hipStream_t s);
+hipError_t launch_geglu(const ::ns2vc_geglu_args& a, int prec, hipStream_t s, const PfArgs& pf = PfArgs(), int* main_grid = nullptr);
 bool geglu_masks_rows(const ::ns2vc_geglu_args& a, int prec);
 hipError_t init_geglu_attributes();
 void set_gg_trace(unsigned long long* p);
@@ -292,7 +293,7 @@
 hipError_t launch_time_embed(const float* t_ptr, int t_stride, const int* step_ptr, int coef_stride,
                              const float* w1t, const float* b1, const float* w2t, const float* b2,
                              const float* aug, float* emb, void* emb_act_op, int prec, int B, int tdim, int edim, hipStream_t s);
-hipError_t launch_rowchain(const ::ns2vc_rowchain_args& a, int prec, hipStream_t s);
+hipError_t launch_rowchain(const ::ns2vc_rowchain_args& a, int prec, hipStream_t s, const PfArgs& pf = PfArgs(), int* main_grid = nullptr);
 bool rowchain_eligible(int dim, int n2, int T, int prec);
 bool rowchain_masks_rows(const ::ns2vc_rowchain_args& a, int prec);
 hipError_t init_rowchain_attributes();
diff --git a/ns2vc_amd/csrc/convts.hip b/ns2vc_amd/csrc/convts.hip
--- a/ns2vc_amd/csrc/convts.hip
+++ b/ns2vc_amd/csrc/convts.hip
@@ -65,7 +65,8 @@
 
 enum { TS_GN_NONE = 0, TS_GN_PRO = 1, TS_GN_INLOOP = 2, TS_GN_PAIR = 3, TS_MASKED = 4 };
 template <typename TM, int BN, int NL, int GNPF, bool KS = false, bool SOL = false>
-__global__ __launch_bounds__(64 * (NL + 4)) void conv3ts_kernel(const GemmArgs g) {
+__global__ __launch_bounds__(64 * (NL + 4)) void conv3ts_kernel(const GemmArgs g, const PfArgs pf) {
+  pf_block(pf);
   constexpr int GNP = GNPF & 3;
   constexpr bool MASKED = (GNPF & TS_MASKED) != 0;
   op_mode_init<TM>();
@@ -572,53 +573,56 @@
 int convts_default_bn(const GemmArgs& g) { return (g.conv_bn == 64 || (g.conv_bn == 128 && g.N % 128 == 0)) ? g.conv_bn : convts_bn_for(g, g_bn128_min); }
 int convts_row_blocks(const GemmArgs& g) { return (int)(((long long)g.B * (g.Tin + 1) + TS_BMO - 1) / TS_BMO); }
 
-template <typename TM, int BN, int NL, bool KS> static hipError_t launch_ts_cfg(const GemmArgs& g, hipStream_t s) {
+template <typename TM, int BN, int NL, bool KS> static hipError_t launch_ts_cfg(const GemmArgs& g, hipStream_t s, const PfArgs& pf_, int* main_grid) {
   const int nbm = convts_row_blocks(g), nbn = g.N / BN;
   int nb = nbm * nbn;
   if (g.gnp_x && g.gnp_sync && nbn > 1) nb = 8 * ((nbm + 7) / 8) * nbn;
+  if (main_grid) { *main_grid = nb; return hipSuccess; }
+  const PfArgs pf = pf_.first == nb ? pf_ : PfArgs();
+  nb += pf.count;
   constexpr bool HAS_INLOOP = NS2VC_TS_CHUNK && NL == 8 && !KS;
   if (g.lens) {
     constexpr bool HAS_MASKED = NL == 8 && !KS;
     if constexpr (HAS_MASKED) {
       if (g.sol_coef) return hipErrorInvalidValue;
       if (g.gnp_x && g.gnp_pair) {
-        if constexpr (!std::is_same<TM, float>::value) hipLaunchKernelGGL((conv3ts_kernel<TM, BN, NL, TS_GN_PAIR | TS_MASKED, KS>), dim3(nb), dim3(64 * (NL + 4)), ts_lds_bytes(BN), s, g);
+        if constexpr (!std::is_same<TM, float>::value) hipLaunchKernelGGL((conv3ts_kernel<TM, BN, NL, TS_GN_PAIR | TS_MASKED, KS>), dim3(nb), dim3(64 * (NL + 4)), ts_lds_bytes(BN), s, g, pf);
         else return hipErrorInvalidValue;
       }
-      else if (g.gnp_x) hipLaunchKernelGGL((conv3ts_kernel<TM, BN, NL, TS_GN_PRO | TS_MASKED, KS>), dim3(nb), dim3(64 * (NL + 4)), ts_lds_bytes(BN), s, g);
-      else hipLaunchKernelGGL((conv3ts_kernel<TM, BN, NL, TS_GN_NONE | TS_MASKED, KS>), dim3(nb), dim3(64 * (NL + 4)), ts_lds_bytes(BN), s, g);
+      else if (g.gnp_x) hipLaunchKernelGGL((conv3ts_kernel<TM, BN, NL, TS_GN_PRO | TS_MASKED, KS>), dim3(nb), dim3(64 * (NL + 4)), ts_lds_bytes(BN), s, g, pf);
+      else hipLaunchKernelGGL((conv3ts_kernel<TM, BN, NL, TS_GN_NONE | TS_MASKED, KS>), dim3(nb), dim3(64 * (NL + 4)), ts_lds_bytes(BN), s, g, pf);
     } else return hipErrorInvalidValue;
   }
   else if (g.sol_coef) {
     constexpr bool HAS_SOL = BN == 128 && NL == 8 && !KS;
     if constexpr (HAS_SOL) {
       if (g.gnp_x && g.gnp_pair) {
-        if constexpr (!std::is_same<TM, float>::value) hipLaunchKernelGGL((conv3ts_kernel<TM, BN, NL, 3, KS, true>), dim3(nb), dim3(64 * (NL + 4)), ts_lds_bytes(BN), s, g);
+        if constexpr (!std::is_same<TM, float>::value) hipLaunchKernelGGL((conv3ts_kernel<TM, BN, NL, 3, KS, true>), dim3(nb), dim3(64 * (NL + 4)), ts_lds_bytes(BN), s, g, pf);
         else return hipErrorInvalidValue;
       }
-      else if (g.gnp_x) hipLaunchKernelGGL((conv3ts_kernel<TM, BN, NL, 1, KS, true>), dim3(nb), dim3(64 * (NL + 4)), ts_lds_bytes(BN), s, g);
-      else hipLaunchKernelGGL((conv3ts_kernel<TM, BN, NL, 0, KS, true>), dim3(nb), dim3(64 * (NL + 4)), ts_lds_bytes(BN), s, g);
+      else if (g.gnp_x) hipLaunchKernelGGL((conv3ts_kernel<TM, BN, NL, 1, KS, true>), dim3(nb), dim3(64 * (NL + 4)), ts_lds_bytes(BN), s, g, pf);
+      else hipLaunchKernelGGL((conv3ts_kernel<TM, BN, NL, 0, KS, true>), dim3(nb), dim3(64 * (NL + 4)), ts_lds_bytes(BN), s, g, pf);
     } else return hipErrorInvalidValue;
   }
   else if (g.gnp_x && g.gnp_pair) {
-    if constexpr (!std::is_same<TM, float>::value && NL == 8 && !KS) hipLaunchKernelGGL((conv3ts_kernel<TM, BN, NL, 3, KS>), dim3(nb), dim3(64 * (NL + 4)), ts_lds_bytes(BN), s, g);
+    if constexpr (!std::is_same<TM, float>::value && NL == 8 && !KS) hipLaunchKernelGGL((conv3ts_kernel<TM, BN, NL, 3, KS>), dim3(nb), dim3(64 * (NL + 4)), ts_lds_bytes(BN), s, g, pf);
     else return hipErrorInvalidValue;
   }
   else if (g.gnp_x && HAS_INLOOP && g.algo != 2) {
-    if constexpr (HAS_INLOOP) hipLaunchKernelGGL((conv3ts_kernel<TM, BN, NL, 2, KS>), dim3(nb), dim3(64 * (NL + 4)), ts_lds_bytes(BN), s, g);
-  }
-  else if (g.gnp_x) hipLaunchKernelGGL((conv3ts_kernel<TM, BN, NL, 1, KS>), dim3(nb), dim3(64 * (NL + 4)), ts_lds_bytes(BN), s, g);
-  else hipLaunchKernelGGL((conv3ts_kernel<TM, BN, NL, 0, KS>), dim3(nb), dim3(64 * (NL + 4)), ts_lds_bytes(BN), s, g);
+    if constexpr (HAS_INLOOP) hipLaunchKernelGGL((conv3ts_kernel<TM, BN, NL, 2, KS>), dim3(nb), dim3(64 * (NL + 4)), ts_lds_bytes(BN), s, g, pf);
+  }
+  else if (g.gnp_x) hipLaunchKernelGGL((conv3ts_kernel<TM, BN, NL, 1, KS>), dim3(nb), dim3(64 * (NL + 4)), ts_lds_bytes(BN), s, g, pf);
+  else hipLaunchKernelGGL((conv3ts_kernel<TM, BN, NL, 0, KS>), dim3(nb), dim3(64 * (NL + 4)), ts_lds_bytes(BN), s, g, pf);
   return hipGetLastError();
 }
-template <typename TM> static hipError_t launch_ts_typed(const GemmArgs& g, int bn, int nl, int ks, hipStream_t s) {
-  if (bn == 64 && nl == 4) return ks ? launch_ts_cfg<TM, 64, 4, true>(g, s) : launch_ts_cfg<TM, 64, 4, false>(g, s);
-  if (bn == 64 && nl == 8) return ks ? launch_ts_cfg<TM, 64, 8, true>(g, s) : launch_ts_cfg<TM, 64, 8, false>(g, s);
-  if (bn == 128 && nl == 4) return launch_ts_cfg<TM, 128, 4, false>(g, s);
-  if (bn == 128 && nl == 8) return launch_ts_cfg<TM, 128, 8, false>(g, s);
+template <typename TM> static hipError_t launch_ts_typed(const GemmArgs& g, int bn, int nl, int ks, hipStream_t s, const PfArgs& pf, int* main_grid) {
+  if (bn == 64 && nl == 4) return ks ? launch_ts_cfg<TM, 64, 4, true>(g, s, pf, main_grid) : launch_ts_cfg<TM, 64, 4, false>(g, s, pf, main_grid);
+  if (bn == 64 && nl == 8) return ks ? launch_ts_cfg<TM, 64, 8, true>(g, s, pf, main_grid) : launch_ts_cfg<TM, 64, 8, false>(g, s, pf, main_grid);
+  if (bn == 128 && nl == 4) return launch_ts_cfg<TM, 128, 4, false>(g, s, pf, main_grid);
+  if (bn == 128 && nl == 8) return launch_ts_cfg<TM, 128, 8, false>(g, s, pf, main_grid);
   return hipErrorInvalidValue;
 }
-hipError_t launch_convts(const GemmArgs& g, int prec, int bn, int nl, int ks, hipStream_t s) {
+hipError_t launch_convts(const GemmArgs& g, int prec, int bn, int nl, int ks, hipStream_t s, const PfArgs& pf, int* main_grid) {
   if (!convts_eligible(g, prec)) return hipErrorInvalidValue;
   if (!bn) bn = convts_default_bn(g);
   if (!nl) nl = NS2VC_TS_NL_DEFAULT;
@@ -627,9 +631,9 @@
   if (g.lens) { nl = 8; ks = 0; }
   if (g.N % bn) return hipErrorInvalidValue;
   switch (prec) {
-    case PREC_BF16: return launch_ts_typed<bf16_t>(g, bn, nl, ks, s);
-    case PREC_F16: return launch_ts_typed<f16_t>(g, bn, nl, ks, s);
-    case PREC_F32: return launch_ts_typed<float>(g, bn, nl, ks, s);
+    case PREC_BF16: return launch_ts_typed<bf16_t>(g, bn, nl, ks, s, pf, main_grid);
+    case PREC_F16: return launch_ts_typed<f16_t>(g, bn, nl, ks, s, pf, main_grid);
+    case PREC_F32: return launch_ts_typed<float>(g, bn, nl, ks, s, pf, main_grid);
     default: return hipErrorInvalidValue;
   }
 }
diff --git a/ns2vc_amd/csrc/engine.cpp b/ns2vc_amd/csrc/engine.cpp
--- a/ns2vc_amd/csrc/engine.cpp
+++ b/ns2vc_amd/csrc/engine.cpp
@@ -42,7 +42,8 @@
   {"fork_temb", "NS2VC_FORK_TEMB", &ns2vc_unet::fork_temb}, {"exact_io", "NS2VC_EXACT_IO", &ns2vc_unet::exact_io},
   {"split_io", "NS2VC_SPLIT_IO", &ns2vc_unet::split_io}, {"masked_fuse", "NS2VC_MASKED_FUSE", &ns2vc_unet::masked_fuse},
   {"masked_attn", "NS2VC_MASKED_ATTN", &ns2vc_unet::masked_attn}, {"masked_rows", "NS2VC_MASKED_ROWS", &ns2vc_unet::masked_rows},
-  {"masked_ffn", "NS2VC_MASKED_FFN", &ns2vc_unet::masked_ffn}, {"masked_geglu", "NS2VC_MASKED_GEGLU", &ns2vc_unet::masked_geglu}};
+  {"masked_ffn", "NS2VC_MASKED_FFN", &ns2vc_unet::masked_ffn}, {"masked_geglu", "NS2VC_MASKED_GEGLU", &ns2vc_unet::masked_geglu},
+  {"prefetch_next", "NS2VC_PREFETCH_NEXT", &ns2vc_unet::prefetch_next}};
 static bool* option_ptr(ns2vc_unet* h, const char* name) {
   for (const auto& o : kOptions)
     if (!strcmp(name, o.name)) return &(h->*o.member);
@@ -413,6 +414,21 @@
     *kind = v[idx]; *flops = 0.0; *bytes = 0.0;
     return 0;
   }
+  if (which == 3 || which == 4) {
+    if (idx < 0 || idx >= (int)h->fwd_ops.size()) return fail("op index out of range");
+    const Op& op = h->fwd_ops[idx];
+    if (which == 4) {
+      snprintf(name, buflen, "%s", op.name.c_str());
+      *kind = op.pf ? op.pf->count : 0; *flops = 0.0; *bytes = (double)op.weight_bytes;
+      return 0;
+    }
+    const bool on = op.pf && op.pf_for >= 0 && op.pf->count > 0;
+    snprintf(name, buflen, "%s", on ? h->fwd_ops[op.pf_for].name.c_str() : "");
+    *kind = on ? op.pf_for : -1;
+    *bytes = on ? (double)op.pf->bytes : 0.0;
+    *flops = on ? (double)(static_cast<const char*>(op.pf->p) - static_cast<const char*>(h->fwd_ops[op.pf_for].weights)) : 0.0;
+    return 0;
+  }
   const std::vector<Op>& ops = which ? h->cond_ops : h->fwd_ops;
   if (idx < 0 || idx >= (int)ops.size()) return fail("op index out of range");
   snprintf(name, buflen, "%s", ops[idx].name.c_str());
diff --git a/ns2vc_amd/csrc/engine_internal.h b/ns2vc_amd/csrc/engine_internal.h
--- a/ns2vc_amd/csrc/engine_internal.h
+++ b/ns2vc_amd/csrc/engine_internal.h
@@ -5,6 +5,7 @@
 #include <cstdio>
 #include <functional>
 #include <map>
+#include <memory>
 #include <string>
 #include <vector>
 
@@ -81,6 +82,13 @@
   double flops = 0.0;
   double bytes = 0.0;
   std::function<hipError_t(hipStream_t)> rearm;
+  const void* weights = nullptr;
+  size_t weight_bytes = 0;
+  std::function<int()> main_grid;
+  std::shared_ptr<PfArgs> pf;
+  int pf_for = -1;
+  int pf_family = 0;
+  int pf_fixed = 0;
 };
 struct Tap {
   std::string name;
@@ -125,6 +133,7 @@
   int prec = -1;
   bool finalized = false;
   std::vector<void*> weight_allocs;
+  std::map<const void*, size_t> weight_alloc_bytes;
 
   std::vector<ns2vc::BlockW> blocks;
   ns2vc::PackedW conv_in_x, conv_in_c, conv_out, temb_all, kv_all, pool_qkv;
@@ -192,6 +201,7 @@
   bool masked_rows = false;
   bool masked_ffn = false;
   bool masked_geglu = false;
+  bool prefetch_next = true;
   struct Lengths {
     bool masked = false;
     int* dev = nullptr;
@@ -266,6 +276,7 @@
 extern int g_geglu_min_rows;
 std::vector<int> level_lengths(int T, int n_levels);
 int build_plan(ns2vc_unet* h, bool sizing);
+void assign_prefetch(ns2vc_unet* h);
 int run_ops(const std::vector<Op>& ops, hipStream_t s, size_t first = 0, size_t last = (size_t)-1);
 bool temb_forks(const ns2vc_unet* h, size_t last);
 void drop_step_graph(ns2vc_unet* h);
diff --git a/ns2vc_amd/csrc/ffn.hip b/ns2vc_amd/csrc/ffn.hip
--- a/ns2vc_amd/csrc/ffn.hip
+++ b/ns2vc_amd/csrc/ffn.hip
@@ -15,7 +15,7 @@
 #define NS2VC_FFN_FENCE 1
 #endif
 #ifndef NS2VC_FFN_WARM
-#define NS2VC_FFN_WARM 1
+#define NS2VC_FFN_WARM 0
 #endif
 #if NS2VC_FFN_FENCE == 1
 #define FFN_FRAG_FENCE() do { asm volatile("s_waitcnt lgkmcnt(0)" ::: "memory"); __builtin_amdgcn_sched_barrier(0); } while (0)
@@ -65,7 +65,8 @@
 };
 
 template <typename TM, int D, bool PRE, bool ATT = false, bool MASKED = false>
-__global__ __launch_bounds__(512) void ffn_kernel(const FfnArgs a) {
+__global__ __launch_bounds__(512) void ffn_kernel(const FfnArgs a, const PfArgs pf) {
+  pf_block(pf);
   op_mode_init<TM>();
   static_assert(!ATT || PRE, "the in-kernel cross-attention feeds the pre-stage");
   static_assert(!(ATT && MASKED), "the in-kernel cross-attention has no masked form");
@@ -238,7 +239,7 @@
   }
 #if NS2VC_FFN_WARM
   {
-    const unsigned nx = (gridDim.x + 7) >> 3, jx = blockIdx.x >> 3;
+    const unsigned nx = (gridDim.x - (unsigned)pf.count + 7) >> 3, jx = blockIdx.x >> 3;
     const unsigned total = (unsigned)NP * FFN_PAIR;
     const unsigned per = (((total + nx - 1) / nx) + 8191u) & ~8191u;
     for (unsigned off = jx * per + wave * 1024; off < min(total, (jx + 1) * per); off += 8192)
@@ -636,20 +637,24 @@
 
 bool ffn_eligible(int dim, int T, int prec) { return (dim == 128 || dim == 256) && T >= 64 && (prec == PREC_BF16 || prec == PREC_F16); }
 
-template <typename TM, int D> static hipError_t launch_ffn_t(const FfnArgs& a, hipStream_t s) {
+template <typename TM, int D> static hipError_t launch_ffn_t(const FfnArgs& a, hipStream_t s, const PfArgs& pf_, int* main_grid) {
+  const int nbm = a.att_q && !a.lens ? a.B * ((a.T + 63) / 64) : (a.M + 63) / 64;
+  if (main_grid) { *main_grid = nbm; return hipSuccess; }
+  const PfArgs pf = pf_.first == nbm ? pf_ : PfArgs();
+  const int nb = nbm + pf.count;
   if (a.lens) {
     const size_t lds = a.pre_a ? FfnGeom<D, true>::LDS : FfnGeom<D, false>::LDS;
-    if (a.pre_a) hipLaunchKernelGGL((ffn_kernel<TM, D, true, false, true>), dim3((a.M + 63) / 64), dim3(512), lds, s, a);
-    else hipLaunchKernelGGL((ffn_kernel<TM, D, false, false, true>), dim3((a.M + 63) / 64), dim3(512), lds, s, a);
+    if (a.pre_a) hipLaunchKernelGGL((ffn_kernel<TM, D, true, false, true>), dim3(nb), dim3(512), lds, s, a, pf);
+    else hipLaunchKernelGGL((ffn_kernel<TM, D, false, false, true>), dim3(nb), dim3(512), lds, s, a, pf);
   } else if (a.att_q) {
     const size_t lds = FfnGeom<D, true>::LDS;
-    hipLaunchKernelGGL((ffn_kernel<TM, D, true, true>), dim3(a.B * ((a.T + 63) / 64)), dim3(512), lds, s, a);
+    hipLaunchKernelGGL((ffn_kernel<TM, D, true, true>), dim3(nb), dim3(512), lds, s, a, pf);
   } else if (a.pre_a) {
     const size_t lds = FfnGeom<D, true>::LDS;
-    hipLaunchKernelGGL((ffn_kernel<TM, D, true>), dim3((a.M + 63) / 64), dim3(512), lds, s, a);
+    hipLaunchKernelGGL((ffn_kernel<TM, D, true>), dim3(nb), dim3(512), lds, s, a, pf);
   } else {
     const size_t lds = FfnGeom<D, false>::LDS;
-    hipLaunchKernelGGL((ffn_kernel<TM, D, false>), dim3((a.M + 63) / 64), dim3(512), lds, s, a);
+    hipLaunchKernelGGL((ffn_kernel<TM, D, false>), dim3(nb), dim3(512), lds, s, a, pf);
   }
   return hipGetLastError();
 }
@@ -658,7 +663,7 @@
   return ffn_eligible(a.dim, a.T, prec) && a.B >= 1 && a.M == a.B * a.T && !a.att_q;
 }
 
-hipError_t launch_ffn(const FfnArgs& a, int prec, hipStream_t s) {
+hipError_t launch_ffn(const FfnArgs& a, int prec, hipStream_t s, const PfArgs& pf, int* main_grid) {
   if (!ffn_eligible(a.dim, a.T, prec) || a.M <= 0 || a.M != a.B * a.T) return hipErrorInvalidValue;
   if (a.lens) {
     if (!ffn_masks_rows(a, prec)) return hipErrorInvalidValue;
@@ -673,8 +678,8 @@
     return hipErrorInvalidValue;
   if ((!a.pre_a && !a.att_q && (a.ldy & 7)) || (a.ldres & 3) || (a.out_f32 && (a.ldo_f32 & 3)) || (a.out_op && (a.ldo_op & 3))) return hipErrorInvalidValue;
   if (!a.pre_a && !a.att_q && (unsigned long long)a.M * a.ldy * 2ull > 0xFFF00000ull) return hipErrorInvalidValue;
-  if (prec == PREC_BF16) return a.dim == 128 ? launch_ffn_t<bf16_t, 128>(a, s) : launch_ffn_t<bf16_t, 256>(a, s);
-  return a.dim == 128 ? launch_ffn_t<f16_t, 128>(a, s) : launch_ffn_t<f16_t, 256>(a, s);
+  if (prec == PREC_BF16) return a.dim == 128 ? launch_ffn_t<bf16_t, 128>(a, s, pf, main_grid) : launch_ffn_t<bf16_t, 256>(a, s, pf, main_grid);
+  return a.dim == 128 ? launch_ffn_t<f16_t, 128>(a, s, pf, main_grid) : launch_ffn_t<f16_t, 256>(a, s, pf, main_grid);
 }
 
 template <typename TM>
diff --git a/ns2vc_amd/csrc/geglu.hip b/ns2vc_amd/csrc/geglu.hip
--- a/ns2vc_amd/csrc/geglu.hip
+++ b/ns2vc_amd/csrc/geglu.hip
@@ -60,7 +60,8 @@
 }
 
 template <typename TM, int D, bool MASKED = false>
-__global__ __launch_bounds__(512) void geglu_kernel(const GegluArgs a) {
+__global__ __launch_bounds__(512) void geglu_kernel(const GegluArgs a, const PfArgs pf) {
+  pf_block(pf);
   op_mode_init<TM>();
   using G = GegluGeom<D>;
   constexpr int KT = G::KT, UB = G::UB, NP = G::NP, RING = GG_RING;
@@ -453,9 +454,11 @@
   return hipSuccess;
 }
 
-template <typename TM, bool MASKED> static hipError_t launch_geglu_t(const GegluArgs& a, hipStream_t s) {
+template <typename TM, bool MASKED> static hipError_t launch_geglu_t(const GegluArgs& a, hipStream_t s, const PfArgs& pf_, int* main_grid) {
   const int ntb = (a.M + GG_TOK - 1) / GG_TOK;
-  hipLaunchKernelGGL((geglu_kernel<TM, 384, MASKED>), dim3(ntb * GG_SPLIT), dim3(512), GegluGeom<384>::LDS, s, a);
+  if (main_grid) { *main_grid = ntb * GG_SPLIT; return hipSuccess; }
+  const PfArgs pf = pf_.first == ntb * GG_SPLIT ? pf_ : PfArgs();
+  hipLaunchKernelGGL((geglu_kernel<TM, 384, MASKED>), dim3(ntb * GG_SPLIT + pf.count), dim3(512), GegluGeom<384>::LDS, s, a, pf);
   return hipGetLastError();
 }
 
@@ -463,15 +466,15 @@
   return geglu_eligible(a.dim, 1, prec) && a.M > 0 && a.T >= 1 && (a.M % a.T) == 0;
 }
 
-hipError_t launch_geglu(const GegluArgs& a, int prec, hipStream_t s) {
+hipError_t launch_geglu(const GegluArgs& a, int prec, hipStream_t s, const PfArgs& pf, int* main_grid) {
   if (!geglu_eligible(a.dim, 1, prec) || a.M <= 0) return hipErrorInvalidValue;
   if (!a.yn || !a.wstream || !a.consts || !a.out_op) return hipErrorInvalidValue;
   if (!a.lens && !a.ln_stats) return hipErrorInvalidValue;
   if (a.lens && !geglu_masks_rows(a, prec)) return hipErrorInvalidValue;
   if (a.ldy < a.dim || a.ldo < 4 * a.dim || (a.ldy & 7) || (a.ldo & 7) || (unsigned long long)a.M * a.ldy * 2ull > 0xFFF00000ull || (unsigned long long)a.M * a.ldo * 2ull > 0x7FF00000ull) return hipErrorInvalidValue;
   if ((reinterpret_cast<uintptr_t>(a.out_op) & 15) != 0) return hipErrorInvalidValue;
-  if (a.lens) return prec == PREC_BF16 ? launch_geglu_t<bf16_t, true>(a, s) : launch_geglu_t<f16_t, true>(a, s);
-  return prec == PREC_BF16 ? launch_geglu_t<bf16_t, false>(a, s) : launch_geglu_t<f16_t, false>(a, s);
+  if (a.lens) return prec == PREC_BF16 ? launch_geglu_t<bf16_t, true>(a, s, pf, main_grid) : launch_geglu_t<f16_t, true>(a, s, pf, main_grid);
+  return prec == PREC_BF16 ? launch_geglu_t<bf16_t, false>(a, s, pf, main_grid) : launch_geglu_t<f16_t, false>(a, s, pf, main_grid);
 }
 
 hipError_t init_geglu_attributes() {
diff --git a/ns2vc_amd/csrc/gemm.hip b/ns2vc_amd/csrc/gemm.hip
--- a/ns2vc_amd/csrc/gemm.hip
+++ b/ns2vc_amd/csrc/gemm.hip
@@ -329,7 +329,8 @@
   static constexpr int NW = SPEC == 0 ? 8 : NL + NC;
 };
 template <typename TM, int BM, int BN, int STAGES, bool LNC, int SPEC = 0, bool GNP = false, bool MASKED = false>
-__global__ __launch_bounds__(64 * G4Waves<SPEC>::NW) void gemm4_kernel(const GemmArgs g NS2VC_G4_FLAGS_PARAM) {
+__global__ __launch_bounds__(64 * G4Waves<SPEC>::NW) void gemm4_kernel(const GemmArgs g, const PfArgs pf NS2VC_G4_FLAGS_PARAM) {
+  pf_block(pf);
   op_mode_init<TM>();
   constexpr int EPC = MmaT<TM>::EPC;
   constexpr int BKE = 8 * EPC;
@@ -640,19 +641,22 @@
   return ring > epi ? ring : epi;
 }
 template <typename TM, int BM, int BN, int STAGES, int SPEC = 0>
-static hipError_t launch_cfg4(const GemmArgs& g, hipStream_t s) {
+static hipError_t launch_cfg4(const GemmArgs& g, hipStream_t s, const PfArgs& pf_, int* main_grid) {
   int nb = (g.N / BN) * ((g.M + BM - 1) / BM);
   if (g.gnp_x && g.gnp_sync && g.N / BN > 1) nb = 8 * (((g.M + BM - 1) / BM + 7) / 8) * (g.N / BN);
+  if (main_grid) { *main_grid = nb; return hipSuccess; }
+  const PfArgs pf = pf_.first == nb ? pf_ : PfArgs();
+  nb += pf.count;
 #if NS2VC_GEMM_ABLATE
   if (g.lens) return hipErrorInvalidValue;
-  if (g.gnp_x) hipLaunchKernelGGL((gemm4_kernel<TM, BM, BN, STAGES, false, SPEC, true>), dim3(nb), dim3(64 * G4Waves<SPEC>::NW), gemm4_lds_bytes(BM, BN, STAGES), s, g, g_gemm_flags);
-  else if (g.ln_stats) hipLaunchKernelGGL((gemm4_kernel<TM, BM, BN, STAGES, true, SPEC>), dim3(nb), dim3(64 * G4Waves<SPEC>::NW), gemm4_lds_bytes(BM, BN, STAGES), s, g, g_gemm_flags);
-  else hipLaunchKernelGGL((gemm4_kernel<TM, BM, BN, STAGES, false, SPEC>), dim3(nb), dim3(64 * G4Waves<SPEC>::NW), gemm4_lds_bytes(BM, BN, STAGES), s, g, g_gemm_flags);
+  if (g.gnp_x) hipLaunchKernelGGL((gemm4_kernel<TM, BM, BN, STAGES, false, SPEC, true>), dim3(nb), dim3(64 * G4Waves<SPEC>::NW), gemm4_lds_bytes(BM, BN, STAGES), s, g, pf, g_gemm_flags);
+  else if (g.ln_stats) hipLaunchKernelGGL((gemm4_kernel<TM, BM, BN, STAGES, true, SPEC>), dim3(nb), dim3(64 * G4Waves<SPEC>::NW), gemm4_lds_bytes(BM, BN, STAGES), s, g, pf, g_gemm_flags);
+  else hipLaunchKernelGGL((gemm4_kernel<TM, BM, BN, STAGES, false, SPEC>), dim3(nb), dim3(64 * G4Waves<SPEC>::NW), gemm4_lds_bytes(BM, BN, STAGES), s, g, pf, g_gemm_flags);
 #else
-  if (g.lens) hipLaunchKernelGGL((gemm4_kernel<TM, BM, BN, STAGES, false, SPEC, false, true>), dim3(nb), dim3(64 * G4Waves<SPEC>::NW), gemm4_lds_bytes(BM, BN, STAGES), s, g);
-  else if (g.gnp_x) hipLaunchKernelGGL((gemm4_kernel<TM, BM, BN, STAGES, false, SPEC, true>), dim3(nb), dim3(64 * G4Waves<SPEC>::NW), gemm4_lds_bytes(BM, BN, STAGES), s, g);
-  else if (g.ln_stats) hipLaunchKernelGGL((gemm4_kernel<TM, BM, BN, STAGES, true, SPEC>), dim3(nb), dim3(64 * G4Waves<SPEC>::NW), gemm4_lds_bytes(BM, BN, STAGES), s, g);
-  else hipLaunchKernelGGL((gemm4_kernel<TM, BM, BN, STAGES, false, SPEC>), dim3(nb), dim3(64 * G4Waves<SPEC>::NW), gemm4_lds_bytes(BM, BN, STAGES), s, g);
+  if (g.lens) hipLaunchKernelGGL((gemm4_kernel<TM, BM, BN, STAGES, false, SPEC, false, true>), dim3(nb), dim3(64 * G4Waves<SPEC>::NW), gemm4_lds_bytes(BM, BN, STAGES), s, g, pf);
+  else if (g.gnp_x) hipLaunchKernelGGL((gemm4_kernel<TM, BM, BN, STAGES, false, SPEC, true>), dim3(nb), dim3(64 * G4Waves<SPEC>::NW), gemm4_lds_bytes(BM, BN, STAGES), s, g, pf);
+  else if (g.ln_stats) hipLaunchKernelGGL((gemm4_kernel<TM, BM, BN, STAGES, true, SPEC>), dim3(nb), dim3(64 * G4Waves<SPEC>::NW), gemm4_lds_bytes(BM, BN, STAGES), s, g, pf);
+  else hipLaunchKernelGGL((gemm4_kernel<TM, BM, BN, STAGES, false, SPEC>), dim3(nb), dim3(64 * G4Waves<SPEC>::NW), gemm4_lds_bytes(BM, BN, STAGES), s, g, pf);
 #endif
   return hipGetLastError();
 }
@@ -669,7 +673,7 @@
   if (bm == -3 || bm == -4) { g_ts = bm == -4 ? 1 : 0; g_ts_nl = (bm == -4 && (stages == 4 || stages == 8)) ? stages : 0; g_ts_ks = bm == -4 ? (bn == 1 ? 1 : bn == 2 ? 0 : -1) : -1; return; } g_force_bm = bm; g_force_bn = bn; g_force_st = stages & 255; g_gemm_flags = stages >> 8; }
 
 template <typename TM>
-static hipError_t launch_typed(const GemmArgs& g, hipStream_t s, bool dry = false) {
+static hipError_t launch_typed(const GemmArgs& g, hipStream_t s, bool dry = false, const PfArgs& pf = PfArgs(), int* main_grid = nullptr) {
   const int bke = 128 / (int)sizeof(TM);
   const int nk = g.K / bke;
   int bm, bn, st;
@@ -701,18 +705,19 @@
   if (dry) return hipSuccess;
   if (st >= 22 && st <= 44) {
     if (bn != 128) return gemm_invalid(__LINE__);
-#define NS2VC_CASE4S(BM_, ST_, SP_) if (bm == BM_ && st == 10 * (1 + SP_) + ST_) return launch_cfg4<TM, BM_, 128, ST_, SP_>(g, s)
+#define NS2VC_CASE4S(BM_, ST_, SP_) if (bm == BM_ && st == 10 * (1 + SP_) + ST_) return launch_cfg4<TM, BM_, 128, ST_, SP_>(g, s, pf, main_grid)
     NS2VC_CASE4S(128, 3, 1); NS2VC_CASE4S(64, 3, 1);
 #undef NS2VC_CASE4S
     return gemm_invalid(__LINE__);
   }
   if (st == 12 || st == 13) {
     if (bn != 128) return gemm_invalid(__LINE__);
-#define NS2VC_CASE4(BM_, ST_) if (bm == BM_ && st == 10 + ST_) return launch_cfg4<TM, BM_, 128, ST_>(g, s)
+#define NS2VC_CASE4(BM_, ST_) if (bm == BM_ && st == 10 + ST_) return launch_cfg4<TM, BM_, 128, ST_>(g, s, pf, main_grid)
     NS2VC_CASE4(128, 2); NS2VC_CASE4(128, 3); NS2VC_CASE4(64, 2); NS2VC_CASE4(64, 3);
 #undef NS2VC_CASE4
     return gemm_invalid(__LINE__);
   }
+  if (main_grid) { *main_grid = 0; return hipSuccess; }
 #define NS2VC_CASE(BM_, BN_, ST_) if (bm == BM_ && bn == BN_ && st == ST_) return launch_cfg<TM, BM_, BN_, ST_>(g, s)
   NS2VC_CASE(64, 128, 2);
   NS2VC_CASE(64, 64, 2); NS2VC_CASE(64, 64, 3); NS2VC_CASE(64, 64, 4);
@@ -720,7 +725,7 @@
   return gemm_invalid(__LINE__);
 }
 
-hipError_t launch_gemm(const GemmArgs& g_, int prec, hipStream_t s) {
+hipError_t launch_gemm(const GemmArgs& g_, int prec, hipStream_t s, const PfArgs& pf, int* main_grid) {
   GemmArgs g = g_;
   if (g.N % 64 != 0 || g.M <= 0) return gemm_invalid(__LINE__);
   if (g.N / 64 > 15) g.gnp_sync = nullptr;
@@ -757,16 +762,16 @@
     const bool forced_ks = g_force_bm == 128 && g_force_bn == 64 && (g_force_st == 64 || g_force_st == 68);
     const bool forced_ts = (g_force_bm == 128 && (g_force_st == 54 || g_force_st == 58)) || forced_ks;
     if (g.algo != 1 && (forced_ts || (g_ts && !g_force_bm)) && convts_eligible(g, prec))
-      return launch_convts(g, prec, forced_ts ? g_force_bn : 0, forced_ts ? g_force_st % 10 : g_ts_nl, forced_ts ? (forced_ks ? 1 : 0) : g_ts_ks, s);
+      return launch_convts(g, prec, forced_ts ? g_force_bn : 0, forced_ts ? g_force_st % 10 : g_ts_nl, forced_ts ? (forced_ks ? 1 : 0) : g_ts_ks, s, pf, main_grid);
     if (forced_ts) return gemm_invalid(__LINE__);
   }
   if (g.sol_coef) return gemm_invalid(__LINE__);
   if (g.gnp_pair) return gemm_invalid(__LINE__);
   if (g.lens && g.gnp_x) return gemm_invalid(__LINE__);
   switch (prec) {
-    case PREC_BF16: return launch_typed<bf16_t>(g, s);
-    case PREC_F16: return launch_typed<f16_t>(g, s);
-    case PREC_F32: return launch_typed<float>(g, s);
+    case PREC_BF16: return launch_typed<bf16_t>(g, s, false, pf, main_grid);
+    case PREC_F16: return launch_typed<f16_t>(g, s, false, pf, main_grid);
+    case PREC_F32: return launch_typed<float>(g, s, false, pf, main_grid);
     default: return gemm_invalid(__LINE__);
   }
 }
diff --git a/ns2vc_amd/csrc/mma.h b/ns2vc_amd/csrc/mma.h
--- a/ns2vc_amd/csrc/mma.h
+++ b/ns2vc_amd/csrc/mma.h
@@ -67,5 +67,19 @@
 }
 template <int N> __device__ __forceinline__ void wait_vmcnt() { asm volatile("s_waitcnt vmcnt(%0)" ::"i"(N) : "memory"); }
 
+__device__ __forceinline__ void pf_block(const PfArgs& pf) {
+  if (__builtin_expect((int)blockIdx.x < pf.first, 1)) return;
+  const int idx = (int)blockIdx.x - pf.first;
+  const PfSlice sl = pf_slice(pf.bytes, pf.count, idx);
+  const i32x4_t rsrc = make_rsrc(pf.p, pf.bytes);
+  const unsigned nt = blockDim.x;
+  for (unsigned l = threadIdx.x; l < sl.lines; l += nt) {
+    unsigned v;
+    asm volatile("buffer_load_dword %0, %1, %2, 0 offen" : "=&v"(v) : "v"(pf_offset(sl.first_line + l)), "s"(rsrc) : "memory");
+  }
+  wait_vmcnt<0>();
+  __builtin_amdgcn_endpgm();
+}
+
 
 }
diff --git a/ns2vc_amd/csrc/pack.cpp b/ns2vc_amd/csrc/pack.cpp
--- a/ns2vc_amd/csrc/pack.cpp
+++ b/ns2vc_amd/csrc/pack.cpp
@@ -151,6 +151,7 @@
     void* d = nullptr;
     if (hipMalloc(&d, std::max<size_t>(bytes, 1)) != hipSuccess) { err = fail("hipMalloc failed (%s)", what); return nullptr; }
     h->weight_allocs.push_back(d);
+    h->weight_alloc_bytes[d] = bytes;
     if (hipMemcpy(d, src, bytes, hipMemcpyHostToDevice) != hipSuccess) err = fail("hipMemcpy failed (weights)");
     return d;
   }
diff --git a/ns2vc_amd/csrc/plan.cpp b/ns2vc_amd/csrc/plan.cpp
--- a/ns2vc_amd/csrc/plan.cpp
+++ b/ns2vc_amd/csrc/plan.cpp
@@ -93,6 +93,16 @@
     Op op;
     op.name = name; op.fn = std::move(fn); op.kind = kind; op.flops = flops; op.bytes = bytes;
     ops->push_back(std::move(op));
+  }
+  void reads_weights(const void* w) {
+    if (sizing || !w) return;
+    auto it = h->weight_alloc_bytes.find(w);
+    if (it == h->weight_alloc_bytes.end()) return;
+    ops->back().weights = w; ops->back().weight_bytes = it->second;
+  }
+  void carries(std::shared_ptr<PfArgs> pf, std::function<int()> grid, int family, int fixed = 0) {
+    if (sizing) return;
+    ops->back().pf = std::move(pf); ops->back().main_grid = std::move(grid); ops->back().pf_family = family; ops->back().pf_fixed = fixed;
   }
   void temb_reader() {
     if (sizing || ops != &h->fwd_ops) return;
@@ -128,7 +138,16 @@
       if (g.gnp_x && g.algo == 0) g.algo = 2;
     } else if (masked && g.stats) { stats_of.erase(g.out_f32); g.stats = nullptr; }
     if (g.gnp_temb) temb_reader();
-    add(g.gnp_x ? name + "[+norm]" : name, [=](hipStream_t s) { return launch_gemm(g, pr, s); }, 1, flops, bytes + pro);
+    auto pf = std::make_shared<PfArgs>();
+    add(g.gnp_x ? name + "[+norm]" : name, [=](hipStream_t s) { return launch_gemm(g, pr, s, *pf); }, 1, flops, bytes + pro);
+    if (!sizing) {
+      Op& op = ops->back();
+      op.weights = (g.w_tiled && gemm_uses_convts(g, pr)) ? g.w_tiled : g.w;
+      op.weight_bytes = (size_t)g.N * g.K * operand_bytes(pr);
+      op.pf = pf;
+      op.pf_family = PF_FAM_GEMM;
+      op.main_grid = [=]() { int n = 0; return launch_gemm(g, pr, nullptr, PfArgs(), &n) == hipSuccess ? n : 0; };
+    }
     if (!sizing && g.gnp_x && g.gnp_sync) {
       unsigned* words = g.gnp_sync;
       const size_t nbytes = (((size_t)g.B * g.Tin + 63) / 64) * 8;
@@ -256,8 +275,10 @@
       a.q_lens = lens_of(Lq);
       if (self) a.k_lens = lens_of(Lk);
     } else if (self) a.bias = selfbias_of(Lk);
-    add(name, [=](hipStream_t s) { return launch_attention(a, hd, pr, s); }, 2, 4.0 * B * a.H * (double)Lq * Lk * hd,
+    auto pf = std::make_shared<PfArgs>();
+    add(name, [=](hipStream_t s) { return launch_attention(a, hd, pr, s, *pf); }, 2, 4.0 * B * a.H * (double)Lq * Lk * hd,
         (double)opsz * B * a.H * hd * (2.0 * Lq + 2.0 * Lk));
+    carries(pf, [=]() { int n = 0; return launch_attention(a, hd, pr, nullptr, PfArgs(), &n) == hipSuccess ? n : 0; }, PF_FAM_ATTN, PF_ATTN_BLOCKS);
     if (!self_mask) mask(name, out, ldo, a.H * hd, opsz, Lq);
   }
 
@@ -295,8 +316,11 @@
       }
       if (!res && stream == a.chain_in && a.chain_in_s2 && h->slice_rows && 2 * ((M + 63) / 64) <= h->cus + 8) { c.wstream = a.chain_in_s2; c.slices = 2; }
       if (lens_rows) { c.lens = lens_of(Tl); c.T = Tl; }
-      add(c.slices == 2 ? nm + "[2 slices]" : nm, [=](hipStream_t s) { return launch_rowchain(c, pr, s); }, 1, 2.0 * M * (double)d * (d + n2),
+      auto pf = std::make_shared<PfArgs>();
+      add(c.slices == 2 ? nm + "[2 slices]" : nm, [=](hipStream_t s) { return launch_rowchain(c, pr, s, *pf); }, 1, 2.0 * M * (double)d * (d + n2),
           (double)M * (d * ((gn_st ? 4.0 : opsz) + 4.0 + (res ? 4.0 : 0.0)) + n2 * opsz) + (double)(d + n2) * d * opsz);
+      reads_weights(c.wstream);
+      carries(pf, [=]() { int n = 0; return launch_rowchain(c, pr, nullptr, PfArgs(), &n) == hipSuccess ? n : 0; }, PF_FAM_CHAIN);
     };
     auto chains_mask_rows = [&]() {
       ns2vc_rowchain_args c;
@@ -383,10 +407,13 @@
       f.B = B; f.T = Tl; f.M = M; f.dim = d; f.ln_health = h->ln_health;
       if (lens_ffn) f.lens = lens_of(Tl);
       const double fl = 2.0 * M * (double)d * ((ffn_pre ? 14.0 : 13.0) * d) + (xatt ? 4.0 * B * h->cfg.heads * (double)Tl * Lp * hd : 0.0);
+      auto pf = std::make_shared<PfArgs>();
       add(a.prefix + (xatt ? ".ffn[attn2.sdpa+to_out+geglu+ff.out+proj_out]" : ffn_pre ? ".ffn[attn2.to_out+geglu+ff.out+proj_out]" : ".ffn[geglu+ff.out+proj_out]"),
-          [=](hipStream_t s) { return launch_ffn(f, pr, s); }, 1, fl,
+          [=](hipStream_t s) { return launch_ffn(f, pr, s, *pf); }, 1, fl,
           (double)M * d * (opsz + 8.0 + (ffn_pre ? 4.0 : 0.0) + (out_op ? opsz : 0.0)) + (ffn_pre ? 14.0 : 13.0) * d * d * opsz +
               (xatt ? (double)opsz * B * d * 2.0 * Lp : 0.0));
+      reads_weights(f.wstream);
+      carries(pf, [=]() { int n = 0; return launch_ffn(f, pr, nullptr, PfArgs(), &n) == hipSuccess ? n : 0; }, PF_FAM_CHAIN);
       return;
     }
     auto geglu_masks = [&]() {
@@ -405,8 +432,11 @@
       if (lens_geglu) { f.yn = qb; f.ln_stats = nullptr; f.T = Tl; f.lens = lens_of(Tl); }
       f.wstream = a.geglu_stream; f.consts = a.geglu_consts;
       f.out_op = ffh; f.ldo = 4 * d; f.M = M; f.dim = d; f.ln_health = h->ln_health;
-      add(t + ".ff.geglu[token-stationary]", [=](hipStream_t s) { return launch_geglu(f, pr, s); }, 1, 2.0 * M * (double)d * 8.0 * d,
+      auto pf = std::make_shared<PfArgs>();
+      add(t + ".ff.geglu[token-stationary]", [=](hipStream_t s) { return launch_geglu(f, pr, s, *pf); }, 1, 2.0 * M * (double)d * 8.0 * d,
           (double)M * d * opsz * 5.0 + (double)M * (d / 64) * 8.0 + 8.0 * d * d * opsz);
+      reads_weights(f.wstream);
+      carries(pf, [=]() { int n = 0; return launch_geglu(f, pr, nullptr, PfArgs(), &n) == hipSuccess ? n : 0; }, PF_FAM_CHAIN);
     } else {
       g = base(yn, d, d, Tl, Tl, a.ff1, nullptr, ffh, 4 * d);
       g.geglu = 1;
@@ -699,11 +729,37 @@
   }
   h->arena_used = P.off;
   h->stats_bytes = std::max<size_t>(P.stats_used, 1) * sizeof(long long);
+  if (!sizing) assign_prefetch(h);
   h->tfork.ok = !sizing && h->tfork.begin > 0 && h->tfork.end > h->tfork.begin && h->tfork.join >= h->tfork.end && h->tfork.first >= h->tfork.join;
   if (!sizing && h->fork_temb && !h->tfork.ok)
     fprintf(stderr, "ns2vc: fork_temb refused for this plan (join at launch %d, first reader of the time scale / shift rows at %d): the step graph stays linear\n",
             h->tfork.join, h->tfork.first);
   return 0;
+}
+
+void assign_prefetch(ns2vc_unet* h) {
+  std::vector<Op>& ops = h->fwd_ops;
+  const int n = (int)ops.size();
+  for (int i = 0; i < n; ++i) {
+    Op& op = ops[i];
+    op.pf_for = -1;
+    if (!op.pf) continue;
+    *op.pf = PfArgs();
+    if (!h->prefetch_next || !op.main_grid || !(op.pf_family & NS2VC_PF_FAMILIES)) continue;
+    int j = -1;
+    for (int d = 1; d <= n && j < 0; ++d)
+      if (ops[(i + d) % n].weights && ops[(i + d) % n].weight_bytes) j = (i + d) % n;
+    if (j < 0 || j == i) continue;
+    const int grid = op.main_grid();
+    if (grid > h->cus && op.pf_family != PF_FAM_ATTN && !(NS2VC_PF_FAMILIES & PF_FAM_MULTIROUND)) continue;
+    const int count = grid <= 0 ? 0 : op.pf_fixed > 0 ? op.pf_fixed : pf_blocks(grid, h->cus);
+    if (count <= 0) continue;
+    op.pf->p = ops[j].weights;
+    op.pf->bytes = pf_budget(ops[j].weight_bytes, count);
+    op.pf->first = grid;
+    op.pf->count = count;
+    op.pf_for = j;
+  }
 }
 
 bool temb_forks(const ns2vc_unet* h, size_t last) {
diff --git a/ns2vc_amd/csrc/prefetch.h b/ns2vc_amd/csrc/prefetch.h
--- /dev/null
+++ b/ns2vc_amd/csrc/prefetch.h
@@ -0,0 +1,60 @@
+#pragma once
+
+#if defined(__HIPCC__) || defined(__CUDACC__)
+#define NS2VC_PF_HD __host__ __device__
+#else
+#define NS2VC_PF_HD
+#endif
+
+namespace ns2vc {
+
+constexpr unsigned PF_LINE = 128;
+constexpr int PF_MAX_BLOCKS = 16;
+constexpr int PF_ATTN_BLOCKS = 8;
+enum { PF_FAM_GEMM = 1, PF_FAM_CHAIN = 2, PF_FAM_ATTN = 4, PF_FAM_MULTIROUND = 8 };
+#ifndef NS2VC_PF_FAMILIES
+#define NS2VC_PF_FAMILIES 15
+#endif
+constexpr unsigned PF_BLOCK_BYTES = 256u << 10;
+
+struct PfArgs {
+  const void* p = nullptr;
+  unsigned bytes = 0;
+  int first = 0x7fffffff;
+  int count = 0;
+};
+
+NS2VC_PF_HD inline int pf_blocks(int main_grid, int cus) {
+  if (main_grid <= 0 || cus <= 0) return 0;
+  const int used = main_grid % cus;
+  if (used == 0) return 0;
+  const int idle = cus - used;
+  return idle < PF_MAX_BLOCKS ? idle : PF_MAX_BLOCKS;
+}
+NS2VC_PF_HD inline unsigned pf_budget(unsigned long long bytes, int count) {
+  const unsigned long long cap = (unsigned long long)(count > 0 ? count : 0) * PF_BLOCK_BYTES;
+  return (unsigned)(bytes < cap ? bytes : cap);
+}
+
+NS2VC_PF_HD inline unsigned pf_lines(unsigned bytes) { return bytes / PF_LINE + (bytes % PF_LINE ? 1u : 0u); }
+
+struct PfSlice { unsigned first_line, lines; };
+NS2VC_PF_HD inline PfSlice pf_slice(unsigned bytes, int count, int idx) {
+  PfSlice s = {0u, 0u};
+  if (count <= 0 || idx < 0 || idx >= count) return s;
+  const unsigned total = pf_lines(bytes);
+  const unsigned per = total / (unsigned)count + (total % (unsigned)count ? 1u : 0u);
+  const unsigned long long lo = (unsigned long long)per * (unsigned)idx;
+  if (lo >= total) return s;
+  s.first_line = (unsigned)lo;
+  s.lines = total - s.first_line < per ? total - s.first_line : per;
+  return s;
+}
+NS2VC_PF_HD inline unsigned pf_offset(unsigned line) { return line * PF_LINE; }
+NS2VC_PF_HD inline unsigned pf_line_bytes(unsigned bytes, unsigned line) {
+  const unsigned long long lo = (unsigned long long)line * PF_LINE;
+  if (lo >= bytes) return 0u;
+  return bytes - lo < PF_LINE ? (unsigned)(bytes - lo) : PF_LINE;
+}
+
+}
diff --git a/ns2vc_amd/csrc/rowchain.hip b/ns2vc_amd/csrc/rowchain.hip
--- a/ns2vc_amd/csrc/rowchain.hip
+++ b/ns2vc_amd/csrc/rowchain.hip
@@ -44,7 +44,8 @@
 };
 
 template <typename TM, int D, int R2, int NT, bool MASKED = false>
-__global__ __launch_bounds__(512) void rowchain_kernel(const RowchainArgs a) {
+__global__ __launch_bounds__(512) void rowchain_kernel(const RowchainArgs a, const PfArgs pf) {
+  pf_block(pf);
   op_mode_init<TM>();
   using G = RowchainGeom<D, R2, NT>;
   constexpr int KT = G::KT, NB1 = G::NB1, S1 = G::S1, S2 = G::S2, NP = G::NP, RING = G::RING, TOK = G::TOK, PTILE = G::PTILE;
@@ -461,25 +462,28 @@
   return (dim == 128 || dim == 256 || dim == 384) && (n2 == dim || n2 == 3 * dim) && T >= 1 && (prec == PREC_BF16 || prec == PREC_F16);
 }
 
-template <typename TM, int D, int R2, int NT, bool MASKED> static hipError_t launch_rc(const RowchainArgs& a, hipStream_t s) {
+template <typename TM, int D, int R2, int NT, bool MASKED> static hipError_t launch_rc(const RowchainArgs& a, hipStream_t s, const PfArgs& pf_, int* main_grid) {
   constexpr int TOK = RowchainGeom<D, R2, NT>::TOK;
   const size_t lds = RowchainGeom<D, R2, NT>::LDS + (MASKED ? TOK * 4 : 0);
   static_assert(RowchainGeom<D, R2, NT>::LDS + TOK * 4 <= 160 * 1024, "LDS budget of the masked form");
   const int nblk = (a.M + TOK - 1) / TOK, S = a.slices > 1 ? a.slices : 1;
-  hipLaunchKernelGGL((rowchain_kernel<TM, D, R2, NT, MASKED>), dim3(S > 1 ? ((nblk + 7) / 8) * 8 * S : nblk), dim3(512), lds, s, a);
+  const int nb = S > 1 ? ((nblk + 7) / 8) * 8 * S : nblk;
+  if (main_grid) { *main_grid = nb; return hipSuccess; }
+  const PfArgs pf = pf_.first == nb ? pf_ : PfArgs();
+  hipLaunchKernelGGL((rowchain_kernel<TM, D, R2, NT, MASKED>), dim3(nb + pf.count), dim3(512), lds, s, a, pf);
   return hipGetLastError();
 }
 static int g_force_nt = 0;
 void set_forced_rowchain_tokens(int nt) { g_force_nt = nt; }
-template <typename TM, bool MK> static hipError_t launch_rc_tm(const RowchainArgs& a, hipStream_t s) {
+template <typename TM, bool MK> static hipError_t launch_rc_tm(const RowchainArgs& a, hipStream_t s, const PfArgs& pf, int* main_grid) {
   if (a.dim == 128) {
     const bool big = g_force_nt ? g_force_nt == 2 : (a.M + 63) / 64 > 256;
-    if (big) return a.n2 == 128 ? launch_rc<TM, 128, 1, 2, MK>(a, s) : launch_rc<TM, 128, 3, 2, MK>(a, s);
-    return a.n2 == 128 ? launch_rc<TM, 128, 1, 1, MK>(a, s) : launch_rc<TM, 128, 3, 1, MK>(a, s);
-  }
-  if (a.dim == 384 && a.slices == 2) return a.n2 == 384 ? launch_rc<TM, 384, 2, 1, MK>(a, s) : launch_rc<TM, 384, 5, 1, MK>(a, s);
-  if (a.dim == 384) return a.n2 == 384 ? launch_rc<TM, 384, 3, 1, MK>(a, s) : launch_rc<TM, 384, 9, 1, MK>(a, s);
-  return a.n2 == 256 ? launch_rc<TM, 256, 2, 1, MK>(a, s) : launch_rc<TM, 256, 6, 1, MK>(a, s);
+    if (big) return a.n2 == 128 ? launch_rc<TM, 128, 1, 2, MK>(a, s, pf, main_grid) : launch_rc<TM, 128, 3, 2, MK>(a, s, pf, main_grid);
+    return a.n2 == 128 ? launch_rc<TM, 128, 1, 1, MK>(a, s, pf, main_grid) : launch_rc<TM, 128, 3, 1, MK>(a, s, pf, main_grid);
+  }
+  if (a.dim == 384 && a.slices == 2) return a.n2 == 384 ? launch_rc<TM, 384, 2, 1, MK>(a, s, pf, main_grid) : launch_rc<TM, 384, 5, 1, MK>(a, s, pf, main_grid);
+  if (a.dim == 384) return a.n2 == 384 ? launch_rc<TM, 384, 3, 1, MK>(a, s, pf, main_grid) : launch_rc<TM, 384, 9, 1, MK>(a, s, pf, main_grid);
+  return a.n2 == 256 ? launch_rc<TM, 256, 2, 1, MK>(a, s, pf, main_grid) : launch_rc<TM, 256, 6, 1, MK>(a, s, pf, main_grid);
 }
 
 bool rowchain_masks_rows(const RowchainArgs& a, int prec) {
@@ -487,7 +491,7 @@
   return !a.gn_x || a.T >= 64;
 }
 
-hipError_t launch_rowchain(const RowchainArgs& a, int prec, hipStream_t s) {
+hipError_t launch_rowchain(const RowchainArgs& a, int prec, hipStream_t s, const PfArgs& pf, int* main_grid) {
   if (!rowchain_eligible(a.dim, a.n2, 64, prec) || a.M <= 0) return hipErrorInvalidValue;
   if (a.slices > 1 && (a.slices != 2 || a.dim != 384 || (a.res && (const void*)a.res == (const void*)a.out1_f32))) return hipErrorInvalidValue;
   if ((!a.a_op && !a.gn_x) || !a.wstream || !a.bias1 || !a.consts2 || !a.out2_op) return hipErrorInvalidValue;
@@ -499,9 +503,9 @@
   if ((unsigned long long)a.M * a.lda * 2ull > 0xFFF00000ull) return hipErrorInvalidValue;
   if (a.lens) {
     if (!rowchain_masks_rows(a, prec)) return hipErrorInvalidValue;
-    return prec == PREC_BF16 ? launch_rc_tm<bf16_t, true>(a, s) : launch_rc_tm<f16_t, true>(a, s);
-  }
-  return prec == PREC_BF16 ? launch_rc_tm<bf16_t, false>(a, s) : launch_rc_tm<f16_t, false>(a, s);
+    return prec == PREC_BF16 ? launch_rc_tm<bf16_t, true>(a, s, pf, main_grid) : launch_rc_tm<f16_t, true>(a, s, pf, main_grid);
+  }
+  return prec == PREC_BF16 ? launch_rc_tm<bf16_t, false>(a, s, pf, main_grid) : launch_rc_tm<f16_t, false>(a, s, pf, main_grid);
 }
 
 hipError_t init_rowchain_attributes() {
diff --git a/ns2vc_amd/engine.py b/ns2vc_amd/engine.py
--- a/ns2vc_amd/engine.py
+++ b/ns2vc_amd/engine.py
@@ -360,6 +360,19 @@
             out[name.value.decode()] = int(v.value)
         return out
 
+    def prefetch_info(self) -> List[Dict[str, object]]:
+        nf, _ = self.launches()
+        out = []
+        name = C.create_string_buffer(256)
+        kind, fl, by = C.c_int(), C.c_double(), C.c_double()
+        for i in range(nf):
+            check(self.lib.ns2vc_unet_op_info(self.h, 4, i, name, 256, C.byref(kind), C.byref(fl), C.byref(by)), "op_info(4)")
+            rec = {"name": name.value.decode(), "weight_bytes": int(by.value), "blocks": int(kind.value)}
+            check(self.lib.ns2vc_unet_op_info(self.h, 3, i, name, 256, C.byref(kind), C.byref(fl), C.byref(by)), "op_info(3)")
+            rec.update(target=int(kind.value), target_name=name.value.decode(), offset=int(fl.value), bytes=int(by.value))
+            out.append(rec)
+        return out
+
     def profile_forward(self, reps: int = 5, stream=None) -> np.ndarray:
         nf, _ = self.launches()
         ms = (C.c_float * nf)()
```

Result: no change. 286.5 denoiser-steps/s (batch 32 per GPU, whole job), median of 6 (+0.9%).
